# mengcaopku/DCNet

Measured on AMD Instinct MI355X. Metric: clips/sec (T=8, 416x416, bs8) fwd+bwd, higher is better.
Workload: dtype f32; 1 GPU; T=8 416x416 bs8/GPU L=20 fp32, 64 img/GPU/step as pairs, fwd+5 losses+bwd+RMSprop; arith=f16x2-split MFMA, fp32 accumulate, parallelism=dp1, ranks_seen=1, reducer=none, step=hipGraph replay (fwd+losses+bwd+RMSprop), sampler=mt

## Files before the change

### dcnet_amd/csrc/optim.hip

```cpp
#include "common.h"

namespace {

constexpr int RMS_CHUNK = 32;
template <int K> struct Chunk { float* t[K][RMS_CHUNK]; long long n[RMS_CHUNK]; };

template <int W, bool READ, class F>
__device__ __forceinline__ void walk(float* const (&w)[W], const float* __restrict__ g, const long long n, F f) {
  uintptr_t bits = READ ? (uintptr_t)g : 0;
#pragma unroll
  for (int k = 0; k < W; ++k) bits |= (uintptr_t)w[k];
  const long long n4 = (bits & 15) == 0 ? n / 4 : 0;
  const long long stride = (long long)gridDim.x * 256;
  for (long long i = (long long)blockIdx.x * 256 + threadIdx.x; i < n4; i += stride) {
    f32x4 x[W];
#pragma unroll
    for (int k = 0; k < W; ++k) x[k] = reinterpret_cast<const f32x4*>(w[k])[i];
    const f32x4 gg = READ ? reinterpret_cast<const f32x4*>(g)[i] : f32x4{};
#pragma unroll
    for (int e = 0; e < 4; ++e) {
      float a[W];
#pragma unroll
      for (int k = 0; k < W; ++k) a[k] = x[k][e];
      f(a, gg[e]);
#pragma unroll
      for (int k = 0; k < W; ++k) x[k][e] = a[k];
    }
#pragma unroll
    for (int k = 0; k < W; ++k) reinterpret_cast<f32x4*>(w[k])[i] = x[k];
  }
  for (long long i = n4 * 4 + (long long)blockIdx.x * 256 + threadIdx.x; i < n; i += stride) {
    float a[W];
#pragma unroll
    for (int k = 0; k < W; ++k) a[k] = w[k][i];
    f(a, READ ? g[i] : 0.f);
#pragma unroll
    for (int k = 0; k < W; ++k) w[k][i] = a[k];
  }
}

__device__ __forceinline__ void rms_update(float& p, const float g0, float& v, float lr, float alpha, float eps, float wd) {
#pragma clang fp contract(off)
  const float g = wd != 0.f ? g0 + wd * p : g0;
  v = v * alpha + (1.f - alpha) * g * g;
  p = p - lr * (g / (sqrtf(v) + eps));
}

constexpr int CTL_NORM = 0, CTL_COEF = 1, CTL_APPLY = 2, CTL_SKIPS = 3;
__device__ __forceinline__ float clip_mul(const float g0, const float coef) {
#pragma clang fp contract(off)
  return g0 * coef;
}

template <bool CLIP, int NS, int K, class F>
__device__ __forceinline__ void update_walk(const Chunk<K>& c, const float* __restrict__ ctl, F f) {
  static_assert(K >= 2 + NS, "parameter, gradient and NS state tables");
  float coef = 1.f;
  if (CLIP) {
    if (reinterpret_cast<const int*>(ctl)[CTL_APPLY] == 0) return;
    coef = ctl[CTL_COEF];
  }
  const int t = blockIdx.y;
  float* w[1 + NS];
  w[0] = c.t[0][t];
#pragma unroll
  for (int k = 0; k < NS; ++k) w[1 + k] = c.t[2 + k][t];
  walk<1 + NS, true>(w, c.t[1][t], c.n[t], [=](float (&a)[1 + NS], const float g0) { f(a, CLIP ? clip_mul(g0, coef) : g0); });
}

template <bool CLIP>
__device__ __forceinline__ void rmsprop_body(const Chunk<3>& c, float lr, const float* __restrict__ lr_dev, float alpha, float eps, float wd,
                                             const float* __restrict__ ctl) {
  if (lr_dev) lr = lr_dev[0];
  update_walk<CLIP, 1>(c, ctl, [=](float (&a)[2], const float g) { rms_update(a[0], g, a[1], lr, alpha, eps, wd); });
}

__global__ __launch_bounds__(256) void rmsprop_kernel(const Chunk<3> c, float lr, const float* __restrict__ lr_dev, float alpha, float eps, float wd) {
  rmsprop_body<false>(c, lr, lr_dev, alpha, eps, wd, nullptr);
}
__global__ __launch_bounds__(256) void rmsprop_clip_kernel(const Chunk<3> c, float lr, const float* __restrict__ lr_dev, float alpha, float eps, float wd,
                                                           const float* __restrict__ ctl) {
  rmsprop_body<true>(c, lr, lr_dev, alpha, eps, wd, ctl);
}

constexpr int STEP_CHUNK = 128;
struct StepChunk { int* step[STEP_CHUNK]; float* scal[STEP_CHUNK]; };

__device__ __forceinline__ void adam_prepare_body(const StepChunk& c, float lr, const float* __restrict__ lr_dev, double beta1, double beta2) {
  if (threadIdx.x != 0) return;
  if (lr_dev) lr = lr_dev[0];
  const int t = c.step[blockIdx.x][0] + 1;
  c.step[blockIdx.x][0] = t;
  const double bc1 = 1.0 - pow(beta1, (double)t), bc2 = 1.0 - pow(beta2, (double)t);
  c.scal[blockIdx.x][0] = (float)((double)lr / bc1);
  c.scal[blockIdx.x][1] = (float)(1.0 / sqrt(bc2));
}

__global__ __launch_bounds__(64) void adam_prepare_kernel(const StepChunk c, float lr, const float* __restrict__ lr_dev, double beta1, double beta2) {
  adam_prepare_body(c, lr, lr_dev, beta1, beta2);
}
__global__ __launch_bounds__(64) void adam_prepare_clip_kernel(const StepChunk c, float lr, const float* __restrict__ lr_dev, double beta1, double beta2,
                                                               const int* __restrict__ ctl) {
  if (ctl[CTL_APPLY] == 0) return;
  adam_prepare_body(c, lr, lr_dev, beta1, beta2);
}

__global__ __launch_bounds__(64) void adamw_prepare_kernel(const StepChunk c, float lr, const float* __restrict__ lr_dev, double beta1, double beta2,
                                                           double wd, const int* __restrict__ ctl) {
  if (ctl && ctl[CTL_APPLY] == 0) return;
  adam_prepare_body(c, lr, lr_dev, beta1, beta2);
  if (threadIdx.x != 0) return;
  if (lr_dev) lr = lr_dev[0];
  c.scal[blockIdx.x][2] = (float)(1.0 - (double)lr * wd);
}

__device__ __forceinline__ void adam_update(float& p, const float g0, float& m, float& v, float step_size, float inv_bc2_sqrt, float w1,
                                            float beta2, float w2, float eps, float wd) {
#pragma clang fp contract(off)
  const float g = wd != 0.f ? g0 + wd * p : g0;
  const float d = g - m;
  m = w1 < 0.5f ? m + w1 * d : g - d * (1.f - w1);
  v = v * beta2 + w2 * g * g;
  const float denom = sqrtf(v) * inv_bc2_sqrt + eps;
  p = p - step_size * (m / denom);
}

__device__ __forceinline__ void adamw_update(float& p, const float g, float& m, float& v, float step_size, float inv_bc2_sqrt, float decay,
                                             float w1, float beta2, float w2, float eps) {
#pragma clang fp contract(off)
  const float q = p * decay;
  const float d = g - m;
  m = w1 < 0.5f ? m + w1 * d : g - d * (1.f - w1);
  v = v * beta2 + w2 * g * g;
  const float denom = sqrtf(v) * inv_bc2_sqrt + eps;
  p = q - step_size * (m / denom);
}

template <bool CLIP, bool DECOUPLED = false>
__device__ __forceinline__ void adam_body(const Chunk<5>& c, float w1, float beta2, float w2, float eps, float wd, const float* __restrict__ ctl) {
  const float* __restrict__ s = c.t[4][blockIdx.y];
  const float step_size = s[0], inv_bc2_sqrt = s[1], decay = DECOUPLED ? s[2] : 1.f;
  update_walk<CLIP, 2>(c, ctl, [=](float (&a)[3], const float g) {
    if (DECOUPLED) adamw_update(a[0], g, a[1], a[2], step_size, inv_bc2_sqrt, decay, w1, beta2, w2, eps);
    else adam_update(a[0], g, a[1], a[2], step_size, inv_bc2_sqrt, w1, beta2, w2, eps, wd);
  });
}

__global__ __launch_bounds__(256) void adamw_kernel(const Chunk<5> c, float w1, float beta2, float w2, float eps) {
  adam_body<false, true>(c, w1, beta2, w2, eps, 0.f, nullptr);
}
__global__ __launch_bounds__(256) void adamw_clip_kernel(const Chunk<5> c, float w1, float beta2, float w2, float eps, const float* __restrict__ ctl) {
  adam_body<true, true>(c, w1, beta2, w2, eps, 0.f, ctl);
}

__global__ __launch_bounds__(256) void adam_kernel(const Chunk<5> c, float w1, float beta2, float w2, float eps, float wd) {
  adam_body<false>(c, w1, beta2, w2, eps, wd, nullptr);
}
__global__ __launch_bounds__(256) void adam_clip_kernel(const Chunk<5> c, float w1, float beta2, float w2, float eps, float wd,
                                                        const float* __restrict__ ctl) {
  adam_body<true>(c, w1, beta2, w2, eps, wd, ctl);
}

__device__ __forceinline__ void sgd_update(float& p, const float g0, float& buf, float lr, float mu, float wd) {
#pragma clang fp contract(off)
  const float g = wd != 0.f ? g0 + wd * p : g0;
  buf = buf * mu + g;
  p = p - lr * buf;
}

template <bool CLIP>
__device__ __forceinline__ void sgd_body(const Chunk<3>& c, float lr, const float* __restrict__ lr_dev, float mu, float wd, const float* __restrict__ ctl) {
  if (lr_dev) lr = lr_dev[0];
  update_walk<CLIP, 1>(c, ctl, [=](float (&a)[2], const float g) { sgd_update(a[0], g, a[1], lr, mu, wd); });
}

__global__ __launch_bounds__(256) void sgd_kernel(const Chunk<3> c, float lr, const float* __restrict__ lr_dev, float mu, float wd) {
  sgd_body<false>(c, lr, lr_dev, mu, wd, nullptr);
}
__global__ __launch_bounds__(256) void sgd_clip_kernel(const Chunk<3> c, float lr, const float* __restrict__ lr_dev, float mu, float wd,
                                                       const float* __restrict__ ctl) {
  sgd_body<true>(c, lr, lr_dev, mu, wd, ctl);
}

__global__ __launch_bounds__(64) void ema_prepare_kernel(int* __restrict__ step, float* __restrict__ w, double decay, double tau,
                                                         const int* __restrict__ ctl) {
  if (threadIdx.x != 0 || blockIdx.x != 0) return;
  if (ctl && ctl[CTL_APPLY] == 0) return;
  const int t = step[0] + 1;
  step[0] = t;
  const double d = tau > 0.0 ? decay * (1.0 - exp(-(double)t / tau)) : decay;
  w[0] = (float)(1.0 - d);
}

template <bool WB, class F>
__device__ __forceinline__ void walk2(const Chunk<2>& c, F f) {
  const int t = blockIdx.y;
  float* __restrict__ a = c.t[0][t]; float* __restrict__ b = c.t[1][t];
  const long long n = c.n[t];
  const long long n4 = ((((uintptr_t)a | (uintptr_t)b) & 15) == 0) ? n / 4 : 0;
  const long long stride = (long long)gridDim.x * 256;
  f32x4* __restrict__ a4 = reinterpret_cast<f32x4*>(a); f32x4* __restrict__ b4 = reinterpret_cast<f32x4*>(b);
  const auto f4 = [&](f32x4& x, f32x4& y) {
#pragma unroll
    for (int e = 0; e < 4; ++e) {
      float xe = x[e], ye = y[e];
      f(xe, ye);
      x[e] = xe; y[e] = ye;
    }
  };
  long long i = (long long)blockIdx.x * 256 + threadIdx.x;
  for (; i + stride < n4; i += 2 * stride) {
    f32x4 x0 = a4[i], x1 = a4[i + stride], y0 = b4[i], y1 = b4[i + stride];
    f4(x0, y0); f4(x1, y1);
    a4[i] = x0; a4[i + stride] = x1;
    if (WB) { b4[i] = y0; b4[i + stride] = y1; }
  }
  for (; i < n4; i += stride) {
    f32x4 x0 = a4[i], y0 = b4[i];
    f4(x0, y0);
    a4[i] = x0;
    if (WB) b4[i] = y0;
  }
  for (i = n4 * 4 + (long long)blockIdx.x * 256 + threadIdx.x; i < n; i += stride) {
    float x = a[i], y = b[i];
    f(x, y);
    a[i] = x;
    if (WB) b[i] = y;
  }
}

__device__ __forceinline__ float ema_lerp(const float s, const float x, const float w) {
#pragma clang fp contract(off)
  const float d = x - s;
  const float r = w < 0.5f ? s + w * d : x - d * (1.f - w);
  return d == 0.f ? s : r;
}

__global__ __launch_bounds__(256) void ema_update_kernel(const Chunk<2> c, const float* __restrict__ wp, const int* __restrict__ ctl) {
  if (ctl && ctl[CTL_APPLY] == 0) return;
  const float w = wp[0];
  walk2<false>(c, [=](float& s, float& x) { s = ema_lerp(s, x, w); });
}

__global__ __launch_bounds__(256) void tensor_swap_kernel(const Chunk<2> c) {
  walk2<true>(c, [](float& a, float& b) { const float a0 = a; a = b; b = a0; });
}


template <int WAVES>
__device__ __forceinline__ double block_sum_f64(double v, double* red) {
#pragma unroll
  for (int o = 32; o > 0; o >>= 1) v += __shfl_xor(v, o);
  if ((threadIdx.x & 63) == 0) red[threadIdx.x >> 6] = v;
  __syncthreads();
  double s = red[0];
#pragma unroll
  for (int w = 1; w < WAVES; ++w) s += red[w];
  return s;
}

__device__ __forceinline__ f32x4 load4(const float* __restrict__ g, long long i, bool vec) {
  if (vec) return reinterpret_cast<const f32x4*>(g)[i];
  f32x4 r;
  r[0] = g[4 * i]; r[1] = g[4 * i + 1]; r[2] = g[4 * i + 2]; r[3] = g[4 * i + 3];
  return r;
}
__device__ __forceinline__ double add_squares(double acc, const f32x4 gg) {
#pragma unroll
  for (int e = 0; e < 4; ++e) { const double x = (double)gg[e]; acc += x * x; }
  return acc;
}

__global__ __launch_bounds__(256) void grad_sumsq_kernel(const Chunk<1> c, double* __restrict__ partials) {
  __shared__ double red[4];
  const int t = blockIdx.y;
  const float* __restrict__ g = c.t[0][t];
  const long long n = c.n[t], n4 = n / 4;
  const bool vec = (((uintptr_t)g) & 15) == 0;
  const long long stride = (long long)gridDim.x * 256;
  double acc = 0.0;
  long long i = (long long)blockIdx.x * 256 + threadIdx.x;
  for (; i + 3 * stride < n4; i += 4 * stride) {
    const f32x4 a = load4(g, i, vec), b = load4(g, i + stride, vec), d = load4(g, i + 2 * stride, vec), e = load4(g, i + 3 * stride, vec);
    acc = add_squares(add_squares(add_squares(add_squares(acc, a), b), d), e);
  }
  for (; i < n4; i += stride) acc = add_squares(acc, load4(g, i, vec));
  for (i = n4 * 4 + (long long)blockIdx.x * 256 + threadIdx.x; i < n; i += stride) {
    const double x = (double)g[i]; acc += x * x;
  }
  const double s = block_sum_f64<4>(acc, red);
  if (threadIdx.x == 0) partials[(long long)t * gridDim.x + blockIdx.x] = s;
}

__device__ __forceinline__ float clip_coef(const float norm, const float max_norm) {
#pragma clang fp contract(off)
  const float coef = max_norm / (norm + 1e-6f);
  return coef > 1.f ? 1.f : coef;
}

__global__ __launch_bounds__(1024) void grad_clip_coef_kernel(const double* __restrict__ partials, long long slots, float max_norm, int skip_nonfinite,
                                                              float* __restrict__ ctl) {
  __shared__ double red[16];
  double a0 = 0.0, a1 = 0.0, a2 = 0.0, a3 = 0.0;
  long long i = threadIdx.x;
  for (; i + 3 * 1024 < slots; i += 4 * 1024) {
    const double p0 = partials[i], p1 = partials[i + 1024], p2 = partials[i + 2 * 1024], p3 = partials[i + 3 * 1024];
    a0 += p0; a1 += p1; a2 += p2; a3 += p3;
  }
  if (i < slots) a0 += partials[i];
  if (i + 1024 < slots) a1 += partials[i + 1024];
  if (i + 2 * 1024 < slots) a2 += partials[i + 2 * 1024];
  const double s = block_sum_f64<16>((a0 + a1) + (a2 + a3), red);
  if (threadIdx.x != 0) return;
  const float norm = (float)sqrt(s);
  const int apply = (skip_nonfinite && !__builtin_isfinite(s)) ? 0 : 1;
  ctl[CTL_NORM] = norm;
  ctl[CTL_COEF] = clip_coef(norm, max_norm);
  int* w = reinterpret_cast<int*>(ctl);
  w[CTL_APPLY] = apply;
  if (!apply) w[CTL_SKIPS] = w[CTL_SKIPS] + 1;
}

__global__ __launch_bounds__(256) void grad_scale_kernel(const Chunk<1> c, const float* __restrict__ ctl) {
  const float coef = ctl[CTL_COEF];
  float* const w[1] = {c.t[0][blockIdx.y]};
  walk<1, false>(w, nullptr, c.n[blockIdx.y], [=](float (&a)[1], float) { a[0] = clip_mul(a[0], coef); });
}

inline unsigned blocks_for(long long biggest) {
  const long long bx = (biggest / 4 + 255) / 256;
  return (unsigned)(bx < 1 ? 1 : (bx > 128 ? 128 : bx));
}
inline long long longest(const int64_t* numel, int m) {
  long long biggest = 0;
  for (int i = 0; i < m; ++i)
    if (numel[i] > biggest) biggest = numel[i];
  return biggest;
}

template <class F>
inline int for_chunks(int count, int cap, F f) {
  for (int base = 0; base < count; base += cap) {
    const int e = f(base, count - base < cap ? count - base : cap);
    if (e != DCN_OK) return e;
  }
  return DCN_OK;
}

inline long long sumsq_slots(const int64_t* numel, int count) {
  long long total = 0;
  for_chunks(count, RMS_CHUNK, [&](int base, int m) {
    total += (long long)blocks_for(longest(numel + base, m)) * m;
    return DCN_OK;
  });
  return total;
}

template <int K> using Tables = const float* const* const (&)[K];

template <int K>
int check_tensors(const char* who, Tables<K> tab, const int64_t* numel, int count, bool empties = false) {
  for (int k = 0; k < count; ++k) {
    bool there = true;
    for (int j = 0; j < K; ++j) there = there && tab[j][k];
    DCN_CHECK_ARG(numel[k] >= 0 && (there || (empties && numel[k] == 0)), "%s: null tensor %d", who, k);
  }
  return DCN_OK;
}

template <int K, class L>
int launch_chunks(const char* who, Tables<K> tab, const int64_t* numel, int count, bool empties, L launch) {
  return for_chunks(count, RMS_CHUNK, [&](int base, int m) -> int {
    Chunk<K> c{};
    for (int i = 0; i < m; ++i) {
      for (int j = 0; j < K; ++j) c.t[j][i] = const_cast<float*>(tab[j][base + i]);
      c.n[i] = numel[base + i];
    }
    const long long biggest = longest(numel + base, m);
    if (empties && biggest == 0) return DCN_OK;
    launch(c, dim3(blocks_for(biggest), m));
    DCN_CHECK_LAUNCH(who);
    return DCN_OK;
  });
}

#define OPTIM_LAUNCH(kernel, ...) hipLaunchKernelGGL(kernel, grid, dim3(256), 0, (hipStream_t)stream, __VA_ARGS__)

}

extern "C" int64_t dcn_grad_sumsq_slots(const int64_t* numel, int count) {
  if (!numel || count <= 0) { dcn_set_error("grad_sumsq_slots: bad argument"); return -1; }
  for (int i = 0; i < count; ++i)
    if (numel[i] < 0) { dcn_set_error("grad_sumsq_slots: negative element count of tensor %d", i); return -1; }
  return sumsq_slots(numel, count);
}

extern "C" int dcn_grad_sumsq(const float* const* grads, const int64_t* numel, int count, double* partials, int64_t slots, void* stream) {
  DCN_CHECK_ARG(grads && numel && partials && count > 0, "grad_sumsq: bad argument");
  if (const int e = check_tensors<1>("grad_sumsq", {grads}, numel, count)) return e;
  DCN_CHECK_ARG(slots == sumsq_slots(numel, count), "grad_sumsq: the partials buffer has %lld slots, these tensors need %lld (dcn_grad_sumsq_slots)",
                (long long)slots, sumsq_slots(numel, count));
  long long at = 0;
  return launch_chunks<1>("grad_sumsq", {grads}, numel, count, false, [&](const Chunk<1>& c, dim3 grid) {
    OPTIM_LAUNCH(grad_sumsq_kernel, c, partials + at);
    at += (long long)grid.x * grid.y;
  });
}

extern "C" int dcn_grad_clip_coef(const double* partials, int64_t slots, float max_norm, int skip_nonfinite, void* ctrl, void* stream) {
  DCN_CHECK_ARG(partials && ctrl && slots > 0, "grad_clip_coef: bad argument");
  DCN_CHECK_ARG(max_norm > 0.f, "grad_clip_coef: max_norm %g is not a positive number", (double)max_norm);
  hipLaunchKernelGGL(grad_clip_coef_kernel, dim3(1), dim3(1024), 0, (hipStream_t)stream, partials, (long long)slots, max_norm, skip_nonfinite,
                     (float*)ctrl);
  DCN_CHECK_LAUNCH("grad_clip_coef");
  return DCN_OK;
}

extern "C" int dcn_grad_scale(float* const* grads, const int64_t* numel, int count, const void* ctrl, void* stream) {
  DCN_CHECK_ARG(grads && numel && ctrl && count > 0, "grad_scale: bad argument");
  if (const int e = check_tensors<1>("grad_scale", {grads}, numel, count)) return e;
  return launch_chunks<1>("grad_scale", {grads}, numel, count, false,
                          [&](const Chunk<1>& c, dim3 grid) { OPTIM_LAUNCH(grad_scale_kernel, c, (const float*)ctrl); });
}

static int rmsprop_step(const char* who, float* const* params, const float* const* grads, float* const* square_avgs, const int64_t* numel,
                        int count, float lr, const float* lr_dev, float alpha, float eps, float weight_decay, const float* ctl, void* stream) {
  DCN_CHECK_ARG(params && grads && square_avgs && numel && count > 0, "%s: bad argument", who);
  if (const int e = check_tensors<3>(who, {params, grads, square_avgs}, numel, count)) return e;
  return launch_chunks<3>(who, {params, grads, square_avgs}, numel, count, false, [&](const Chunk<3>& c, dim3 grid) {
    if (ctl) OPTIM_LAUNCH(rmsprop_clip_kernel, c, lr, lr_dev, alpha, eps, weight_decay, ctl);
    else OPTIM_LAUNCH(rmsprop_kernel, c, lr, lr_dev, alpha, eps, weight_decay);
  });
}

extern "C" int dcn_rmsprop_step(float* const* params, const float* const* grads, float* const* square_avgs, const int64_t* numel,
                                int count, float lr, const float* lr_dev, float alpha, float eps, float weight_decay, void* stream) {
  return rmsprop_step("rmsprop_step", params, grads, square_avgs, numel, count, lr, lr_dev, alpha, eps, weight_decay, nullptr, stream);
}

extern "C" int dcn_rmsprop_step_clipped(float* const* params, const float* const* grads, float* const* square_avgs, const int64_t* numel,
                                        int count, float lr, const float* lr_dev, float alpha, float eps, float weight_decay, const void* ctrl,
                                        void* stream) {
  DCN_CHECK_ARG(ctrl, "rmsprop_step_clipped: no control block");
  return rmsprop_step("rmsprop_step_clipped", params, grads, square_avgs, numel, count, lr, lr_dev, alpha, eps, weight_decay, (const float*)ctrl, stream);
}

static int adam_prepare(const char* who, bool decoupled, int* const* steps, float* const* scal, int count, float lr, const float* lr_dev, double beta1,
                        double beta2, double weight_decay, const int* ctl, void* stream) {
  DCN_CHECK_ARG(steps && scal && count > 0, "%s: bad argument", who);
  DCN_CHECK_ARG(beta1 >= 0.0 && beta1 < 1.0 && beta2 >= 0.0 && beta2 < 1.0, "%s: betas (%g, %g) outside [0, 1)", who, beta1, beta2);
  DCN_CHECK_ARG(!decoupled || weight_decay >= 0.0, "%s: negative weight_decay", who);
  for (int k = 0; k < count; ++k)
    DCN_CHECK_ARG(steps[k] && scal[k], "%s: null tensor %d", who, k);
  return for_chunks(count, STEP_CHUNK, [&](int base, int m) -> int {
    StepChunk c{};
    for (int i = 0; i < m; ++i) { c.step[i] = steps[base + i]; c.scal[i] = scal[base + i]; }
    const dim3 grid(m), block(64);
    if (decoupled) hipLaunchKernelGGL(adamw_prepare_kernel, grid, block, 0, (hipStream_t)stream, c, lr, lr_dev, beta1, beta2, weight_decay, ctl);
    else if (ctl) hipLaunchKernelGGL(adam_prepare_clip_kernel, grid, block, 0, (hipStream_t)stream, c, lr, lr_dev, beta1, beta2, ctl);
    else hipLaunchKernelGGL(adam_prepare_kernel, grid, block, 0, (hipStream_t)stream, c, lr, lr_dev, beta1, beta2);
    DCN_CHECK_LAUNCH(who);
    return DCN_OK;
  });
}

extern "C" int dcn_adam_prepare(int* const* steps, float* const* scal, int count, float lr, const float* lr_dev, double beta1, double beta2,
                                void* stream) {
  return adam_prepare("adam_prepare", false, steps, scal, count, lr, lr_dev, beta1, beta2, 0.0, nullptr, stream);
}

extern "C" int dcn_adam_prepare_clipped(int* const* steps, float* const* scal, int count, float lr, const float* lr_dev, double beta1, double beta2,
                                        const void* ctrl, void* stream) {
  DCN_CHECK_ARG(ctrl, "adam_prepare_clipped: no control block");
  return adam_prepare("adam_prepare_clipped", false, steps, scal, count, lr, lr_dev, beta1, beta2, 0.0, (const int*)ctrl, stream);
}

extern "C" int dcn_adamw_prepare(int* const* steps, float* const* scal, int count, float lr, const float* lr_dev, double beta1, double beta2,
                                 double weight_decay, void* stream) {
  return adam_prepare("adamw_prepare", true, steps, scal, count, lr, lr_dev, beta1, beta2, weight_decay, nullptr, stream);
}

extern "C" int dcn_adamw_prepare_clipped(int* const* steps, float* const* scal, int count, float lr, const float* lr_dev, double beta1, double beta2,
                                         double weight_decay, const void* ctrl, void* stream) {
  DCN_CHECK_ARG(ctrl, "adamw_prepare_clipped: no control block");
  return adam_prepare("adamw_prepare_clipped", true, steps, scal, count, lr, lr_dev, beta1, beta2, weight_decay, (const int*)ctrl, stream);
}

static int adam_step(const char* who, bool decoupled, float* const* params, const float* const* grads, float* const* exp_avgs,
                     float* const* exp_avg_sqs, const float* const* scal, const int64_t* numel, int count, double beta1, double beta2, float eps,
                     float weight_decay, const float* ctl, void* stream) {
  DCN_CHECK_ARG(params && grads && exp_avgs && exp_avg_sqs && scal && numel && count > 0, "%s: bad argument", who);
  DCN_CHECK_ARG(beta1 >= 0.0 && beta1 < 1.0 && beta2 >= 0.0 && beta2 < 1.0, "%s: betas (%g, %g) outside [0, 1)", who, beta1, beta2);
  if (decoupled) DCN_CHECK_ARG(eps >= 0.f, "%s: negative eps", who);
  else DCN_CHECK_ARG(eps >= 0.f && weight_decay >= 0.f, "%s: negative eps or weight_decay", who);
  if (const int e = check_tensors<5>(who, {params, grads, exp_avgs, exp_avg_sqs, scal}, numel, count)) return e;
  const float w1 = (float)(1.0 - beta1), b2 = (float)beta2, w2 = (float)(1.0 - beta2);
  return launch_chunks<5>(who, {params, grads, exp_avgs, exp_avg_sqs, scal}, numel, count, false, [&](const Chunk<5>& c, dim3 grid) {
    if (decoupled && ctl) OPTIM_LAUNCH(adamw_clip_kernel, c, w1, b2, w2, eps, ctl);
    else if (decoupled) OPTIM_LAUNCH(adamw_kernel, c, w1, b2, w2, eps);
    else if (ctl) OPTIM_LAUNCH(adam_clip_kernel, c, w1, b2, w2, eps, weight_decay, ctl);
    else OPTIM_LAUNCH(adam_kernel, c, w1, b2, w2, eps, weight_decay);
  });
}

extern "C" int dcn_adam_step(float* const* params, const float* const* grads, float* const* exp_avgs, float* const* exp_avg_sqs,
                             const float* const* scal, const int64_t* numel, int count, double beta1, double beta2, float eps,
                             float weight_decay, void* stream) {
  return adam_step("adam_step", false, params, grads, exp_avgs, exp_avg_sqs, scal, numel, count, beta1, beta2, eps, weight_decay, nullptr, stream);
}

extern "C" int dcn_adam_step_clipped(float* const* params, const float* const* grads, float* const* exp_avgs, float* const* exp_avg_sqs,
                                     const float* const* scal, const int64_t* numel, int count, double beta1, double beta2, float eps,
                                     float weight_decay, const void* ctrl, void* stream) {
  DCN_CHECK_ARG(ctrl, "adam_step_clipped: no control block");
  return adam_step("adam_step_clipped", false, params, grads, exp_avgs, exp_avg_sqs, scal, numel, count, beta1, beta2, eps, weight_decay,
                   (const float*)ctrl, stream);
}

extern "C" int dcn_adamw_step(float* const* params, const float* const* grads, float* const* exp_avgs, float* const* exp_avg_sqs,
                              const float* const* scal, const int64_t* numel, int count, double beta1, double beta2, float eps, void* stream) {
  return adam_step("adamw_step", true, params, grads, exp_avgs, exp_avg_sqs, scal, numel, count, beta1, beta2, eps, 0.f, nullptr, stream);
}

extern "C" int dcn_adamw_step_clipped(float* const* params, const float* const* grads, float* const* exp_avgs, float* const* exp_avg_sqs,
                                      const float* const* scal, const int64_t* numel, int count, double beta1, double beta2, float eps,
                                      const void* ctrl, void* stream) {
  DCN_CHECK_ARG(ctrl, "adamw_step_clipped: no control block");
  return adam_step("adamw_step_clipped", true, params, grads, exp_avgs, exp_avg_sqs, scal, numel, count, beta1, beta2, eps, 0.f, (const float*)ctrl,
                   stream);
}

static int sgd_step(const char* who, float* const* params, const float* const* grads, float* const* momentum_bufs, const int64_t* numel, int count,
                    float lr, const float* lr_dev, float momentum, float weight_decay, const float* ctl, void* stream) {
  DCN_CHECK_ARG(params && grads && momentum_bufs && numel && count > 0, "%s: bad argument", who);
  DCN_CHECK_ARG(momentum >= 0.f && weight_decay >= 0.f, "%s: negative momentum or weight_decay", who);
  if (const int e = check_tensors<3>(who, {params, grads, momentum_bufs}, numel, count)) return e;
  return launch_chunks<3>(who, {params, grads, momentum_bufs}, numel, count, false, [&](const Chunk<3>& c, dim3 grid) {
    if (ctl) OPTIM_LAUNCH(sgd_clip_kernel, c, lr, lr_dev, momentum, weight_decay, ctl);
    else OPTIM_LAUNCH(sgd_kernel, c, lr, lr_dev, momentum, weight_decay);
  });
}

extern "C" int dcn_sgd_step(float* const* params, const float* const* grads, float* const* momentum_bufs, const int64_t* numel, int count,
                            float lr, const float* lr_dev, float momentum, float weight_decay, void* stream) {
  return sgd_step("sgd_step", params, grads, momentum_bufs, numel, count, lr, lr_dev, momentum, weight_decay, nullptr, stream);
}

extern "C" int dcn_sgd_step_clipped(float* const* params, const float* const* grads, float* const* momentum_bufs, const int64_t* numel, int count,
                                    float lr, const float* lr_dev, float momentum, float weight_decay, const void* ctrl, void* stream) {
  DCN_CHECK_ARG(ctrl, "sgd_step_clipped: no control block");
  return sgd_step("sgd_step_clipped", params, grads, momentum_bufs, numel, count, lr, lr_dev, momentum, weight_decay, (const float*)ctrl, stream);
}

extern "C" int dcn_ema_prepare(int* step, float* w, double decay, double tau, const void* ctrl, void* stream) {
  DCN_CHECK_ARG(step && w, "ema_prepare: bad argument");
  DCN_CHECK_ARG(decay >= 0.0 && decay < 1.0, "ema_prepare: decay %g outside [0, 1)", decay);
  DCN_CHECK_ARG(tau >= 0.0, "ema_prepare: tau %g is negative", tau);
  hipLaunchKernelGGL(ema_prepare_kernel, dim3(1), dim3(64), 0, (hipStream_t)stream, step, w, decay, tau, (const int*)ctrl);
  DCN_CHECK_LAUNCH("ema_prepare");
  return DCN_OK;
}

extern "C" int dcn_ema_update(float* const* shadow, const float* const* src, const int64_t* numel, int count, const float* w, const void* ctrl,
                              void* stream) {
  DCN_CHECK_ARG(count >= 0 && w && (count == 0 || (shadow && src && numel)), "ema_update: bad argument");
  if (const int e = check_tensors<2>("ema_update", {shadow, src}, numel, count, true)) return e;
  return launch_chunks<2>("ema_update", {shadow, src}, numel, count, true,
                          [&](const Chunk<2>& c, dim3 grid) { OPTIM_LAUNCH(ema_update_kernel, c, w, (const int*)ctrl); });
}

extern "C" int dcn_tensor_swap(float* const* a, float* const* b, const int64_t* numel, int count, void* stream) {
  DCN_CHECK_ARG(count >= 0 && (count == 0 || (a && b && numel)), "tensor_swap: bad argument");
  if (const int e = check_tensors<2>("tensor_swap", {a, b}, numel, count, true)) return e;
  return launch_chunks<2>("tensor_swap", {a, b}, numel, count, true, [&](const Chunk<2>& c, dim3 grid) { OPTIM_LAUNCH(tensor_swap_kernel, c); });
}
```

### dcnet_amd/csrc/wprep.hip

```cpp
#include "common.h"

namespace {

struct FilterJob {
  const float* src;
  float* ohwi;
  float* ohwi_split;
  float* t;
  float* t_split;
  unsigned* amax;
  void* ohwi_b16;
  void* t_b16;
  int co, ci, T;
  int blk0;
  int ablk0;
  int pad_;
};

__device__ __forceinline__ int find_job(const FilterJob* jobs, int njobs, int b, bool amax) {
  int lo = 0, hi = njobs - 1;
  while (lo < hi) {
    const int mid = (lo + hi + 1) >> 1;
    if ((amax ? jobs[mid].ablk0 : jobs[mid].blk0) <= b) lo = mid; else hi = mid - 1;
  }
  return lo;
}

constexpr int AMAX_CHUNK = 4096;

__global__ __launch_bounds__(256) void filters_amax_kernel(const FilterJob* __restrict__ jobs, int njobs) {
  __shared__ float red[4];
  const int j = find_job(jobs, njobs, blockIdx.x, true);
  const FilterJob job = jobs[j];
  const long long numel = (long long)job.co * job.ci * job.T;
  const long long base = (long long)(blockIdx.x - job.ablk0) * AMAX_CHUNK;
  float vmax = 0.f;
#pragma unroll
  for (int k = 0; k < AMAX_CHUNK / 1024; ++k) {
    const long long i = base + k * 1024 + threadIdx.x * 4;
    if (i + 3 < numel) {
      const f32x4 v = *reinterpret_cast<const f32x4*>(job.src + i);
      vmax = fmaxf(fmaxf(vmax, fmaxf(fabsf(v[0]), fabsf(v[1]))), fmaxf(fabsf(v[2]), fabsf(v[3])));
    } else {
      for (long long q = i; q < numel; ++q) vmax = fmaxf(vmax, fabsf(job.src[q]));
    }
  }
  vmax = wave_max(vmax);
  if ((threadIdx.x & 63) == 0) red[threadIdx.x >> 6] = vmax;
  __syncthreads();
  if (threadIdx.x == 0) amax_update(job.amax, fmaxf(fmaxf(red[0], red[1]), fmaxf(red[2], red[3])), blockIdx.x);
}

__device__ __forceinline__ float scale_of(unsigned bits) {
  const int be = (int)((bits >> 23) & 0xFF);
  int e = (be == 0 || be == 255) ? 0 : 14 - (be - 126);
  e = e > 100 ? 100 : (e < -100 ? -100 : e);
  return __uint_as_float((unsigned)(e + 127) << 23);
}

typedef _Float16 f16x8_t __attribute__((ext_vector_type(8)));
__device__ __forceinline__ void split_store8(float* dst, const float* v, float s) {
  f16x8_t h, l;
#pragma unroll
  for (int k = 0; k < 8; ++k) { const float t = v[k] * s; h[k] = (_Float16)t; l[k] = (_Float16)(t - (float)h[k]); }
  *reinterpret_cast<f16x8_t*>(dst) = h;
  *reinterpret_cast<f16x8_t*>(dst + 4) = l;
}

__global__ __launch_bounds__(256) void filters_xform_kernel(const FilterJob* __restrict__ jobs, int njobs) {
  __shared__ float tile[32][33];
  const int j = find_job(jobs, njobs, blockIdx.x, false);
  const FilterJob job = jobs[j];
  const int tci = job.ci / 32, tco = job.co / 32;
  int b = blockIdx.x - job.blk0;
  const int ci0 = (b % tci) * 32; b /= tci;
  const int co0 = (b % tco) * 32; b /= tco;
  const int tap = b;
  const float s = scale_of(amax_read(job.amax));
  const long long numel = (long long)job.co * job.ci * job.T;
  const int r = threadIdx.x >> 3, c4 = (threadIdx.x & 7) * 4;
  {
    const float* sp = job.src + ((long long)(co0 + r) * job.ci + ci0 + c4) * job.T + tap;
#pragma unroll
    for (int e = 0; e < 4; ++e) tile[r][c4 + e] = sp[(long long)e * job.T];
  }
  __syncthreads();
  if (job.ohwi) {
    const f32x4 v = {tile[r][c4], tile[r][c4 + 1], tile[r][c4 + 2], tile[r][c4 + 3]};
    *reinterpret_cast<f32x4*>(job.ohwi + ((long long)(co0 + r) * job.T + tap) * job.ci + ci0 + c4) = v;
  }
  if (job.t) {
    const f32x4 v = {tile[c4][r], tile[c4 + 1][r], tile[c4 + 2][r], tile[c4 + 3][r]};
    *reinterpret_cast<f32x4*>(job.t + ((long long)(ci0 + r) * job.T + tap) * job.co + co0 + c4) = v;
  }
  if (threadIdx.x < 128) {
    const int rr = threadIdx.x >> 2, g = (threadIdx.x & 3) * 8;
    float v[8];
    typedef __bf16 bf16x8_t __attribute__((ext_vector_type(8)));
    if (job.ohwi_b16) {
      bf16x8_t b;
#pragma unroll
      for (int e = 0; e < 8; ++e) b[e] = (__bf16)tile[rr][g + e];
      *reinterpret_cast<bf16x8_t*>(reinterpret_cast<__bf16*>(job.ohwi_b16) + ((long long)(co0 + rr) * job.T + tap) * job.ci + ci0 + g) = b;
    }
    if (job.t_b16) {
      bf16x8_t b;
#pragma unroll
      for (int e = 0; e < 8; ++e) b[e] = (__bf16)tile[g + e][rr];
      *reinterpret_cast<bf16x8_t*>(reinterpret_cast<__bf16*>(job.t_b16) + ((long long)(ci0 + rr) * job.T + tap) * job.co + co0 + g) = b;
    }
    if (job.ohwi_split) {
#pragma unroll
      for (int e = 0; e < 8; ++e) v[e] = tile[rr][g + e];
      split_store8(job.ohwi_split + ((long long)(co0 + rr) * job.T + tap) * job.ci + ci0 + g, v, s);
    }
    if (job.t_split) {
#pragma unroll
      for (int e = 0; e < 8; ++e) v[e] = tile[g + e][rr];
      split_store8(job.t_split + ((long long)(ci0 + rr) * job.T + tap) * job.co + co0 + g, v, s);
    }
  }
  if (blockIdx.x == job.blk0 && threadIdx.x == 0) {
    if (job.ohwi_split) job.ohwi_split[numel] = s;
    if (job.t_split) job.t_split[numel] = s;
  }
}

}

extern "C" int dcn_filter_job_bytes(void) { return (int)sizeof(FilterJob); }

extern "C" int dcn_prepare_filters(const void* jobs, int njobs, int total_blocks, int total_amax_blocks,
                                   uint32_t* amax_all, int64_t amax_words, void* stream_) {
  hipStream_t stream = (hipStream_t)stream_;
  DCN_CHECK_ARG(jobs && njobs > 0 && total_blocks > 0 && total_amax_blocks > 0 && amax_all && amax_words > 0, "prepare_filters: bad argument");
  if (hipMemsetAsync(amax_all, 0, (size_t)amax_words * 4, stream) != hipSuccess) { dcn_set_error("prepare_filters: memset failed"); return DCN_ERR_LAUNCH; }
  hipLaunchKernelGGL(filters_amax_kernel, dim3(total_amax_blocks), dim3(256), 0, stream, (const FilterJob*)jobs, njobs);
  DCN_CHECK_LAUNCH("filters_amax");
  hipLaunchKernelGGL(filters_xform_kernel, dim3(total_blocks), dim3(256), 0, stream, (const FilterJob*)jobs, njobs);
  DCN_CHECK_LAUNCH("filters_xform");
  return DCN_OK;
}
```

### dcnet_amd/darknet.py

```python
from __future__ import annotations

import os
from typing import Dict, List, Optional, Sequence

import numpy as np
import torch
import torch.nn as nn

from . import convblock, ops


def parse_model_config(path: str) -> List[dict]:
    blocks: List[dict] = []
    with open(path, "r") as fh:
        for raw in fh:
            line = raw.strip()
            if not line or line.startswith("#"):
                continue
            if line.startswith("["):
                blocks.append({"type": line[1:-1].rstrip()})
                if blocks[-1]["type"] in ("convolutional", "yoloconvolutional"):
                    blocks[-1]["batch_normalize"] = 0
            else:
                key, value = line.split("=", 1)
                blocks[-1][key.strip()] = value.strip()
    return blocks


_ANCHORS = "10,13,  16,30,  33,23,  30,61,  62,45,  59,119,  116,90,  156,198,  373,326"


def yolov3_blocks(width: int = 416, height: int = 416) -> List[dict]:
    blocks: List[dict] = [dict(type="net", batch="1", subdivisions="1", width=str(width), height=str(height),
                               channels="3", momentum="0.9", decay="0.0005")]

    def conv(filters, size, stride=1, bn=1, act="leaky", kind="convolutional"):
        b = {"type": kind, "batch_normalize": bn} if bn else {"type": kind, "batch_normalize": 0}
        if bn:
            b["batch_normalize"] = "1"
        b.update(filters=str(filters), size=str(size), stride=str(stride), pad="1", activation=act)
        blocks.append(b)

    def shortcut():
        blocks.append({"type": "shortcut", "from": "-3", "activation": "linear"})

    conv(32, 3)
    for filters, reps in ((64, 1), (128, 2), (256, 8), (512, 8), (1024, 4)):
        conv(filters, 3, 2)
        for _ in range(reps):
            conv(filters // 2, 1); conv(filters, 3); shortcut()
    for mask, (filters, lateral) in zip(("6,7,8", "3,4,5", "0,1,2"), ((512, None), (256, 61), (128, 36))):
        if lateral is not None:
            blocks.append({"type": "route", "layers": "-4"})
            conv(filters, 1)
            blocks.append({"type": "upsample", "stride": "2"})
            blocks.append({"type": "route", "layers": f"-1, {lateral}"})
        for _ in range(2):
            conv(filters, 1); conv(filters * 2, 3)
        conv(filters, 1, kind="yoloconvolutional")
        conv(filters * 2, 3)
        conv(255, 1, bn=0, act="linear")
        blocks.append({"type": "yolo", "mask": mask, "anchors": _ANCHORS, "classes": "80", "num": "9",
                       "jitter": ".3", "ignore_thresh": ".7", "truth_thresh": "1", "random": "1"})
    return blocks


def write_cfg(path: str, blocks: Optional[Sequence[dict]] = None) -> None:
    blocks = yolov3_blocks() if blocks is None else blocks
    with open(path, "w") as fh:
        for b in blocks:
            fh.write(f"[{b['type']}]\n")
            for k, v in b.items():
                if k != "type" and not (k == "batch_normalize" and str(v) == "0"):
                    fh.write(f"{k}={v}\n")
            fh.write("\n")


class EmptyLayer(nn.Module):
    """Placeholder for route / shortcut slots (model/darknet.py:239-243)."""


class MyUpsample2(nn.Module):
    def forward(self, x):
        return x[:, :, :, None, :, None].expand(-1, -1, -1, 2, -1, 2).reshape(x.size(0), x.size(1), x.size(2) * 2, x.size(3) * 2)


class YOLOLayer(nn.Module):
    def __init__(self, anchors, num_classes, img_dim):
        super().__init__()
        self.anchors, self.num_classes, self.image_dim = anchors, num_classes, img_dim


def create_modules(module_defs: List[dict]):
    hyper = module_defs.pop(0)
    filters_out = [int(hyper["channels"])]
    module_list = nn.ModuleList()
    for i, d in enumerate(module_defs):
        seq = nn.Sequential()
        t = d["type"]
        if t in ("convolutional", "yoloconvolutional"):
            bn = int(d["batch_normalize"]); filters = int(d["filters"]); k = int(d["size"])
            pad = (k - 1) // 2 if int(d["pad"]) else 0
            seq.add_module(f"conv_{i}", nn.Conv2d(filters_out[-1], filters, k, int(d["stride"]), pad, bias=not bn))
            if bn:
                seq.add_module(f"batch_norm_{i}", nn.BatchNorm2d(filters))
            if d["activation"] == "leaky":
                seq.add_module(f"leaky_{i}", nn.LeakyReLU(0.1))
        elif t == "upsample":
            assert int(d["stride"]) == 2
            seq.add_module(f"upsample_{i}", MyUpsample2())
            filters = filters_out[-1]
        elif t == "route":
            layers = [int(x) for x in d["layers"].split(",")]
            filters = sum(filters_out[1:][l] if l >= 0 else filters_out[l] for l in layers)
            seq.add_module(f"route_{i}", EmptyLayer())
        elif t == "shortcut":
            filters = filters_out[int(d["from"])]
            seq.add_module(f"shortcut_{i}", EmptyLayer())
        elif t == "yolo":
            idx = [int(x) for x in d["mask"].split(",")]
            a = [int(x) for x in d["anchors"].split(",")]
            a = [(a[j], a[j + 1]) for j in range(0, len(a), 2)]
            seq.add_module(f"yolo_{i}", YOLOLayer([a[j] for j in idx], int(d["classes"]), 256))
            filters = filters_out[-1]
        else:
            raise ValueError(f"unsupported cfg block type {t!r}")
        module_list.append(seq)
        filters_out.append(filters)
    return hyper, module_list



class _ConvOp:
    __slots__ = ("slot", "src", "dst", "res", "cin", "cout", "k", "stride", "bn", "leaky", "need_dx")


class _UpCatOp:
    __slots__ = ("dst", "up_src", "lat_src", "c_up", "c_lat")


class _AliasOp:
    __slots__ = ("dst", "src")


def build_plan(module_defs: List[dict], in_channels: int = 3):
    n = len(module_defs)
    ch: List[int] = []
    prev = in_channels
    for i, d in enumerate(module_defs):
        t = d["type"]
        if t in ("convolutional", "yoloconvolutional"):
            prev = int(d["filters"])
        elif t == "route":
            ls = [int(x) for x in d["layers"].split(",")]
            prev = sum(ch[l if l >= 0 else i + l] for l in ls)
        elif t == "shortcut":
            prev = ch[i + int(d["from"])]
        ch.append(prev)
    taps = [i - 1 for i, d in enumerate(module_defs) if d["type"] == "yoloconvolutional"]
    live = [False] * n
    stack = list(taps)
    while stack:
        i = stack.pop()
        if i < 0 or live[i]:
            continue
        live[i] = True
        d = module_defs[i]; t = d["type"]
        if t in ("convolutional", "yoloconvolutional", "upsample"):
            stack.append(i - 1)
        elif t == "shortcut":
            stack += [i - 1, i + int(d["from"])]
        elif t == "route":
            stack += [l if l >= 0 else i + l for l in (int(x) for x in d["layers"].split(","))]
    consumers: Dict[int, List[int]] = {i: [] for i in range(-1, n)}
    for i, d in enumerate(module_defs):
        if not live[i]:
            continue
        t = d["type"]
        if t in ("convolutional", "yoloconvolutional", "upsample"):
            consumers[i - 1].append(i)
        elif t == "shortcut":
            consumers[i - 1].append(i); consumers[i + int(d["from"])].append(i)
        elif t == "route":
            for l in (int(x) for x in d["layers"].split(",")):
                consumers[l if l >= 0 else i + l].append(i)
    plan = []
    fused_shortcuts = set(); fused_upsamples = set()
    for i, d in enumerate(module_defs):
        if not live[i]:
            continue
        t = d["type"]
        if t in ("convolutional", "yoloconvolutional"):
            op = _ConvOp()
            op.slot = i; op.src = i - 1; op.dst = i; op.res = None
            op.cin = in_channels if i == 0 else ch[i - 1]; op.cout = int(d["filters"])
            op.k = int(d["size"]); op.stride = int(d["stride"])
            op.bn = bool(int(d["batch_normalize"])); op.leaky = d["activation"] == "leaky"
            op.need_dx = i > 0
            nxt = module_defs[i + 1] if i + 1 < n else None
            if (nxt is not None and nxt["type"] == "shortcut" and live[i + 1] and consumers[i] == [i + 1]
                    and i not in taps):
                op.dst = i + 1; op.res = i + 1 + int(nxt["from"])
                fused_shortcuts.add(i + 1)
            plan.append(op)
        elif t == "shortcut":
            if i not in fused_shortcuts:
                raise NotImplementedError("unfused shortcut (pattern not present in YOLOv3)")
        elif t == "upsample":
            nxt = module_defs[i + 1]
            ok = nxt["type"] == "route" and consumers[i] == [i + 1]
            ls = [int(x) for x in nxt["layers"].split(",")] if ok else []
            if not (ok and len(ls) == 2 and ls[0] == -1):
                raise NotImplementedError("upsample not followed by route(-1, k)")
            fused_upsamples.add(i + 1)
            op = _UpCatOp()
            op.dst = i + 1; op.up_src = i - 1; op.lat_src = ls[1] if ls[1] >= 0 else i + 1 + ls[1]
            op.c_up = ch[i - 1]; op.c_lat = ch[op.lat_src]
            plan.append(op)
        elif t == "route":
            if i in fused_upsamples:
                continue
            ls = [int(x) for x in d["layers"].split(",")]
            if len(ls) != 1:
                raise NotImplementedError("route concat without upsample")
            op = _AliasOp(); op.dst = i; op.src = ls[0] if ls[0] >= 0 else i + ls[0]
            plan.append(op)
    return plan, taps, ch



def _inputs(op):
    return (op.src, op.res) if isinstance(op, _ConvOp) else (op.up_src, op.lat_src) if isinstance(op, _UpCatOp) else (op.src,)


def _cpad(c: int) -> int:
    return 4 if c <= 4 else ops.pad32(c)


def _b16_diag_layer(diag, op, p, x, res, w, bank, act, out, amx):
    fold = (p["gamma"], p["beta"], p["rm"], p["rv"], 1e-5)
    if not diag.get("layers", lambda s_: True)(op.slot):
        ops.set_precision(diag.get("arith", "fp32"))
        try:
            ss = ops.bn_fold(*fold) if op.bn else (None, p["b"])
            o, _ = ops.conv2d_fwd(ops.to_f32(x), w, op.k, op.stride, ss[0], ss[1], act, 0.1,
                                  residual=None if res is None else ops.to_f32(diag.get("_r32", {}).get(op.res, res)))
        finally:
            ops.set_precision("bf16s")
        if res is not None and diag.get("res32"):
            diag.setdefault("_r32", {})[op.dst] = o
        out[op.dst] = o; amx[op.dst] = None
        return x, res, True
    x = ops.to_b16(x)
    if res is not None and diag.get("res32"):
        o32, _ = convblock.conv_forward(x, op.k, op.stride, op.cout, bank=bank, fold=fold, act=act, slope=0.1, out_f32=True)
        r32 = diag.setdefault("_r32", {})
        o32 = o32 + (r32[op.res] if op.res in r32 else ops.to_f32(res))
        r32[op.dst] = o32
        out[op.dst] = ops.to_b16(o32); amx[op.dst] = None
        return x, res, True
    return x, (None if res is None else ops.to_b16(res)), False


def _run_forward(plan, taps, x_nhwc, P, training: bool, save: Optional[dict], banks=None, taps_b16: bool = False):
    out: Dict[int, torch.Tensor] = {-1: x_nhwc}
    am = ops.use_amax()
    s16 = ops.storage_b16()
    amx: Dict[int, Optional[torch.Tensor]] = {-1: None}
    readers: Dict[int, list] = {}
    f8_left: Dict[int, int] = {}
    for op in plan:
        for s_ in _inputs(op):
            if s_ is not None:
                readers.setdefault(s_, []).append(op)

    def sole_pre_reader(op, x):
        rd = readers.get(op.dst, [])
        if not (am and ops.PRE_ACT and training and save is not None and len(rd) == 1 and op.dst not in taps and op.res is None):
            return False
        nx = rd[0]
        ho, wo = ops.conv_out_hw(x.shape[1], x.shape[2], op.k, op.stride)
        return (isinstance(nx, _ConvOp) and nx.bn and nx.src == op.dst and nx.res != op.dst
                and ops.pre_supported(x.shape[0], ho, wo, nx.cin, nx.cout, nx.k, nx.stride))

    early = [i for i, op in enumerate(plan) if isinstance(op, _ConvOp) and op.k == 3 and op.cin == 32 and op.cout == 64]
    early_at = early[-1] if early else -1
    early_event = None
    for i_op, op in enumerate(plan):
        if i_op == early_at + 1 and early_at >= 0:
            early_event = torch.cuda.Event(); early_event.record()
        if isinstance(op, _ConvOp):
            p = P[op.slot]
            x = out[op.src]; ax = amx.get(op.src)
            bank = banks.get(op.slot, p["w"]) if banks is not None else None
            if bank is not None and getattr(banks, "pending", None) is not None:
                torch.cuda.current_stream().wait_stream(banks.pending)
                banks.pending = None
            if bank is not None:
                w, aw, wsp, w16 = bank["ohwi"], (bank["amax"] if am else None), bank["split"], bank["b16"]
            else:
                w = ops.weight_to_ohwi(p["w"]); wsp = w16 = None
                aw = ops.absmax(p["w"]) if (am and op.cin > 4) else None
            ao = ops.amax_slot(x.device) if am else None
            res = out[op.res] if op.res is not None else None
            act = ops.ACT_LEAKY if op.leaky else ops.ACT_NONE
            if s16 and ops.B16_DIAG is not None and not training and op.cin > 4:
                x, res, done = _b16_diag_layer(ops.B16_DIAG, op, p, x, res, w, bank, act, out, amx)
                if done:
                    continue
            last8 = (s16 and x.dtype == torch.bfloat16 and ops.f8_takes(op.cin, op.cout, op.k)
                     and convblock.last_q8_reader(f8_left, op.src, sum(1 for r_ in readers.get(op.src, []) if isinstance(r_, _ConvOp)
                                                                      and ops.f8_takes(r_.cin, r_.cout, r_.k))))

            def conv(**kw):
                return convblock.conv_forward(x, op.k, op.stride, op.cout, w=w, bank=bank, amax_x=ax, amax_w=aw, w_split=wsp, w_b16=w16,
                                              drop_q8=last8, **kw)

            if op.bn and training:
                ay = ops.amax_slot(x.device) if (not isinstance(x, ops.PreAct) and sole_pre_reader(op, x)) else None
                y, stats = conv(want_stats=True, amax_out=ay)
                q_ = ops.storage_f8() and any(isinstance(r_, _ConvOp) and r_.src == op.dst and ops.f8_takes(r_.cin, r_.cout, r_.k)
                                              for r_ in readers.get(op.dst, []))
                mi, o, ao = convblock.train_bn_forward(y, stats, p["gamma"], p["beta"], 1e-5, p["momentum"], p["rm"], p["rv"], act, 0.1,
                                                       residual=res, amax_out=ao, amax_y=ay, out_b16=s16, quant=q_)
                if save is not None:
                    save[op.slot] = convblock.SavedLayer(x, y, w, bank, ax, aw, mi=mi)
            else:
                fold, shift = ((p["gamma"], p["beta"], p["rm"], p["rv"], 1e-5), None) if op.bn else (None, p["b"])
                if save is None:
                    o, _ = conv(fold=fold, shift=shift, act=act, slope=0.1, residual=res, amax_out=ao)
                else:
                    a, ss = conv(fold=fold, shift=shift, act=act, slope=0.1, amax_out=ao if res is None else None)
                    o = a if res is None else ops.scale_act(a, None, None, ops.ACT_NONE, 0.0, residual=res, amax_out=ao)
                    save[op.slot] = convblock.SavedLayer(x, a, w, bank, ax, aw, scale=None if ss is None else ss[0])
            if s16:
                o = ops.to_b16(o)
            out[op.dst] = o; amx[op.dst] = ao
        elif isinstance(op, _UpCatOp):
            up, lat = out[op.up_src], out[op.lat_src]
            if up.dtype != lat.dtype:
                up = ops.to_b16(up) if lat.dtype == torch.bfloat16 else ops.to_f32(up)
            n, h, w_, _ = lat.shape
            buf = torch.empty((n, h, w_, op.c_up + op.c_lat), dtype=lat.dtype, device=lat.device)
            ops.upsample2_into(up, buf[..., :op.c_up])
            ops.copy_slice(lat, buf[..., op.c_up:])
            out[op.dst] = buf
            amx[op.dst] = ops.absmax(lat, ops.absmax(up)) if am else None
        else:
            out[op.dst] = out[op.src]; amx[op.dst] = amx.get(op.src)
    return [ops.to_f32(out[t]) if (s16 and not taps_b16) else out[t] for t in taps], [amx.get(t) for t in taps], early_event


def _run_backward(plan, taps, grads_taps, P, save, training: bool, sink=None, bucket_bytes: int = 0):
    pending: list = []
    pending_bytes = 0
    g: Dict[int, Optional[torch.Tensor]] = {}
    s16 = ops.storage_b16()

    def add(slot, t):
        cur = g.get(slot)
        if cur is None:
            if not t.is_contiguous():
                buf = torch.empty(t.shape, dtype=t.dtype, device=t.device)
                ops.copy_slice(t, buf)
                t = buf
            g[slot] = t
        else:
            ops.copy_slice(t, cur, accumulate=True)

    for t, gt in zip(taps, grads_taps):
        if gt is not None:
            g0 = gt.clone(memory_format=torch.contiguous_format)
            add(t, ops.to_b16(g0) if s16 else g0)
    pg: Dict[int, dict] = {}
    producer = {op.dst: op for op in plan if isinstance(op, _ConvOp)}
    first_use: Dict[int, int] = {}
    for i, op in enumerate(plan):
        for s_ in _inputs(op):
            if s_ is not None:
                first_use.setdefault(s_, i)
    index_of = {id(op): i for i, op in enumerate(plan)}
    tapped: Dict[int, torch.Tensor] = {}
    held = None

    def release():
        nonlocal held, pending_bytes
        ops.release_held_wgrads()
        if held is not None:
            d_, slot_, hw_ = held
            held = None
            d_["w"] = hw_.issue()
            if sink is not None:
                pending.append((slot_, "w", d_["w"])); pending_bytes += d_["w"].numel() * 4

    def finished(slot, d):
        nonlocal pending, pending_bytes
        pg[slot] = d
        if sink is not None:
            for k_, t_ in d.items():
                if t_ is not None:
                    pending.append((slot, k_, t_)); pending_bytes += t_.numel() * 4
            if pending_bytes >= bucket_bytes:
                sink(pending); pending = []; pending_bytes = 0

    for op in reversed(plan):
        dout = g.pop(op.dst, None)
        if dout is None:
            continue
        if isinstance(op, _AliasOp):
            add(op.src, dout)
        elif isinstance(op, _UpCatOp):
            n, h2, w2, _ = dout.shape
            cur = g.get(op.up_src)
            if cur is None:
                cur = torch.empty((n, h2 // 2, w2 // 2, op.c_up), dtype=dout.dtype, device=dout.device)
                ops.upsample2_bwd(dout[..., :op.c_up], cur, False)
                g[op.up_src] = cur
            else:
                ops.upsample2_bwd(dout[..., :op.c_up], cur, True)
            add(op.lat_src, dout[..., op.c_up:])
        else:
            p = P[op.slot]
            rec = save.pop(op.slot)
            x, y = rec.x, rec.y
            act = ops.ACT_LEAKY if op.leaky else ops.ACT_NONE
            stem_fused = (op.bn and training and not op.need_dx and ops.STEM_FUSED_BWD and torch.is_tensor(x) and x.shape[3] == 4 and op.cout == 32
                          and op.k == 3 and op.stride == 1 and op.res is None and torch.is_tensor(y) and y.is_contiguous() and x.shape[2] >= 32)
            if s16 and torch.is_tensor(x) and x.dtype == torch.float32 and dout.dtype == torch.bfloat16 and not stem_fused:
                dout = ops.to_f32(dout)
            shape = tuple(p["w"].shape)
            d = {}
            ady = ops.amax_slot(dout.device) if ops.use_amax() else None
            if stem_fused:
                dw, d["gamma"], d["beta"] = ops.stem_bwd_weight_bn(x, y, dout, rec.mi[0], rec.mi[1], p["gamma"], p["beta"], act, 0.1,
                                                                   part=tapped.pop(op.slot, None))
                d["w"] = ops.weight_grad_to_oihw(dw, shape)
                finished(op.slot, d)
                continue
            if op.bn and training:
                dy, d["gamma"], d["beta"] = ops.bn_act_bwd(y, dout, rec.mi[0], rec.mi[1], p["gamma"], p["beta"], act, 0.1, amax_out=ady,
                                                           part=tapped.pop(op.slot, None),
                                                           quant=bool(op.need_dx) and ops.f8_takes(op.cout, op.cin, op.k))
            else:
                if rec.scale is not None:
                    dy, dgamma, d["beta"] = convblock.frozen_bn_backward(y, dout, rec.scale, p["gamma"], p["beta"], act, 0.1,
                                                                         want_sums=p["affine_grad"])
                    d["gamma"] = dgamma
                else:
                    dy = ops.act_bwd(y, dout, 0.1) if op.leaky else dout
                    if p["b"] is not None:
                        d["b"] = dy.reshape(-1, op.cout).sum(0)
                ady = None
            if op.res is not None:
                add(op.res, dout)
            release()

            def dgrad():
                if not op.need_dx:
                    return
                cur = g.get(op.src)
                b16 = s16 and dy.dtype == torch.bfloat16
                prev = producer.get(op.src)
                tap = None
                if prev is not None and prev.bn and first_use.get(op.src) == index_of[id(op)]:
                    tap = convblock.bn_tap_for(b16, training, x.shape[3], op.k, op.stride, save.get(prev.slot), P[prev.slot]["gamma"],
                                               P[prev.slot]["beta"], ops.ACT_LEAKY if prev.leaky else ops.ACT_NONE, 0.1)
                fb = rec.bank
                dx, part = convblock.conv_dgrad(dy, x.shape, op.k, op.stride, w=rec.w, bank=fb, out=cur, accumulate=cur is not None, tap=tap,
                                                amax_dy=ady, amax_w=rec.aw, wt_ready=fb and (fb["t"], fb["tsplit"]), wt_b16=fb and fb["tb16"])
                if part is not None:
                    tapped[prev.slot] = part
                if cur is None:
                    g[op.src] = dx

            _, dw = convblock.schedule_wgrad(x, dy, op.k, op.stride, shape, dgrad, amax_x=rec.ax, amax_dy=ady, may_hold=True)
            if isinstance(dw, ops.HeldWgrad):
                held = (d, op.slot, dw)
            else:
                d["w"] = dw
            finished(op.slot, d)
    release()
    if sink is not None and pending:
        sink(pending)
    if pg:
        ops.join_side(next(iter(P.values()))["w"].device)
    return pg


class _DarknetFn(torch.autograd.Function):

    @staticmethod
    def forward(ctx, net: "Darknet", training: bool, image: torch.Tensor, *flat):
        plan, taps = net._plan, net._taps
        P = net._param_table(flat, ctx.needs_input_grad[3:])
        x = ops.nchw_to_nhwc(image.contiguous(), 4)
        need_grad = any(ctx.needs_input_grad[3:]) and bool(net.__dict__.get("_grad_on", True))
        ctx.no_backward_reason = None if need_grad else "nothing was saved: the forward ran with gradients off (or no parameter requires one)"
        if ops.storage_f8() and not training and need_grad:
            need_grad = False
            ctx.no_backward_reason = ("fp8 storage has no backward with BatchNorm on its running statistics (eval mode, freeze_batchnorm): "
                                      "fp32 and bf16 storage (\"bf16s\") have it")
        save = {} if need_grad else None
        outs, tap_amax, net._early_event = _run_forward(plan, taps, x, P, training, save, net._filter_banks(P),
                                                        taps_b16=bool(net.__dict__.get("_taps_b16")))
        net._tap_amax = tap_amax
        if save is not None:
            for rec in save.values():
                rec.unlink_outputs(outs)
            ctx.save_for_backward(*outs)
        ctx.net, ctx.training, ctx.save, ctx.nflat = net, training, save, len(flat)
        ctx.P = P
        return tuple(outs)

    @staticmethod
    def backward(ctx, *grads):
        net = ctx.net
        if ctx.save is None:
            why = getattr(ctx, "no_backward_reason", None) or ("this node's saved tensors were consumed by an earlier backward "
                                                               "(one backward per forward; retain_graph is not supported)")
            raise (NotImplementedError if "fp8 storage" in why else RuntimeError)("dcnet_amd.Darknet: " + why)
        outs = ctx.saved_tensors
        save = ctx.save
        ctx.save = None
        for rec in save.values():
            rec.link_outputs(outs)
        red = net.__dict__.get("_grad_reducer")
        sink = None
        if red is not None:
            pmap = net._slot_params()
            sink = lambda items: red.push([(pmap[(slot, key)], t) for slot, key, t in items if (slot, key) in pmap])
        pg = _run_backward(net._plan, net._taps, grads, ctx.P, save, ctx.training, sink, red.bucket_bytes if red is not None else 0)
        if red is not None:
            red.join_backward()
        flat_grads: List[Optional[torch.Tensor]] = []
        for op in net._conv_ops:
            d = pg.get(op.slot, {})
            flat_grads.append(d.get("w"))
            if op.bn:
                flat_grads += [d.get("gamma"), d.get("beta")]
            else:
                flat_grads.append(d.get("b"))
        return (None, None, None) + tuple(flat_grads)


class Darknet(nn.Module):

    def __init__(self, config_path: str = "./model/yolov3.cfg", img_size: int = 416, obj_out: bool = False):
        super().__init__()
        if obj_out:
            raise NotImplementedError("obj_out=True (YOLO detection output) is outside the DCNet hot path")
        self.config_path = config_path
        self.obj_out = obj_out
        if config_path and os.path.exists(config_path):
            self.module_defs = parse_model_config(config_path)
        else:
            self.module_defs = yolov3_blocks()
        self.hyperparams, self.module_list = create_modules(self.module_defs)
        self.img_size = img_size
        self.seen = 0
        self.header_info = np.array([0, 0, 0, self.seen, 0], dtype=np.int32)
        self._plan, self._taps, self._ch = build_plan(self.module_defs, int(self.hyperparams["channels"]))
        self._conv_ops = [op for op in self._plan if isinstance(op, _ConvOp)]

    def _flat_params(self) -> List[torch.Tensor]:
        flat = []
        for op in self._conv_ops:
            seq = self.module_list[op.slot]
            conv = seq[0]
            flat.append(conv.weight)
            if op.bn:
                flat += [seq[1].weight, seq[1].bias]
            else:
                flat.append(conv.bias)
        return flat

    def _param_table(self, flat, needs=None):
        P = {}
        it = iter(flat)
        nd = iter(needs if needs is not None else [True] * len(flat))
        for op in self._conv_ops:
            seq = self.module_list[op.slot]
            d = dict(w=next(it).detach(), b=None, gamma=None, beta=None, rm=None, rv=None, momentum=0.1, affine_grad=True)
            next(nd)
            if op.bn:
                bn = seq[1]
                d["gamma"], d["beta"] = next(it).detach(), next(it).detach()
                d["affine_grad"] = bool(next(nd)) | bool(next(nd))
                d["rm"], d["rv"], d["momentum"] = bn.running_mean, bn.running_var, bn.momentum
            else:
                d["b"] = next(it).detach()
                next(nd)
            P[op.slot] = d
        return P

    def _slot_params(self):
        out = {}
        for op in self._conv_ops:
            seq = self.module_list[op.slot]
            out[(op.slot, "w")] = seq[0].weight
            if op.bn:
                out[(op.slot, "gamma")] = seq[1].weight; out[(op.slot, "beta")] = seq[1].bias
            elif seq[0].bias is not None:
                out[(op.slot, "b")] = seq[0].bias
        return out

    def _filter_banks(self, P):
        if not ops.FILTER_BANKS:
            return None
        fb = convblock.cached_filter_banks(self.__dict__, "_fbanks", {slot: d["w"] for slot, d in P.items()})
        main = torch.cuda.current_stream()
        prep = self.__dict__.get("_prep_stream")
        if prep is None or prep.device != main.device:
            prep = torch.cuda.Stream(device=main.device)
            self.__dict__["_prep_stream"] = prep
        prep.wait_stream(main)
        with torch.cuda.stream(prep):
            fb.refresh()
        fb.pending = prep
        return fb

    def forward_nhwc(self, x: torch.Tensor, taps_b16: bool = False) -> List[torch.Tensor]:
        self.__dict__["_taps_b16"] = bool(taps_b16) and ops.storage_b16()
        self.__dict__["_grad_on"] = torch.is_grad_enabled()
        if not x.is_cuda:
            raise RuntimeError("dcnet_amd.Darknet runs on an MI355X only: move the model and inputs to cuda "
                               "(there is no CPU path; the CPU restatement lives in oracle/ for tests)")
        training = self.training and not self.__dict__.get("_bn_frozen", False)
        if training:
            torch._foreach_add_([self.module_list[op.slot][1].num_batches_tracked for op in self._conv_ops if op.bn], 1)
        return list(_DarknetFn.apply(self, training, x, *self._flat_params()))

    def freeze_batchnorm(self, frozen: bool = True) -> None:
        self.__dict__["_bn_frozen"] = bool(frozen)
        self.train(self.training)

    def train(self, mode: bool = True):
        super().train(mode)
        if self.__dict__.get("_bn_frozen", False):
            for m in self.modules():
                if isinstance(m, nn.modules.batchnorm._BatchNorm):
                    m.training = False
        return self

    def forward(self, x, targets=None):
        if targets is not None:
            raise NotImplementedError("YOLO detection training (targets=...) is outside the DCNet hot path")
        return [t.permute(0, 3, 1, 2) for t in self.forward_nhwc(x)]

    def load_weights(self, weights_path: str) -> None:
        with open(weights_path, "rb") as fp:
            header = np.fromfile(fp, dtype=np.int32, count=5)
            weights = np.fromfile(fp, dtype=np.float32)
        self.header_info = header
        self.seen = int(header[3])
        ptr = 0

        def take(t: torch.Tensor):
            nonlocal ptr
            n = t.numel()
            if ptr + n > weights.size:
                raise ValueError(f"{weights_path}: truncated weights file")
            t.data.copy_(torch.from_numpy(weights[ptr:ptr + n]).view_as(t))
            ptr += n

        for d, seq in zip(self.module_defs, self.module_list):
            if d["type"] in ("convolutional", "yoloconvolutional"):
                conv = seq[0]
                if int(d["batch_normalize"]):
                    bn = seq[1]
                    take(bn.bias); take(bn.weight); take(bn.running_mean); take(bn.running_var)
                else:
                    take(conv.bias)
                take(conv.weight)

    def save_weights(self, path: str, cutoff: int = -1, reference_layout: bool = False) -> None:
        hdr = np.array(self.header_info, dtype=np.int32).copy()
        hdr[3] = self.seen
        defs = self.module_defs if cutoff == -1 else self.module_defs[:cutoff]
        if reference_layout and cutoff == -1:
            defs = self.module_defs[:-1]
        kinds = ("convolutional",) if reference_layout else ("convolutional", "yoloconvolutional")
        with open(path, "wb") as fp:
            hdr.tofile(fp)
            for d, seq in zip(defs, self.module_list):
                if d["type"] in kinds:
                    conv = seq[0]
                    if int(d["batch_normalize"]):
                        bn = seq[1]
                        for t in (bn.bias, bn.weight, bn.running_mean, bn.running_var):
                            t.detach().cpu().numpy().astype(np.float32).tofile(fp)
                    else:
                        conv.bias.detach().cpu().numpy().astype(np.float32).tofile(fp)
                    conv.weight.detach().cpu().numpy().astype(np.float32).tofile(fp)
```

### dcnet_amd/functions.py

```python
from __future__ import annotations

from typing import Optional

import torch

from . import convblock, ops


class ConvBNAct(torch.autograd.Function):

    @staticmethod
    def forward(ctx, x, weight, gamma, beta, bn, ksize: int, training: bool, slope: float, amax_x=None, bank=None, out_b16: bool = False,
                grad_on: bool = True):
        cout = weight.shape[0]
        am = ops.use_amax()
        if bank is not None and x.shape[3] != weight.shape[1]:
            bank = None
        ctx.wparam = convblock.direct_wgrad_param(weight, training)
        ctx.b16 = ops.storage_b16() and bank is not None
        ctx.x_f32 = x.dtype == torch.float32
        w = wsp = aw = ax = ao = None
        if ctx.b16:
            x = ops.to_b16(x.contiguous())
        else:
            if bank is not None:
                w, wsp = bank["ohwi"], bank["split"]
                aw = bank["amax"] if am else None
            else:
                w = ops.weight_to_ohwi(weight, ci_pad=x.shape[3])
                aw = ops.absmax(weight.detach()) if am else None
            ax = (amax_x if amax_x is not None else ops.absmax(x)) if am else None
            ao = ops.amax_slot(x.device) if am else None
        if training:
            y, stats = convblock.conv_forward(x, ksize, 1, cout, w=w, bank=bank, want_stats=True, amax_x=ax, amax_w=aw, w_split=wsp)
            aux, out, _ = convblock.train_bn_forward(y, stats, gamma.detach(), beta.detach(), bn.eps, bn.momentum, bn.running_mean,
                                                     bn.running_var, ops.ACT_LEAKY, slope, bn=bn, amax_out=ao, out_f32=not out_b16)
        else:
            out, aux = convblock.conv_forward(x, ksize, 1, cout, w=w, bank=bank, fold=(gamma.detach(), beta.detach(), bn.running_mean,
                                                                                       bn.running_var, bn.eps),
                                              act=ops.ACT_LEAKY, slope=slope, out_f32=not out_b16, amax_x=ax, amax_w=aw, amax_out=ao, w_split=wsp)
            y = out
            if ctx.b16 and ops.storage_f8():
                y = None
            elif ctx.b16 and grad_on and any(ctx.needs_input_grad[:4]):
                y = ops.to_b16(out)
        if y is not None:
            ctx.save_for_backward(x, y, aux, w, gamma, beta)
        ctx.bank = bank
        ctx.meta = (ksize, training, slope, tuple(weight.shape))
        ctx.amax = (ax, aw)
        if ao is not None:
            ctx.mark_non_differentiable(ao)
        return out, ao

    @staticmethod
    def backward(ctx, dout, _ga=None):
        ksize, training, slope, wshape = ctx.meta
        if ctx.b16 and not training and not ctx.saved_tensors:
            raise NotImplementedError("ConvBNAct, fp8 storage: no backward with BatchNorm on its running statistics (eval mode, "
                                      "freeze_batchnorm); fp32 and bf16 storage (\"bf16s\") have it")
        x, y, aux, w, gamma, beta = ctx.saved_tensors
        gamma, beta = gamma.detach(), beta.detach()
        ax, aw = ctx.amax
        bank = ctx.bank
        dout = dout.contiguous()
        ady = None
        if training:
            ady = ops.amax_slot(dout.device) if ops.use_amax() else None
            dy, dgamma, dbeta = ops.bn_act_bwd(y, dout, aux[0], aux[1], gamma, beta, ops.ACT_LEAKY, slope, amax_out=ady,
                                               quant=ctx.needs_input_grad[0] and ops.f8_takes(y.shape[3], x.shape[3], ksize))
        else:
            dy, dgamma, dbeta = convblock.frozen_bn_backward(y, dout, aux[0], gamma, beta, ops.ACT_LEAKY, slope,
                                                             want_sums=ctx.needs_input_grad[2] or ctx.needs_input_grad[3])

        def dgrad():
            if not ctx.needs_input_grad[0]:
                return None
            return convblock.conv_dgrad(dy, x.shape, ksize, 1, w=w, bank=bank, out_f32=ctx.x_f32, amax_dy=ady, amax_w=aw,
                                        wt_ready=bank and (bank["t"], bank["tsplit"]))[0]

        dx, dwt = convblock.schedule_wgrad(x, dy, ksize, 1, wshape, dgrad, amax_x=ax, amax_dy=ady, direct_into=ctx.wparam)
        if ctx.wparam is None:
            ops.join_side(x.device)
        return dx, dwt, dgamma, dbeta, None, None, None, None, None, None, None, None


class ConvBias(torch.autograd.Function):

    @staticmethod
    def forward(ctx, x, weight, bias, amax_x=None):
        cout = weight.shape[0]
        cop = ops.pad32(cout)
        ctx.wparam = convblock.direct_wgrad_param(weight)
        w = ops.weight_to_ohwi(weight, ci_pad=x.shape[3], co_pad=cop)
        b = torch.zeros(cop, dtype=torch.float32, device=x.device)
        b[:cout] = bias.detach()
        ctx.wshape = tuple(weight.shape)
        ctx.b16 = ops.storage_b16() and weight.shape[2] == 1 and x.shape[3] % 32 == 0
        ctx.x_f32 = x.dtype == torch.float32
        ctx.amax, bank = (None, None), None
        if ctx.b16:
            x = ops.to_b16(x.contiguous())
            w = w.reshape(cop, -1).to(torch.bfloat16)
            bank = {"b16": w.reshape(-1)}
        y, _ = convblock.conv_forward(x, weight.shape[2], 1, cop, w=w, bank=bank, shift=b, out_f32=True)
        ctx.save_for_backward(x, w)
        if not ctx.b16:
            ctx.amax = (amax_x, ops.absmax(weight.detach()) if ops.use_amax() else None)
        return y

    @staticmethod
    def backward(ctx, dy):
        x, w = ctx.saved_tensors
        co, ci, k, _ = ctx.wshape
        ax, aw = ctx.amax
        dy = dy.contiguous()
        rowsum = lambda: ops.colsum_rows(dy.view(-1, dy.shape[-1]))[:co]
        if ctx.b16:
            db = rowsum()
            dy, ady = ops.to_b16(dy), None
        else:
            db = None
            ady = ops.absmax(dy) if ops.use_amax() else None

        def dgrad():
            nonlocal db
            if db is None:
                db = rowsum()
            if not ctx.needs_input_grad[0]:
                return None
            bank = {"tb16": w.t().contiguous().reshape(-1)} if ctx.b16 else None
            return convblock.conv_dgrad(dy, x.shape, k, 1, w=w, bank=bank, out_f32=ctx.x_f32, amax_dy=ady, amax_w=aw)[0]

        dx, dwt = convblock.schedule_wgrad(x, dy, k, 1, ctx.wshape, dgrad, amax_x=ax, amax_dy=ady, after=False, direct_into=ctx.wparam)
        if ctx.wparam is None:
            ops.join_side(x.device)
        return dx, dwt, db, None


class L2Norm(torch.autograd.Function):

    @staticmethod
    def forward(ctx, x):
        out, norm, _, _ = ops.l2norm_score_fwd(x)
        ctx.save_for_backward(out, norm)
        return out

    @staticmethod
    def backward(ctx, dout):
        out, norm = ctx.saved_tensors
        dx, _ = ops.l2norm_score_bwd(out, norm, dout.contiguous(), None, None, 0)
        return dx


class NormScore(torch.autograd.Function):

    @staticmethod
    def forward(ctx, x, q, want_neg: bool):
        n, h, w, e = x.shape
        q = q.contiguous()
        corr, norm, score, flip = ops.l2norm_score_fwd(x, q, h * w, want_flip=want_neg)
        ctx.save_for_backward(corr, norm, q)
        if not want_neg:
            return corr, score.view(n, h, w), None
        return corr, score.view(n, h, w), flip.view(n, h, w)

    @staticmethod
    def backward(ctx, dcorr, dscore, dneg):
        corr, norm, q = ctx.saved_tensors
        q = q.detach()
        n, h, w, _ = corr.shape
        dout = dcorr.contiguous() if dcorr is not None else None
        ds = dscore.contiguous().view(-1) if dscore is not None else None
        dn = dneg.contiguous().view(-1) if dneg is not None else None
        use_q = q if (ds is not None or dn is not None) else None
        dx, dq = ops.l2norm_score_bwd(corr, norm, dout, use_q, ds, h * w, dscore_flip=dn)
        return dx, dq, None


class RowDot(torch.autograd.Function):

    @staticmethod
    def forward(ctx, x, q, flip: bool):
        n, h, w, e = x.shape
        x = x.contiguous(); q = q.contiguous()
        ctx.save_for_backward(x, q)
        ctx.flip = flip
        return ops.rowdot_fwd(x, q, h * w, flip).view(n, h, w)

    @staticmethod
    def backward(ctx, ds):
        x, q = ctx.saved_tensors
        n, h, w, e = x.shape
        dx, dq = ops.rowdot_bwd(x, q.detach(), ds.contiguous().view(-1), h * w, ctx.flip, ctx.needs_input_grad[0], ctx.needs_input_grad[1])
        return dx, dq, None


class NormAccumulate(torch.autograd.Function):

    @staticmethod
    def forward(ctx, x, acc: Optional[torch.Tensor], scale: float):
        out, _, _, _ = ops.l2norm_score_fwd(x, out=acc, out_scale=scale, accumulate=acc is not None)
        ctx.mark_dirty(*([acc] if acc is not None else []))
        return out

    @staticmethod
    def backward(ctx, g):
        raise NotImplementedError("the n_frame (inference) model has no backward; train with pair semantics")


class PhraseAttn(torch.autograd.Function):

    @staticmethod
    def forward(ctx, context, embedded, ids, w0, b0, w1, b1, normalize: bool):
        context = context.contiguous(); embedded = embedded.contiguous(); ids = ids.contiguous()
        d = context.shape[2]
        wa = w0.detach().reshape(-1).contiguous(); wb = None if w1 is None else w1.detach().reshape(-1).contiguous()
        attn, out, vnorm = ops.phrase_attn_fwd(context, embedded, ids, wa, b0.detach(), wb, None if b1 is None else b1.detach(), normalize)
        ctx.save_for_backward(context, embedded, wa, wb if wb is not None else wa.new_empty(0), attn, out,
                              vnorm if vnorm is not None else wa.new_empty(0))
        ctx.meta = (normalize, w1 is not None, tuple(w0.shape), d)
        ctx.mark_non_differentiable(attn)
        return out[0], (out[1] if w1 is not None else None), attn

    @staticmethod
    def backward(ctx, g0, g1, _gattn):
        context, embedded, wa, wb, attn, out, vnorm = ctx.saved_tensors
        normalize, two, wshape, d = ctx.meta
        dout = torch.zeros_like(out) if (g0 is None or (two and g1 is None)) else torch.empty_like(out)
        if g0 is not None:
            ops.copy_slice(g0.contiguous(), dout[0])
        if two and g1 is not None:
            ops.copy_slice(g1.contiguous(), dout[1])
        dctx, demb, dwb = ops.phrase_attn_bwd(context, embedded, wa, wb if two else None, attn, out, vnorm if normalize else None, dout, normalize)
        h = 2 if two else 1
        dw0 = dwb[:d].view(wshape); db0 = dwb[h * d:h * d + 1]
        dw1 = dwb[d:2 * d].view(wshape) if two else None
        db1 = dwb[2 * d + 1:2 * d + 2] if two else None
        return dctx, demb, None, dw0, db0, dw1, db1, None


class HeadTail(torch.autograd.Function):

    @staticmethod
    def forward(ctx, l0, l1, l2, s0, s1, s2, q_loc, coord, w_le, b_le, g_le, be_le, w_lt, b_lt, g_lt, be_lt, bn_le, bn_lt, training: bool):
        logits = [l0.contiguous(), l1.contiguous(), l2.contiguous()]
        B = logits[0].shape[0]
        sims = [s.contiguous().view(B, -1) for s in (s0, s1, s2)]
        P = coord.shape[0]
        cnt = B * P
        det = lambda t: t.detach().contiguous()
        w_le, b_le, g_le, be_le, w_lt, b_lt, g_lt, be_lt = map(det, (w_le, b_le, g_le, be_le, w_lt, b_lt, g_lt, be_lt))
        q_loc = q_loc.contiguous()
        e8, xh, stat, mom = ops.locemb_fwd(coord, w_le, b_le, g_le, be_le, bn_le, training, cnt)
        only, obj_map, objn, X = ops.head_obj(logits, sims, e8)
        wp = ops.pad_rows(w_lt, X.shape[1])
        M = ops.gemm_nt(X, wp).view(B, 8, -1)
        Mp, bp, saved = ops.locbn_fwd(M, mom, b_lt, g_lt, be_lt, bn_lt, training, cnt)
        loc_map = ops.locmod_fwd(e8, Mp, bp, q_loc)
        outbox, loc, mm = ops.head_final_fwd(logits, sims, loc_map)
        if training:
            ops.bump_batches(bn_le); ops.bump_batches(bn_lt)
        ctx.save_for_backward(*logits, *sims, *loc, *only, q_loc, coord, w_le, g_le, be_le, b_lt, g_lt, e8, xh, stat, mom, obj_map, objn, X,
                              wp, M, Mp, bp, saved, mm, bn_lt.running_mean)
        ctx.training = training
        ctx.wshape = tuple(w_lt.shape)
        return (*outbox, *loc, *only)

    @staticmethod
    def backward(ctx, do0, do1, do2, dl0, dl1, dl2, dn0, dn1, dn2):
        sv = ctx.saved_tensors
        logits, sims, loc, only = list(sv[0:3]), list(sv[3:6]), list(sv[6:9]), list(sv[9:12])
        (q_loc, coord, w_le, g_le, be_le, b_lt, g_lt, e8, xh, stat, mom, obj_map, objn, X, wp, M, Mp, bp, saved, mm, rmean_lt) = sv[12:]
        B, P = obj_map.shape
        cnt = B * P
        training = ctx.training
        cg = lambda t: None if t is None else t.contiguous()
        d_out = [cg(do0), cg(do1), cg(do2)]; d_loc = [cg(dl0), cg(dl1), cg(dl2)]; d_only = [cg(dn0), cg(dn1), cg(dn2)]
        dloc_map = ops.head_dloc(logits, sims, loc, d_out, d_loc, mm)
        dE_part, dsum = ops.locmod_bwd(e8, Mp, bp, q_loc, dloc_map)
        dE_a = ops.colsum(dE_part.view(B, P * 8)).view(P, 8)
        dMp = dsum[:, :8]
        dbp = ops.colsum(dsum[:, 8])
        dq_loc = dsum[:, 9]
        dM, gout, dmom = ops.locbn_bwd(M, mom, b_lt, g_lt, rmean_lt, saved, dMp, dbp, training, cnt)
        dM2 = dM.view(B * 8, -1)
        dX = ops.gemm_nn(dM2, wp)
        dwp = ops.gemm_tn(dM2, X)
        dw_lt = ops.pad_rows(dwp, P)
        dobj, dE_b = ops.head_fold(dX, e8, obj_map)
        dlogits, dsim = ops.head_dlogits(logits, sims, loc, only, d_out, d_only, obj_map, objn, dobj)
        g88 = ops.locemb_bwd(coord, w_le, g_le, be_le, xh, stat, dE_a, dE_b, dmom, training)
        shp = [t.shape for t in logits]
        dsim = [d.view(s_[0], s_[1], s_[2]) for d, s_ in zip(dsim, shp)]
        return (*dlogits, *dsim, dq_loc, None, g88[:64].view(8, 8), g88[64:72], g88[72:80], g88[80:88],
                dw_lt.view(ctx.wshape), gout[2], gout[0], gout[1], None, None, None)


class InterframeSample(torch.autograd.Function):

    @staticmethod
    def forward(ctx, fv, raw_neg, top_k: int):
        n, h, w, e = fv.shape
        f = fv.contiguous().view(n, h * w, e)
        index, neg_idx, frame, corr, negf = ops.k9_fwd(f, raw_neg, top_k)
        ctx.save_for_backward(index, neg_idx)
        ctx.shape = (n, h, w, e)
        ctx.mark_non_differentiable(index, neg_idx)
        return frame, corr, negf, index, neg_idx

    @staticmethod
    def backward(ctx, d_frame, d_corr, d_neg, _a, _b):
        index, neg_idx = ctx.saved_tensors
        n, h, w, e = ctx.shape
        z = lambda g, like: torch.zeros(like, dtype=torch.float32, device=index.device) if g is None else g.contiguous()
        b, k, m = neg_idx.shape
        dfv = ops.k9_bwd(index, neg_idx, z(d_frame, (b, k, e)), z(d_corr, (b, k, e)), z(d_neg, (b, k, m, e)), h * w)
        return dfv.view(n, h, w, e), None, None


class CrossModalSample(torch.autograd.Function):

    @staticmethod
    def forward(ctx, fv, context, conv_w, conv_b, neg, csr_off, csr_src):
        n, h, w, e = fv.shape
        v = fv.contiguous().view(n, h * w, e)
        context = context.contiguous()
        vit, cn = ops.colnorm_fwd(v)
        lag, ln = ops.lagnorm_fwd(context)
        cols, _ = ops.crossmap(lag, vit, conv_w.detach().contiguous(), conv_b.detach().contiguous())
        lag_pos, neg_cross = ops.k14_gather(lag, vit, cols, neg)
        ctx.save_for_backward(vit, cn, lag, ln, cols, csr_off, csr_src)
        ctx.shape = (n, h, w, e)
        ctx.mark_non_differentiable(cols)
        return vit, lag_pos, neg_cross, cols

    @staticmethod
    def backward(ctx, d_vit, d_lag_pos, d_neg, _c):
        vit, cn, lag, ln, cols, csr_off, csr_src = ctx.saved_tensors
        n, h, w, e = ctx.shape
        hw = h * w
        dq = torch.zeros_like(vit) if d_vit is None else d_vit.contiguous()
        extra = ops.k14_negscatter(d_neg.contiguous(), csr_off, csr_src, hw) if d_neg is not None else None
        dv = ops.colnorm_bwd(vit, cn, dq, extra, n - 1)
        dctx = None
        if d_lag_pos is not None and ctx.needs_input_grad[1]:
            dctx = ops.k14_dlag(lag, ln, cols, d_lag_pos.contiguous())
        return dv.view(n, h, w, e), dctx, None, None, None, None, None


class Contrastive(torch.autograd.Function):

    @staticmethod
    def forward(ctx, q, pos, neg, temperature: float):
        q, pos, neg = q.contiguous(), pos.contiguous(), neg.contiguous()
        ctx.save_for_backward(q, pos, neg)
        ctx.t = temperature
        return ops.contrastive_fwd(q, pos, neg, temperature)

    @staticmethod
    def backward(ctx, g):
        q, pos, neg = ctx.saved_tensors
        dq, dpos, dneg = ops.contrastive_bwd(q, pos, neg, ctx.t, g.contiguous().view(1))
        return dq, dpos, dneg, None


class DenseLosses(torch.autograd.Function):

    @staticmethod
    def forward(ctx, ob0, ob1, ob2, s0, s1, s2, n0, n1, n2, l0, l1, l2, ti, tf, size: int):
        c = lambda t: t.contiguous()
        outbox = [c(ob0), c(ob1), c(ob2)]; sim = [c(s0), c(s1), c(s2)]; neg = [c(n0), c(n1), c(n2)]; loc = [c(l0), c(l1), c(l2)]
        out, lse = ops.dense_loss_fwd(outbox, sim, neg, loc, ti, tf, size)
        ctx.save_for_backward(*outbox, *sim, *neg, *loc, ti, tf, lse)
        ctx.size = size
        return out[0], out[1], out[2]

    @staticmethod
    def backward(ctx, gy, gr, gl):
        sv = ctx.saved_tensors
        outbox, sim, neg, loc = list(sv[0:3]), list(sv[3:6]), list(sv[6:9]), list(sv[9:12])
        ti, tf, lse = sv[12:]
# ... 268 lines not shown
```

### dcnet_amd/lib.py

```python
from __future__ import annotations

import ctypes
import os
from ctypes import c_char_p, c_double, c_float, c_int, c_int64, c_void_p

_HERE = os.path.dirname(os.path.abspath(__file__))
LIB_PATH = os.path.join(_HERE, "libdcnet_hip.so")

P, I, L, F, D = c_void_p, c_int, c_int64, c_float, c_double

SIGNATURES = {
    "dcn_last_error": (c_char_p, []),
    "dcn_version": (I, []),
    "dcn_nchw_to_nhwc": (I, [P, P, I, I, I, I, I, P]),
    "dcn_nhwc_to_nchw": (I, [P, P, I, I, I, I, I, P]),
    "dcn_oihw_to_ohwi": (I, [P, P, I, I, I, I, I, P]),
    "dcn_ohwi_to_oihw": (I, [P, P, I, I, I, I, I, P]),
    "dcn_conv2d_fwd": (I, [P, P, P, I, I, I, I, I, I, I, P, P, I, F, P, I, I, P, I, P, P, P, P, P, I, P]),
    "dcn_absmax": (I, [P, L, I, I, P, P]),
    "dcn_f8_scale": (I, [P, L, I, I, P, P, P]),
    "dcn_conv2d_stats_rows": (I, [I, I, I, I, I, I]),
    "dcn_conv1_tile": (I, [L, I, I, I, I, I]),
    "dcn_l2norm_score_fwd_form": (I, [I]),
    "dcn_bn_apply_form": (I, [I, I]),
    "dcn_igemm_split_build": (I, [I, I]),
    "dcn_gemm3_variant": (I, []),
    "dcn_conv2d_bwd_data": (I, [P, I, P, P, P, I, I, I, I, I, I, I, I, P, P, P, I, P, P]),
    "dcn_conv2d_bwd_data_tap": (I, [P, I, P, P, P, I, I, I, I, I, I, I, I, P, P, P, I, P, P, P, P, P, P, I, F, P, I, P, P]),
    "dcn_conv2d_bwd_data_tap_rows": (I, [I, I, I, I, I, I, I]),
    "dcn_conv2d_pre_supported": (I, [I, I, I, I, I, I, I]),
    "dcn_conv2d_fwd_pre": (I, [P, P, P, I, I, I, I, I, I, I, P, P, I, F, I, P, P, P, P]),
    "dcn_conv2d_bwd_weight_pre_supported": (I, [I, I, I, I, I, I, I]),
    "dcn_conv2d_bwd_weight_pre": (I, [P, I, P, I, P, P, P, I, I, I, I, I, I, I, P, P, I, F, P, P, P]),
    "dcn_bn_act_amax_bound": (I, [P, P, P, I, F, P, P]),
    "dcn_gemm3_supported": (I, [I, I, I, I]),
    "dcn_gemm3_presplit": (I, [P, I, L, P, I, L, I, I, I, P, P]),
    "dcn_gemm3": (I, [P, I, L, I, P, I, L, I, P, I, L, P, L, I, I, I, I, I, P, P, P]),
    "dcn_filter_job_bytes": (I, []),
    "dcn_prepare_filters": (I, [P, I, I, I, P, L, P]),
    "dcn_conv2d_geom_size": (L, [I, I, I, I, I]),
    "dcn_conv2d_geom": (I, [P, I, I, I, I, I, P]),
    "dcn_conv2d_bwd_weight": (I, [P, I, P, I, P, P, P, P, I, I, I, I, I, I, I, P, P, P]),
    "dcn_conv2d_bwd_weight_ws": (L, [I, I, I, I, I, I, I]),
    "dcn_stem_bwd_weight_bn": (I, [P, P, P, I, P, P, P, P, I, F, P, L, I, I, I, I, P, P, P]),
    "dcn_stem_bwd_weight_bn_ws": (L, [I, I, I]),
    "dcn_stem_bwd_weight_bn_b16": (I, [P, P, P, I, P, P, P, P, I, F, P, L, I, I, I, I, P, P, P]),
    "dcn_bn_ws": (L, [I]),
    "dcn_bn_finalize": (I, [P, I, I, L, P, P, F, F, P, P, P, P, P, P, P, P]),
    "dcn_bn_fold": (I, [P, P, P, P, F, I, P, P, P]),
    "dcn_channel_stats": (I, [P, L, I, I, P, P]),
    "dcn_channel_stats_rows": (I, [L]),
    "dcn_scale_act": (I, [P, P, P, I, F, P, P, L, I, I, P, P]),
    "dcn_bn_act_bwd_reduce": (I, [P, P, I, P, P, P, P, I, F, L, I, P, P]),
    "dcn_bn_bwd_sums": (I, [P, I, I, P, P, P]),
    "dcn_bn_act_bwd_apply": (I, [P, P, I, P, P, P, P, I, F, P, L, L, I, P, P, P]),
    "dcn_act_bwd": (I, [P, P, I, F, L, I, P, P]),
    "dcn_frozen_bn_act_bwd": (I, [P, P, I, P, P, P, I, F, L, I, I, P, P, P, P]),
    "dcn_coattn_e_size": (L, [I, I]),
    "dcn_coattn_saved_size": (L, [I, I, I]),
    "dcn_coattn_fwd_ws": (L, [I, I, I]),
    "dcn_coattn_fwd": (I, [P, P, I, L, P, P, I, L, P, P, P, P, I, I, I, F, P]),
    "dcn_coattn_bwd_ws": (L, [I, I, I]),
    "dcn_coattn_bwd": (I, [P, P, I, L, P, P, I, L, P, P, I, L, P, P, P, P, P, I, L, I, P, I, I, I, F, P]),
    "dcn_l2norm_score_fwd": (I, [P, I, P, I, P, P, P, P, L, I, I, F, I, P]),
    "dcn_l2norm_score_bwd": (I, [P, I, P, P, I, P, P, P, P, I, P, L, I, I, P]),
    "dcn_rowdot_fwd": (I, [P, I, P, I, P, L, I, I, P]),
    "dcn_rowdot_bwd": (I, [P, I, P, I, P, P, I, P, L, I, I, P]),
    "dcn_phrase_attn_fwd": (I, [P, P, P, P, P, P, P, P, P, P, I, I, I, I, I, P]),
    "dcn_phrase_attn_bwd_ws": (L, [I, I, I]),
    "dcn_phrase_attn_bwd": (I, [P, P, P, P, P, P, P, P, P, P, P, P, I, I, I, I, I, P]),
    "dcn_colsum": (I, [P, I, I, I, P, P]),
    "dcn_locemb_fwd": (I, [P, P, P, P, P, P, P, F, F, I, L, I, P, P, P, P, P]),
    "dcn_locemb_bwd": (I, [P, P, P, P, P, P, P, P, P, I, I, P, P]),
    "dcn_head_obj": (I, [P, P, P, P, P, P, P, P, P, I, P]),
    "dcn_pad_rows": (I, [P, I, P, I, I, I, I, P]),
    "dcn_locbn_fwd": (I, [P, P, P, P, P, P, P, F, F, I, I, L, I, P, P, P, P]),
    "dcn_locbn_bwd": (I, [P, P, P, P, P, P, P, L, P, I, I, L, I, P, P, P, P]),
    "dcn_head_final_fwd": (I, [P, P, P, P, P, P, P, P, I, P]),
    "dcn_head_dloc": (I, [P, P, P, P, P, P, P, P, P, I, P]),
    "dcn_head_fold": (I, [P, P, P, I, I, I, P, P, P]),
    "dcn_head_dlogits": (I, [P, P, P, P, P, P, P, P, P, P, P, P, P, I, P]),
    "dcn_k9_fwd": (I, [P, P, P, I, I, I, I, I, P, P, P, P, P, P]),
    "dcn_k9_bwd": (I, [P, P, P, P, P, I, I, I, I, I, P, P]),
    "dcn_colnorm_fwd": (I, [P, I, I, I, P, P, P]),
    "dcn_colnorm_bwd": (I, [P, P, P, P, I, I, I, I, P, P]),
    "dcn_lagnorm_fwd": (I, [P, I, I, I, P, P, P]),
    "dcn_crossmap": (I, [P, P, P, P, I, I, I, I, P, P, P]),
    "dcn_k14_gather": (I, [P, P, P, P, I, I, I, I, I, P, P, P]),
    "dcn_k14_negscatter": (I, [P, P, P, I, I, P, P]),
    "dcn_k14_dlag": (I, [P, P, P, P, I, I, I, I, P, P]),
    "dcn_build_target": (I, [P, P, I, I, P, P, P]),
    "dcn_target_dense": (I, [P, P, I, I, P, P, P]),
    "dcn_dense_loss_fwd": (I, [P, P, P, P, P, P, I, I, P, P, P, P]),
    "dcn_dense_loss_bwd": (I, [P, P, P, P, P, P, P, P, I, I, P, P, P, P, P]),
    "dcn_contrastive_fwd": (I, [P, P, P, L, I, I, F, P, P, P]),
    "dcn_contrastive_bwd": (I, [P, P, P, L, I, I, F, P, P, P, P, P]),
    "dcn_decode_boxes": (I, [P, P, I, I, P, P, P]),
    "dcn_box_iou": (I, [P, P, I, P, P]),
    "dcn_gemm_nt_batched": (I, [P, I, L, P, I, L, P, I, L, I, I, I, I, P]),
    "dcn_mt_sample_crossmodal_csr": (I, [P, I, I, I, P, P]),
    "dcn_upsample2_nhwc": (I, [P, I, P, I, I, I, I, I, P]),
    "dcn_upsample2_nhwc_bwd": (I, [P, I, P, I, I, I, I, I, I, P]),
    "dcn_copy_slice": (I, [P, I, P, I, L, I, I, P]),
    "dcn_locmod_fwd": (I, [P, P, P, P, P, I, I, I, P]),
    "dcn_locmod_bwd_ws": (L, [I, I]),
    "dcn_locmod_bwd": (I, [P, P, P, P, P, P, P, P, I, I, I, P]),
    "dcn_gemm_nt": (I, [P, I, P, I, P, I, I, I, I, P, I, P, I, I, P]),
    "dcn_gemm_nn": (I, [P, I, P, I, P, I, I, I, I, I, I, P]),
    "dcn_gemm_tn": (I, [P, I, P, I, P, I, I, I, I, I, P]),
    "dcn_lstm_cell_fwd": (I, [P, P, P, P, I, P, P, P, P, I, I, I, P]),
    "dcn_lstm_cell_bwd": (I, [P, I, P, P, P, P, P, I, P, I, P, P, I, I, P]),
    "dcn_bilstm_sync_bytes": (L, []),
    "dcn_bilstm_fwd": (I, [P, P, P, P, P, P, P, P, P, P, P, I, I, I, P]),
    "dcn_bilstm_bwd": (I, [P, P, P, P, P, P, P, P, I, I, I, P]),
    "dcn_rmsprop_step": (I, [P, P, P, P, I, F, P, F, F, F, P]),
    "dcn_adam_prepare": (I, [P, P, I, F, P, D, D, P]),
    "dcn_adam_step": (I, [P, P, P, P, P, P, I, D, D, F, F, P]),
    "dcn_sgd_step": (I, [P, P, P, P, I, F, P, F, F, P]),
    "dcn_grad_sumsq_slots": (L, [P, I]),
    "dcn_grad_sumsq": (I, [P, P, I, P, L, P]),
    "dcn_grad_clip_coef": (I, [P, L, F, I, P, P]),
    "dcn_grad_scale": (I, [P, P, I, P, P]),
    "dcn_rmsprop_step_clipped": (I, [P, P, P, P, I, F, P, F, F, F, P, P]),
    "dcn_adam_prepare_clipped": (I, [P, P, I, F, P, D, D, P, P]),
    "dcn_adam_step_clipped": (I, [P, P, P, P, P, P, I, D, D, F, F, P, P]),
    "dcn_sgd_step_clipped": (I, [P, P, P, P, I, F, P, F, F, P, P]),
    "dcn_adamw_prepare": (I, [P, P, I, F, P, D, D, D, P]),
    "dcn_adamw_step": (I, [P, P, P, P, P, P, I, D, D, F, P]),
    "dcn_adamw_prepare_clipped": (I, [P, P, I, F, P, D, D, D, P, P]),
    "dcn_adamw_step_clipped": (I, [P, P, P, P, P, P, I, D, D, F, P, P]),
    "dcn_ema_prepare": (I, [P, P, D, D, P, P]),
    "dcn_ema_update": (I, [P, P, P, I, P, P, P]),
    "dcn_tensor_swap": (I, [P, P, P, I, P]),
    "dcn_fusion_prefill": (I, [P, P, P, I, P, I, I, I, P]),
    "dcn_fusion_bwd_ws": (L, [I, I]),
    "dcn_fusion_bwd": (I, [P, P, P, P, P, P, P, I, I, I, I, I, P]),
    "dcn_row_lengths": (I, [P, I, I, P, P]),
    "dcn_embedding_fwd": (I, [P, P, P, I, I, I, P]),
    "dcn_embedding_bwd": (I, [P, P, P, I, I, I, P]),
    "dcn_set_tuning": (I, [c_char_p, I]),
    "dcn_tuning_info": (I, [I, P, P, P, P, P]),
    "dcn_stream_create": (P, [I]),
    "dcn_stream_destroy": (I, [P]),
    "dcn_stream_priority_range": (I, [P, P]),
    "dcn_prof_enable": (I, [I]),
    "dcn_prof_collect": (I, [P, P, P, P]),
    "dcn_prof_records": (I, [P, P, P, P, I]),
    "dcn_mt_sample_interframe": (I, [P, P, I, I, I, I, P]),
    "dcn_mt_sample_crossmodal": (I, [P, I, I, I, P]),
    "dcn_quant_job_bytes": (I, []),
    "dcn_quant_rows_e4m3_batched": (I, [P, I, I, L, P]),
    "dcn_mt_sample_step": (I, [P, I, I, I, I, I, P, P, P, P, P]),
    "dcn_device_sample_ws": (L, [I]),
    "dcn_device_sample": (I, [P, I, I, I, I, I, P, P, P, P, P, P]),
    "dcn_conv2d_stats_rows_b16": (I, [I, I, I, I, I, I]),
    "dcn_conv2d_fwd_b16": (I, [P, P, P, I, I, I, I, I, I, I, I, P, P, I, F, P, I, I, P, I, P]),
    "dcn_conv2d_bwd_data_b16": (I, [P, I, P, P, I, I, I, I, I, I, I, I, I, P, P, P, P, P, I, F, P, I, P, P]),
    "dcn_conv2d_bwd_weight_ws_b16": (L, [I, I, I, I, I, I, I]),
    "dcn_conv2d_bwd_weight_b16": (I, [P, I, P, I, P, P, P, P, I, I, I, I, I, I, I, P]),
    "dcn_scale_act_b16": (I, [P, I, P, P, I, F, P, I, P, I, L, I, I, P]),
    "dcn_bn_act_bwd_reduce_rows_b16": (I, [L]),
    "dcn_bn_act_bwd_reduce_b16": (I, [P, I, P, I, I, P, P, P, P, I, F, L, I, P, P]),
    "dcn_bn_act_bwd_apply_b16": (I, [P, I, P, I, I, P, P, P, P, I, F, P, L, L, I, P, P]),
    "dcn_frozen_bn_act_bwd_b16": (I, [P, P, I, I, P, P, P, I, F, L, I, I, P, P, P]),
    "dcn_cast_rows": (I, [P, I, I, P, I, I, L, I, I, P]),
    "dcn_upsample2_nhwc_b16": (I, [P, I, P, I, I, I, I, I, P]),
    "dcn_upsample2_nhwc_bwd_b16": (I, [P, I, P, I, I, I, I, I, I, P]),
    "dcn_quant_rows_e4m3": (I, [P, I, L, I, P, I, P, P]),
    "dcn_quant_fusable": (I, [I]),
    "dcn_scale_act_b16_q": (I, [P, P, P, I, F, P, I, P, L, I, P, P, P]),
    "dcn_bn_act_bwd_apply_b16_q": (I, [P, P, I, P, P, P, P, I, F, P, L, L, I, P, P, P, P]),
    "dcn_conv2d_stats_rows_f8": (I, [I, I, I, I, I, I]),
    "dcn_conv2d_fwd_f8": (I, [P, P, P, P, P, I, I, I, I, I, I, I, I, P, P, I, F, P, I, I, P, I, P]),
    "dcn_conv2d_bwd_data_f8": (I, [P, P, P, P, P, I, I, I, I, I, I, I, I, I, P, P, P, P, P, I, F, P, I, P, P]),
    "dcn_post_topk": (I, [P, P, P, P, P, I, I, I, I, P, P, P, P, P, P, P, P, P]),
    "dcn_post_fusion": (I, [P, P, P, P, I, I, I, I, P, P, P]),
    "dcn_clip_prep_ws": (L, [I, I]),
    "dcn_clip_prep": (I, [P, L, P, P, I, I, P, P, P, P]),
    "dcn_bank_write": (I, [P, I, P, P, L, I, P]),
    "dcn_coattn_bank_fwd": (I, [P, P, P, P, L, P, P, I, L, P, P, P, P, I, I, I, F, P]),
    "dcn_post_fusion_bank": (I, [P, P, I, I, I, I, P, P, P]),
    "dcn_bank_write_b16": (I, [P, I, P, P, P, L, I, P]),
    "dcn_bank_concat_b16": (I, [P, L, P, I, L, P, I, I, I, P]),
    "dcn_coattn_bank_form": (I, [I, I]),
}
_VALUE_FUNCS = {"dcn_version", "dcn_conv2d_stats_rows", "dcn_conv2d_bwd_data_tap_rows", "dcn_conv2d_pre_supported",
                "dcn_conv2d_bwd_weight_pre_supported", "dcn_gemm3_supported", "dcn_channel_stats_rows", "dcn_filter_job_bytes", "dcn_prof_records",
                "dcn_conv2d_stats_rows_b16", "dcn_bn_act_bwd_reduce_rows_b16", "dcn_conv2d_stats_rows_f8", "dcn_quant_fusable", "dcn_quant_job_bytes",
                "dcn_conv1_tile", "dcn_l2norm_score_fwd_form", "dcn_bn_apply_form", "dcn_igemm_split_build", "dcn_gemm3_variant",
                "dcn_coattn_bank_form"}
ABI_VERSION = 317


class DcnError(RuntimeError):
    pass


class _Lib:
    def __init__(self, path: str):
        if not os.path.exists(path):
            raise DcnError(
                f"{path} not found: build it with `python -m dcnet_amd.build` "
                "(hipcc --offload-arch=gfx950).  There is no CPU or eager fallback.")
        self._dll = ctypes.CDLL(path)
        for name, (res, args) in SIGNATURES.items():
            try:
                fn = getattr(self._dll, name)
            except AttributeError as e:
                raise DcnError(f"{path} does not export {name}; rebuild the library") from e
            fn.restype = res
            fn.argtypes = args
            if res is I and name not in _VALUE_FUNCS:
                setattr(self, name[4:], self._checked(name, fn))
            else:
                setattr(self, name[4:], fn)
        for kv in [t for t in os.environ.get("DCN_TUNE", "").split(",") if t]:
            k_, v_ = kv.split("=")
            if self._dll.dcn_set_tuning(k_.encode(), int(v_)) != 0:
                raise DcnError(f"DCN_TUNE: {self._dll.dcn_last_error().decode()}")
        if self._dll.dcn_version() != ABI_VERSION:
            raise DcnError(f"{path} has ABI version {self._dll.dcn_version()}, this binding was written for {ABI_VERSION}: "
                           "rebuild the library (python -m dcnet_amd.build --force)")

    def _checked(self, name, fn):
        def call(*a):
            rc = fn(*a)
            if rc != 0:
                raise DcnError(f"{name} failed ({rc}): {self._dll.dcn_last_error().decode()}")
        call.__name__ = name
        return call


def tuning(L: "_Lib" = None) -> dict:
    dll = (L or lib())._dll
    out = {}
    name, desc, val, dflt, abl = c_char_p(), c_char_p(), c_int(), c_int(), c_int()
    while dll.dcn_tuning_info(len(out), ctypes.byref(name), ctypes.byref(val), ctypes.byref(dflt), ctypes.byref(desc), ctypes.byref(abl)) == 0:
        out[name.value.decode()] = {"value": val.value, "default": dflt.value, "desc": desc.value.decode(), "ablation": abl.value}
    return out


def ablation_build() -> bool:
    return tuning()["abl"]["ablation"] == 2


_lib = None


def lib() -> _Lib:
    global _lib
    if _lib is None:
        _lib = _Lib(LIB_PATH)
    return _lib
```

### dcnet_amd/ops.py

```python
from __future__ import annotations

from typing import Optional, Tuple

import ctypes
import os

import torch

from .lib import DcnError, ablation_build, lib

ACT_NONE, ACT_LEAKY = 0, 1

PRECISIONS = {"fp32_mfma": 0, "fp32_bf16x3": 1, "bf16": 2, "fp8": 3, "fp32": 4, "bf16s": 2, "fp8s": 2}
_precision = "fp32"


def set_precision(mode: str) -> None:
    global _precision
    if mode not in PRECISIONS:
        raise ValueError(f"precision {mode!r}: expected one of {sorted(PRECISIONS)}")
    lib().set_tuning(b"precision", PRECISIONS[mode])
    _precision = mode


# ... 177 lines not shown
SLAB_COUNTERS = 4096


def slab_counters(device, slot: int = 0) -> torch.Tensor:
    key = (torch.device(device).index, slot, torch.cuda.current_stream().cuda_stream)
    buf = _slab_counters.get(key)
    if buf is None:
        buf = torch.zeros(SLAB_COUNTERS, dtype=torch.int32, device=device)
        _slab_counters[key] = buf
    return buf


def pad32(c: int) -> int:
    return (c + 31) // 32 * 32


def nchw_to_nhwc(x: torch.Tensor, c_pad: Optional[int] = None) -> torch.Tensor:
    _chk(x, "nchw_to_nhwc")
    n, c, h, w = x.shape
    c_pad = c if c_pad is None else c_pad
    out = torch.empty((n, h, w, c_pad), dtype=torch.float32, device=x.device)
    lib().nchw_to_nhwc(x.data_ptr(), out.data_ptr(), n, c, h, w, c_pad, _s())
    return out


def nhwc_to_nchw(x: torch.Tensor, c: Optional[int] = None) -> torch.Tensor:
    _chk(x, "nhwc_to_nchw")
    n, h, w, ld = x.shape
    c = ld if c is None else c
    out = torch.empty((n, c, h, w), dtype=torch.float32, device=x.device)
    lib().nhwc_to_nchw(x.data_ptr(), out.data_ptr(), n, c, h, w, ld, _s())
    return out


def weight_to_ohwi(w: torch.Tensor, ci_pad: Optional[int] = None, co_pad: Optional[int] = None) -> torch.Tensor:
    w = w.detach()
    _chk(w, "weight_to_ohwi")
    co, ci, kh, kw = w.shape
    if ci <= 4:
        tmp = torch.empty((co, kh, kw, 4), dtype=torch.float32, device=w.device)
        lib().oihw_to_ohwi(w.data_ptr(), tmp.data_ptr(), co, ci, kh, kw, 4, _s())
        out = torch.zeros((co, 64), dtype=torch.float32, device=w.device)
        out[:, :kh * kw * 4] = tmp.view(co, -1)
        return out
    ci_pad = pad32(ci) if ci_pad is None else ci_pad
    co_pad = co if co_pad is None else co_pad
    if kh == 1 and kw == 1 and ci_pad == ci and co_pad == co:
        return w.view(co, 1, 1, ci)
    alloc = torch.zeros if co_pad != co else torch.empty
    out = alloc((co_pad, kh, kw, ci_pad), dtype=torch.float32, device=w.device)
    lib().oihw_to_ohwi(w.data_ptr(), out.data_ptr(), co, ci, kh, kw, ci_pad, _s())
    return out


def weight_grad_to_oihw(dw: torch.Tensor, shape: Tuple[int, int, int, int]) -> torch.Tensor:
    co, ci, kh, kw = shape
    if ci <= 4:
        tmp = dw[:, :kh * kw * 4].contiguous().view(co, kh, kw, 4)
        out = torch.empty(shape, dtype=torch.float32, device=dw.device)
        lib().ohwi_to_oihw(tmp.data_ptr(), out.data_ptr(), co, ci, kh, kw, 4, _s())
        return out
    _chk(dw, "weight_grad_to_oihw")
    ci_pad = dw.shape[3]
    if kh == 1 and kw == 1 and ci_pad == ci and dw.shape[0] == co:
        return dw.view(co, ci, 1, 1)
    out = torch.empty(shape, dtype=torch.float32, device=dw.device)
    lib().ohwi_to_oihw(dw.data_ptr(), out.data_ptr(), co, ci, kh, kw, ci_pad, _s())
    return out


def conv_out_hw(h: int, w: int, k: int, stride: int) -> Tuple[int, int]:
    pad = (k - 1) // 2
    return (h + 2 * pad - k) // stride + 1, (w + 2 * pad - k) // stride + 1


class PreAct:
    __slots__ = ("y", "scale", "shift", "act", "slope")

    def __init__(self, y, scale, shift, act, slope):
        self.y, self.scale, self.shift, self.act, self.slope = y, scale, shift, act, slope

    shape = property(lambda self: self.y.shape)
    device = property(lambda self: self.y.device)

    def materialise(self, amax_out=None):
        return scale_act(self.y, self.scale, self.shift, self.act, self.slope, amax_out=amax_out)


PRE_ACT = True


def pre_supported(n, h, wd, cin, cout, ksize, stride) -> bool:
    return bool(PRE_ACT and _precision == "fp32" and lib().conv2d_pre_supported(n, h, wd, cin, cout, ksize, stride)
                and lib().conv2d_bwd_weight_pre_supported(n, h, wd, cin, cout, ksize, stride))


def bn_act_amax_bound(amax_y, scale, shift, slope):
    out = amax_slot(amax_y.device)
    lib().bn_act_amax_bound(amax_y.data_ptr(), scale.data_ptr(), shift.data_ptr(), scale.numel(), float(slope), out.data_ptr(), _s())
    return out


def conv2d_fwd(x, w_ohwi, ksize, stride, scale=None, shift=None, act=ACT_NONE, slope=0.0,
               residual=None, out=None, want_stats=False, accumulate=False, amax_x=None, amax_w=None, amax_out=None,
               w_split_ready=None, w_b16=None):
    pre = isinstance(x, PreAct)
    if pre and not (scale is None and shift is None and residual is None and act == ACT_NONE and not accumulate and amax_out is None
                    and amax_x is not None and amax_w is not None):
        raise DcnError("conv2d_fwd: a PreAct input takes no epilogue and needs both abs-max words")
    _chk(x.y if pre else x, "conv2d_fwd x")
    n, h, wd, cin = x.shape
    cout = w_ohwi.shape[0]
    ho, wo = conv_out_hw(h, wd, ksize, stride)
    if out is None:
        out = torch.empty((n, ho, wo, cout), dtype=torch.float32, device=x.device)
    ldy = out.stride(2)
    stats = None
    if want_stats:
        rows = lib().conv2d_stats_rows(n, h, wd, cout, ksize, stride)
        stats = torch.empty((rows, 2, cout), dtype=torch.float32, device=x.device)
    if pre:
        lib().conv2d_fwd_pre(x.y.data_ptr(), w_ohwi.data_ptr(), out.data_ptr(), n, h, wd, cin, cout, ksize, stride,
                             x.scale.data_ptr(), x.shift.data_ptr(), x.act, float(x.slope), ldy, _p(stats),
                             amax_x.data_ptr(), amax_w.data_ptr(), _s())
        return out, stats
    wsplit = None
    if cin != 4:
        amax_x = _amax_or_pass(x, amax_x); amax_w = _amax_or_pass(w_ohwi, amax_w)
        if w_split_ready is not None and amax_w is not None and _precision == "fp32":
            wsplit = w_split_ready
        elif amax_w is not None and _precision == "fp32":
            wsplit = scratch(w_ohwi.numel() + 16, x.device, slot=5)
    else:
        wsplit = scratch(27 * 32 + 16, x.device, slot=5)
    ready = int(wsplit is not None and wsplit is w_split_ready)
    if w_b16 is not None and cin != 4 and _precision == "bf16":
        wsplit, ready = w_b16, 2
    lib().conv2d_fwd(x.data_ptr(), w_ohwi.data_ptr(), out.data_ptr(), n, h, wd, cin, cout, ksize, stride,
                     _p(scale), _p(shift), act, float(slope), _p(residual),
                     0 if residual is None else residual.stride(2), ldy, _p(stats), int(accumulate), 0,
                     _p(amax_x), _p(amax_w), _p(amax_out), _p(wsplit), ready, _s())
    return out, stats


def conv2d_bwd_data(dy, w_ohwi, in_hw, ksize, stride, out=None, accumulate=False, amax_dy=None, amax_w=None, wt_ready=None,
                    wt_b16=None, tap=None):
    n, ho, wo, cout = dy.shape
    cin = w_ohwi.shape[3]
    h, wd = in_hw
    if out is None:
        out = torch.empty((n, h, wd, cin), dtype=torch.float32, device=dy.device)
    amax_dy = _amax_or_pass(dy, amax_dy); amax_w = _amax_or_pass(w_ohwi, amax_w)
    if wt_ready is not None:
        wt, wts = wt_ready
        if _precision != "fp32":
            wts = None
    else:
        wt, wts = scratch(w_ohwi.numel() + 16, dy.device, slot=1), None
    ready = int(wt_ready is not None)
    if wt_ready is not None and wt_b16 is not None and _precision == "bf16":
        wts, ready = wt_b16, 2
    if tap is not None:
        cap = lib().conv2d_bwd_data_tap_rows(n, h, wd, cin, cout, ksize, stride)
        part = torch.empty((max(cap, 1), 2, cin), dtype=torch.float32, device=dy.device)
        rows = ctypes.c_int(0)
        lib().conv2d_bwd_data_tap(dy.data_ptr(), dy.stride(2), w_ohwi.data_ptr(), wt.data_ptr(), out.data_ptr(),
                                  n, h, wd, cin, cout, ksize, stride, int(accumulate), 0, _p(amax_dy), _p(amax_w),
                                  ready, _p(wts), tap["y"].data_ptr() if cap else 0, tap["mean"].data_ptr(), tap["invstd"].data_ptr(),
                                  _p(tap.get("gamma")), _p(tap.get("beta")), int(tap["act"]), float(tap["slope"]),
                                  part.data_ptr() if cap else 0, cap, ctypes.addressof(rows), _s())
        return out, (part[:rows.value] if rows.value > 0 else None)
    lib().conv2d_bwd_data(dy.data_ptr(), dy.stride(2), w_ohwi.data_ptr(), wt.data_ptr(), out.data_ptr(),
                          n, h, wd, cin, cout, ksize, stride, int(accumulate), 0, _p(amax_dy), _p(amax_w),
                          ready, _p(wts), _s())
    return out


def _fwd_out_stats(name, x, cout, ksize, stride, out, out_f32, stats_rows):
    n, h, wd, _ = x.shape
    dtype = torch.float32 if out_f32 else torch.bfloat16
    if out is None:
        out = torch.empty((n, *conv_out_hw(h, wd, ksize, stride), cout), dtype=dtype, device=x.device)
    if out.dtype != dtype or out.stride(3) != 1:
        raise ValueError(f"{name}: out dtype / layout")
    stats = None
    if stats_rows is not None:
        stats = torch.empty((stats_rows(n, h, wd, cout, ksize, stride), 2, cout), dtype=torch.float32, device=x.device)
    return out, stats


def _bwd_data_tapped(fn, operands, out, out_f32, n, h, wd, cin, cout, ksize, stride, accumulate, tap, stats_rows):
    part = None
    rows = ctypes.c_int(0)
    cap = 0
    if tap is not None and stride == 1 and _b16(tap["y"]) and tap["y"].is_contiguous():
        cap = stats_rows(n, h, wd, cin, ksize, 1)
        part = torch.empty((max(cap, 1), 2, cin), dtype=torch.float32, device=out.device)
    fn(*operands, out.data_ptr(), int(out_f32), n, h, wd, cin, cout, ksize, stride, int(accumulate),
       tap["y"].data_ptr() if cap else 0, tap["mean"].data_ptr() if cap else 0, tap["invstd"].data_ptr() if cap else 0,
       _p(tap.get("gamma")) if cap else 0, _p(tap.get("beta")) if cap else 0, int(tap["act"]) if cap else 0, float(tap["slope"]) if cap else 0.0,
       part.data_ptr() if cap else 0, cap, ctypes.addressof(rows), _s())
    if tap is not None:
        return out, (part[:rows.value] if rows.value > 0 else None)
    return out


def conv2d_fwd_b16(x, w16, cout, ksize, stride, scale=None, shift=None, act=ACT_NONE, slope=0.0, residual=None, out=None,
                   want_stats=False, accumulate=False, out_f32=False):
    _chk16(x, "conv2d_fwd_b16 x")
    n, h, wd, cin = x.shape
    if not (w16.is_cuda and w16.dtype == torch.bfloat16 and w16.is_contiguous() and w16.numel() == cout * ksize * ksize * cin):
        raise ValueError("conv2d_fwd_b16: w16 must be the contiguous bf16 bank [Cout][k*k*Cin]")
    out, stats = _fwd_out_stats("conv2d_fwd_b16", x, cout, ksize, stride, out, out_f32, lib().conv2d_stats_rows_b16 if want_stats else None)
    if residual is not None:
        _rows16(residual, "conv2d_fwd_b16 residual")
        if not _b16(residual):
            raise ValueError("conv2d_fwd_b16: residual must be bf16")
    lib().conv2d_fwd_b16(x.data_ptr(), w16.data_ptr(), out.data_ptr(), int(out_f32), n, h, wd, cin, cout, ksize, stride, _p(scale), _p(shift),
                         act, float(slope), _p(residual), 0 if residual is None else residual.stride(2), out.stride(2), _p(stats),
                         int(accumulate), _s())
    return out, stats


def conv2d_bwd_data_b16(dy, wt16, in_hw, cin, ksize, stride, out=None, accumulate=False, tap=None, out_f32=False):
    n, ho, wo, cout = dy.shape
    h, wd = in_hw
    _rows16(dy, "conv2d_bwd_data_b16 dy")
    if not _b16(dy) or not (wt16.dtype == torch.bfloat16 and wt16.is_contiguous() and wt16.numel() == cin * ksize * ksize * cout):
        raise ValueError("conv2d_bwd_data_b16: dy must be bf16, wt16 the contiguous bf16 bank [Cin][k*k*Cout]")
    if out is None:
        out = torch.empty((n, h, wd, cin), dtype=torch.float32 if out_f32 else torch.bfloat16, device=dy.device)
    if out.dtype != (torch.float32 if out_f32 else torch.bfloat16) or not out.is_contiguous():
        raise ValueError("conv2d_bwd_data_b16: out dtype / layout")
    return _bwd_data_tapped(lib().conv2d_bwd_data_b16, (dy.data_ptr(), dy.stride(2), wt16.data_ptr()), out, out_f32, n, h, wd, cin, cout, ksize, stride,
                            accumulate, tap, lib().conv2d_stats_rows_b16)


def quant_rows_e4m3(x: torch.Tensor):
    _rows16(x, "quant_rows_e4m3 x")
    if not _b16(x):
        raise ValueError("quant_rows_e4m3: x must be bf16")
    c = x.shape[-1]
    rows = x.numel() // c
    q = torch.empty(x.shape, dtype=torch.uint8, device=x.device)
    sc = torch.empty(rows, dtype=torch.uint8, device=x.device)
    lib().quant_rows_e4m3(x.data_ptr(), x.stride(-2) if x.dim() > 1 else c, rows, c, q.data_ptr(), c, sc.data_ptr(), _s())
    return q, sc


def bank_q8(bank, key: str, b16: torch.Tensor, rows: int):
    q = bank.get(key) if isinstance(bank, dict) else None
    return q if q is not None else quant_rows_e4m3(b16.view(rows, -1))


def conv2d_fwd_f8(x8, xs, w8, ws, cout, ksize, stride, scale=None, shift=None, act=ACT_NONE, slope=0.0, residual=None, want_stats=False,
                  out_f32=False):
    n, h, wd, cin = x8.shape
    if not (x8.dtype == torch.uint8 and x8.is_contiguous() and w8.dtype == torch.uint8 and w8.is_contiguous() and w8.numel() == cout * ksize * ksize * cin
            and xs.dtype == torch.uint8 and xs.numel() == n * h * wd and ws.dtype == torch.uint8 and ws.numel() == cout):
        raise ValueError("conv2d_fwd_f8: x8 / w8 must be contiguous uint8 e4m3 tensors with one e8m0 byte per pixel / per filter")
    out, stats = _fwd_out_stats("conv2d_fwd_f8", x8, cout, ksize, stride, None, out_f32, lib().conv2d_stats_rows_f8 if want_stats else None)
    if residual is not None and not (_b16(residual) and residual.is_contiguous()):
        raise ValueError("conv2d_fwd_f8: residual must be a contiguous bf16 tensor")
    lib().conv2d_fwd_f8(x8.data_ptr(), xs.data_ptr(), w8.data_ptr(), ws.data_ptr(), out.data_ptr(), int(out_f32), n, h, wd, cin, cout, ksize, stride,
                        _p(scale), _p(shift), act, float(slope), _p(residual), 0, cout, _p(stats), 0, _s())
    return out, stats


def conv2d_bwd_data_f8(dy8, dys, wt8, wts, in_hw, cin, ksize, stride, out=None, accumulate=False, tap=None, out_f32=False):
    n, ho, wo, cout = dy8.shape
    h, wd = in_hw
    if not (dy8.dtype == torch.uint8 and dy8.is_contiguous() and wt8.dtype == torch.uint8 and wt8.is_contiguous()
            and wt8.numel() == cin * ksize * ksize * cout and dys.numel() == n * ho * wo and wts.numel() == cin):
        raise ValueError("conv2d_bwd_data_f8: dy8 / wt8 must be contiguous uint8 e4m3 tensors with one e8m0 byte per pixel / per bank row")
    if out is None:
        out = torch.empty((n, h, wd, cin), dtype=torch.float32 if out_f32 else torch.bfloat16, device=dy8.device)
    if out.dtype != (torch.float32 if out_f32 else torch.bfloat16) or not out.is_contiguous():
        raise ValueError("conv2d_bwd_data_f8: out dtype / layout")
    return _bwd_data_tapped(lib().conv2d_bwd_data_f8, (dy8.data_ptr(), dys.data_ptr(), wt8.data_ptr(), wts.data_ptr()), out, out_f32, n, h, wd, cin, cout,
                            ksize, stride, accumulate, tap, lib().conv2d_stats_rows_f8)


def conv2d_bwd_weight_b16(x, dy, ksize, stride, slot: int = 0):
    n, h, wd, cin = x.shape
    cout = dy.shape[3]
    _rows16(x, "conv2d_bwd_weight_b16 x"); _rows16(dy, "conv2d_bwd_weight_b16 dy")
    if not (_b16(x) and _b16(dy)):
        raise ValueError("conv2d_bwd_weight_b16: bf16 tensors only")
    dw = torch.empty((cout, ksize, ksize, cin), dtype=torch.float32, device=x.device)
    if STEP_ABL and _step_abl(1):
        return dw
    nws = lib().conv2d_bwd_weight_ws_b16(n, h, wd, cin, cout, ksize, stride)
    ws = scratch(nws, x.device, slot=slot) if nws > 0 else None
    cnt = slab_counters(x.device, slot) if nws > 0 else None
    geom = conv_geom(x.device, n, h, wd, ksize, stride)
    lib().conv2d_bwd_weight_b16(x.data_ptr(), x.stride(2), dy.data_ptr(), dy.stride(2), dw.data_ptr(), _p(ws), _p(cnt), geom.data_ptr(),
                                n, h, wd, cin, cout, ksize, stride, _s())
    return dw


FILTER_BANKS = True


class FilterBanks:

    def __init__(self, weights, device):
        import struct
        self.device = torch.device(device)
        self.items = {}
        pairs = weights.items() if isinstance(weights, dict) else enumerate(weights)
        ok = [(i, w) for i, w in pairs if w is not None and w.dim() == 4 and w.shape[0] % 32 == 0 and w.shape[1] % 32 == 0
              and w.is_cuda and w.dtype == torch.float32 and w.is_contiguous()]
        self.amax = torch.zeros(max(1, len(ok)) * AMAX_WORDS, dtype=torch.int32, device=self.device)
        rec = lib().filter_job_bytes()
        assert rec == 8 * 8 + 6 * 4, rec
        blob = bytearray()
        blk = ablk = 0
        self._ptrs = []
        for j, (i, w) in enumerate(ok):
            co, ci, kh, kw = w.shape
            T = kh * kw
            numel = w.numel()
            ohwi = torch.empty((co, kh, kw, ci), dtype=torch.float32, device=self.device) if T > 1 else None
            split = torch.empty(numel + 16, dtype=torch.float32, device=self.device)
            t = torch.empty(numel + 16, dtype=torch.float32, device=self.device)
            tsplit = torch.empty(numel + 16, dtype=torch.float32, device=self.device)
            am = self.amax[j * AMAX_WORDS:(j + 1) * AMAX_WORDS]
            b16 = torch.empty(numel, dtype=torch.bfloat16, device=self.device)
            tb16 = torch.empty(numel, dtype=torch.bfloat16, device=self.device)
            self.items[i] = dict(ohwi=ohwi, split=split, t=t, tsplit=tsplit, amax=am, b16=b16, tb16=tb16, shape=(co, ci, kh, kw))
            blob += struct.pack("<8Q6i", w.data_ptr(), 0 if ohwi is None else ohwi.data_ptr(), split.data_ptr(), t.data_ptr(),
                                tsplit.data_ptr(), am.data_ptr(), b16.data_ptr(), tb16.data_ptr(), co, ci, T, blk, ablk, 0)
            self._ptrs.append((i, w.data_ptr()))
            blk += T * (co // 32) * (ci // 32); ablk += (numel + 4095) // 4096
        self.njobs, self.blocks, self.ablocks = len(ok), blk, ablk
        self._q8_jobs = None; self._q8_key = None
        self.jobs = torch.frombuffer(blob, dtype=torch.uint8).clone().to(self.device) if ok else None

    def valid_for(self, weights) -> bool:
        return all(weights.get(i) is not None and weights[i].data_ptr() == ptr for i, ptr in self._ptrs) if isinstance(weights, dict) \
            else all(weights[i] is not None and weights[i].data_ptr() == ptr for i, ptr in self._ptrs)

    def refresh(self):
        if self.njobs:
            lib().prepare_filters(self.jobs.data_ptr(), self.njobs, self.blocks, self.ablocks, self.amax.data_ptr(),
                                  self.amax.numel(), _s())
            if storage_f8():
                self._refresh_q8()

    def _refresh_q8(self):
        import struct
        if self._q8_jobs is None or self._q8_key != F8_MIN_K:
            rec = lib().quant_job_bytes()
            assert rec == 3 * 8 + 4 * 4, rec
            blob = bytearray(); blk = 0; elems = 0; n = 0
            for it in self.items.values():
                co, ci, kh, kw = it["shape"]
                it.pop("q8", None); it.pop("tq8", None)
                for key, src, rows, ok in (("q8", it["b16"], co, f8_takes(ci, co, kh)), ("tq8", it["tb16"], ci, f8_takes(co, ci, kh))):
                    if not ok:
                        continue
                    c = src.numel() // rows
                    q = torch.empty((rows, c), dtype=torch.uint8, device=self.device)
                    sc = torch.empty(rows, dtype=torch.uint8, device=self.device)
                    it[key] = (q, sc)
                    blob += struct.pack("<3Q4i", src.data_ptr(), q.data_ptr(), sc.data_ptr(), rows, c, blk, 0)
                    blk += (rows + 3) // 4; elems += rows * c; n += 1
            self._q8_jobs = (torch.frombuffer(blob, dtype=torch.uint8).clone().to(self.device), n, blk, elems) if n else (None, 0, 0, 0)
            self._q8_key = F8_MIN_K
        jobs, n, blk, elems = self._q8_jobs
        if n:
            lib().quant_rows_e4m3_batched(jobs.data_ptr(), n, blk, elems, _s())

    def get(self, i, w):
        it = self.items.get(i)
        if it is None:
            return None
        if it["ohwi"] is None:
            co, ci, kh, kw = it["shape"]
            it = dict(it); it["ohwi"] = w.detach().view(co, 1, 1, ci)
        return it


_geom = {}


def conv_geom(device, n: int, h: int, wd: int, ksize: int, stride: int) -> torch.Tensor:
    key = (torch.device(device).index, n, h, wd, ksize, stride)
    t = _geom.get(key)
    if t is None:
        t = torch.empty(lib().conv2d_geom_size(n, h, wd, ksize, stride), dtype=torch.int32, device=device)
        lib().conv2d_geom(t.data_ptr(), n, h, wd, ksize, stride, _s())
        torch.cuda.current_stream().synchronize()
        _geom[key] = t
    return t


STEP_ABL = 0


def _step_abl(bit: int) -> bool:
    if not ablation_build():
        raise RuntimeError(f"ops.STEP_ABL = {STEP_ABL} makes results wrong by construction and is honoured only by an ablation build "
                           "of the library: DCN_EXTRA_FLAGS=-DDCN_ABL=1 python -m dcnet_amd.build")
    return bool(STEP_ABL & bit)


def conv2d_bwd_weight(x, dy, ksize, stride, cout=None, slot: int = 0, amax_x=None, amax_dy=None):
    if _b16(dy) and not isinstance(x, PreAct):
        return conv2d_bwd_weight_b16(x, dy, ksize, stride, slot=slot)
    n, h, wd, cin = x.shape
    cout = dy.shape[3] if cout is None else cout
    dw = torch.empty((cout, 64) if cin == 4 else (cout, ksize, ksize, cin), dtype=torch.float32, device=x.device)
    if STEP_ABL and _step_abl(1):
        return dw
    nws = lib().conv2d_bwd_weight_ws(n, h, wd, cin, cout, ksize, stride)
    ws = scratch(nws, x.device, slot=slot) if nws > 0 else None
    cnt = slab_counters(x.device, slot) if nws > 0 else None
    if isinstance(x, PreAct):
        if amax_x is None:
            raise DcnError("conv2d_bwd_weight: a PreAct input needs the abs-max word of the activation")
        amax_dy = _amax_or_pass(dy, amax_dy)
        lib().conv2d_bwd_weight_pre(x.y.data_ptr(), x.y.stride(2), dy.data_ptr(), dy.stride(2), dw.data_ptr(), _p(ws), _p(cnt),
                                    n, h, wd, cin, cout, ksize, stride, x.scale.data_ptr(), x.shift.data_ptr(), x.act, float(x.slope),
                                    amax_x.data_ptr(), amax_dy.data_ptr(), _s())
        return dw
    geom = conv_geom(x.device, n, h, wd, ksize, stride)
    if (cin >= 64 and cout >= 64 and (cin >= 128 or cout >= 128)) or (cin == 32 and cout == 64 and ksize == 3):
        amax_x = _amax_or_pass(x, amax_x); amax_dy = _amax_or_pass(dy, amax_dy)
    lib().conv2d_bwd_weight(x.data_ptr(), x.stride(2), dy.data_ptr(), dy.stride(2), dw.data_ptr(), _p(ws), _p(cnt), geom.data_ptr(),
                            n, h, wd, cin, cout, ksize, stride, _p(amax_x), _p(amax_dy), _s())
    return dw


_side = {}


def side_stream(device) -> "torch.cuda.Stream":
    key = (torch.device(device).index, torch.cuda.current_stream(device).cuda_stream, SIDE_PRIORITY)
    if key not in _side:
        if SIDE_PRIORITY:
            with torch.cuda.device(device):
                handle = lib().stream_create(SIDE_PRIORITY)
            if not handle:
                raise DcnError("dcn_stream_create failed")
            _side[key] = torch.cuda.ExternalStream(handle, device=device)
        else:
            _side[key] = torch.cuda.Stream(device=device)
    return _side[key]


SIDE_PRIORITY = 0
WGRAD_SIDE = True
WGRAD_AFTER_DGRAD = True


WGRAD_HELD = True


class HeldWgrad:

    def __init__(self, x, dy, ksize, stride, wshape, amax_x=None, amax_dy=None):
        self.args = (x, dy, ksize, stride, wshape, amax_x, amax_dy)
        self.main = torch.cuda.current_stream()
        self.side = side_stream(x.device)
        self.event = torch.cuda.Event()
        self.event.record(self.main)

    def issue(self):
        x, dy, ksize, stride, wshape, amax_x, amax_dy = self.args
        self.args = None
        self.side.wait_event(self.event)
        return _wgrad_side_launch(self.main, self.side, x, dy, ksize, stride, wshape, amax_x, amax_dy)


def _wgrad_oihw(x, dy, ksize, stride, wshape, slot, amax_x, amax_dy):
    dw = conv2d_bwd_weight(x, dy, ksize, stride, slot=slot, amax_x=amax_x, amax_dy=amax_dy)
    if wshape[0] != dw.shape[0]:
        dw = dw[:wshape[0]].contiguous()
    return weight_grad_to_oihw(dw, wshape)


def _wgrad_side_launch(main, side, x, dy, ksize, stride, wshape, amax_x, amax_dy):
    with torch.cuda.stream(side):
        out = _wgrad_oihw(x, dy, ksize, stride, wshape, 3, amax_x, amax_dy)
    for t in ((x.y, x.scale, x.shift) if isinstance(x, PreAct) else (x,)) + (dy,):
        t.record_stream(side)
    out.record_stream(main)
    return out


def wgrad_on_side(x, dy, ksize, stride, wshape, amax_x=None, amax_dy=None):
    if not WGRAD_SIDE:
        return _wgrad_oihw(x, dy, ksize, stride, wshape, 0, amax_x, amax_dy)
    main = torch.cuda.current_stream()
    side = side_stream(x.device)
    side.wait_stream(main)
    return _wgrad_side_launch(main, side, x, dy, ksize, stride, wshape, amax_x, amax_dy)


WGRAD_DIRECT = False
HEAD_WGRAD_DIRECT = True
_held_direct: list = []


def hold_wgrad_into(param, x, dy, ksize, stride, wshape, amax_x=None, amax_dy=None) -> None:
    _held_direct.append((HeldWgrad(x, dy, ksize, stride, wshape, amax_x=amax_x, amax_dy=amax_dy), param))


def reset_held_wgrads() -> None:
    _held_direct.clear()


def release_held_wgrads() -> None:
    while _held_direct:
        hw, param = _held_direct.pop(0)
        out = hw.issue()
        with torch.cuda.stream(hw.side):
            if param.grad is None:
                param.grad = out.view_as(param)
            else:
                param.grad.add_(out.view_as(param))


def finish_wgrads(device) -> None:
    release_held_wgrads()
    cur = torch.cuda.current_stream(device)
    idx = torch.device(device).index
    for key, st in _side.items():
        if key[0] == idx and st is not cur:
            cur.wait_stream(st)


def join_side(device) -> None:
    if WGRAD_SIDE:
        torch.cuda.current_stream().wait_stream(side_stream(device))


def bn_finalize(stats, count, gamma, beta, eps, momentum, running_mean, running_var):
    rows, _, c = stats.shape
    dev = stats.device
    res = torch.empty((4, c), dtype=torch.float32, device=dev)
    ws = scratch(lib().bn_ws(c), dev, slot=2)
    lib().bn_finalize(stats.data_ptr(), rows, c, int(count), _p(gamma), _p(beta), float(eps), float(momentum),
                      _p(running_mean), _p(running_var), res[0].data_ptr(), res[1].data_ptr(),
                      res[2].data_ptr(), res[3].data_ptr(), ws.data_ptr(), _s())
    return res


def bn_fold(gamma, beta, running_mean, running_var, eps=1e-5):
    c = gamma.numel()
    res = torch.empty((2, c), dtype=torch.float32, device=gamma.device)
    lib().bn_fold(gamma.data_ptr(), beta.data_ptr(), running_mean.data_ptr(), running_var.data_ptr(), float(eps), c,
                  res[0].data_ptr(), res[1].data_ptr(), _s())
    return res


def channel_stats(x2d):
    rows, c = x2d.shape
    r = lib().channel_stats_rows(rows)
    stats = torch.empty((r, 2, c), dtype=torch.float32, device=x2d.device)
    lib().channel_stats(x2d.data_ptr(), rows, c, c, stats.data_ptr(), _s())
    return stats


def quant_of(x: torch.Tensor):
    q = getattr(x, "_dcn_q8", None)
    return q if q is not None else quant_rows_e4m3(x)


def scale_act(y, scale, shift, act, slope, residual=None, out=None, amax_out=None, out_b16=False, out_f32=False, quant=False):
    c = y.shape[-1]
    rows = y.numel() // c
    if quant and _b16(y) and out is None and not out_f32 and y.is_contiguous() and lib().quant_fusable(c) and (residual is None or _b16(residual)):
        out = torch.empty(y.shape, dtype=torch.bfloat16, device=y.device)
        q8 = torch.empty(y.shape, dtype=torch.uint8, device=y.device)
        qs = torch.empty(rows, dtype=torch.uint8, device=y.device)
        if residual is not None:
            _rows16(residual, "scale_act residual")
        lib().scale_act_b16_q(y.data_ptr(), _p(scale), _p(shift), act, float(slope), _p(residual), 0 if residual is None else residual.stride(-2),
                              out.data_ptr(), rows, c, q8.data_ptr(), qs.data_ptr(), _s())
        out._dcn_q8 = (q8, qs)
        return out
    if _b16(y) or out_b16 or _b16(out):
        if out is None:
            out = torch.empty(y.shape, dtype=torch.float32 if out_f32 else torch.bfloat16, device=y.device)
        if not y.is_contiguous() or (residual is not None and not _b16(residual)):
            raise ValueError("scale_act (bf16 storage): contiguous y, bf16 residual")
        _rows16(out, "scale_act out")
        if residual is not None:
            _rows16(residual, "scale_act residual")
        lib().scale_act_b16(y.data_ptr(), int(not _b16(y)), _p(scale), _p(shift), act, float(slope), _p(residual),
                            0 if residual is None else residual.stride(-2), out.data_ptr(), int(not _b16(out)), rows, c, out.stride(-2), _s())
        return out
    if out is None:
        out = torch.empty_like(y)
    _chk(y, "scale_act y"); _rows(out, "scale_act out")
    lib().scale_act(y.data_ptr(), _p(scale), _p(shift), act, float(slope), _p(residual), out.data_ptr(), rows, c,
                    out.stride(-2), _p(amax_out), _s())
    return out


def _bn_bwd_partials(y, dout, mean, invstd, gamma, beta, act, slope, part):
    c = y.shape[-1]
    rows = y.numel() // c
    if part is not None:
        return part, part.shape[0]
    if _b16(dout) or _b16(y):
        r = lib().bn_act_bwd_reduce_rows_b16(rows)
        part = scratch(r * 2 * c, y.device, slot=0)
        lib().bn_act_bwd_reduce_b16(y.data_ptr(), int(not _b16(y)), dout.data_ptr(), int(not _b16(dout)), dout.stride(-2), mean.data_ptr(), invstd.data_ptr(),
                                    _p(gamma), _p(beta), act, float(slope), rows, c, part.data_ptr(), _s())
        return part, r
    r = lib().channel_stats_rows(rows)
    part = scratch(r * 2 * c, y.device, slot=0)
    lib().bn_act_bwd_reduce(y.data_ptr(), dout.data_ptr(), dout.stride(-2), mean.data_ptr(), invstd.data_ptr(), _p(gamma), _p(beta),
                            act, float(slope), rows, c, part.data_ptr(), _s())
    return part, r


def bn_act_bwd(y, dout, mean, invstd, gamma, beta, act, slope, amax_out=None, part=None, quant=False):
    c = y.shape[-1]
    rows = y.numel() // c
    dev = y.device
    lddo = dout.stride(-2)
    part, r = _bn_bwd_partials(y, dout, mean, invstd, gamma, beta, act, slope, part)
    sums = torch.empty((2, c), dtype=torch.float32, device=dev)
    ws = scratch(lib().bn_ws(c), dev, slot=2)
    lib().bn_bwd_sums(part.data_ptr(), r, c, sums.data_ptr(), ws.data_ptr(), _s())
    if _b16(dout) or _b16(y):
        dy = torch.empty(y.shape, dtype=torch.bfloat16, device=dev)
        if quant and _b16(y) and _b16(dout) and lib().quant_fusable(c):
            q8 = torch.empty(y.shape, dtype=torch.uint8, device=dev)
            qs = torch.empty(rows, dtype=torch.uint8, device=dev)
            lib().bn_act_bwd_apply_b16_q(y.data_ptr(), dout.data_ptr(), lddo, mean.data_ptr(), invstd.data_ptr(), _p(gamma), _p(beta), act, float(slope),
                                         sums.data_ptr(), rows, rows, c, dy.data_ptr(), q8.data_ptr(), qs.data_ptr(), _s())
            dy._dcn_q8 = (q8, qs)
            return dy, sums[1], sums[0]
        lib().bn_act_bwd_apply_b16(y.data_ptr(), int(not _b16(y)), dout.data_ptr(), int(not _b16(dout)), lddo, mean.data_ptr(), invstd.data_ptr(), _p(gamma),
                                   _p(beta), act, float(slope), sums.data_ptr(), rows, rows, c, dy.data_ptr(), _s())
        return dy, sums[1], sums[0]
    dy = torch.empty_like(y)
    lib().bn_act_bwd_apply(y.data_ptr(), dout.data_ptr(), lddo, mean.data_ptr(), invstd.data_ptr(), _p(gamma), _p(beta),
                           act, float(slope), sums.data_ptr(), rows, rows, c, dy.data_ptr(), _p(amax_out), _s())
    return dy, sums[1], sums[0]


def stem_bwd_weight_bn(x, y, dout, mean, invstd, gamma, beta, act, slope, part=None):
    n, h, wd, c = y.shape
    rows = n * h * wd
    dev = y.device
    lddo = dout.stride(-2)
    part, r = _bn_bwd_partials(y, dout, mean, invstd, gamma, beta, act, slope, part)
    sums = torch.empty((2, c), dtype=torch.float32, device=dev)
    ws = scratch(lib().bn_ws(c), dev, slot=2)
    lib().bn_bwd_sums(part.data_ptr(), r, c, sums.data_ptr(), ws.data_ptr(), _s())
    dw = torch.empty((c, 64), dtype=torch.float32, device=dev)
    slabs = scratch(lib().stem_bwd_weight_bn_ws(n, h, wd), dev, slot=0)
    fn = lib().stem_bwd_weight_bn_b16 if _b16(dout) else lib().stem_bwd_weight_bn
    fn(x.data_ptr(), y.data_ptr(), dout.data_ptr(), lddo, mean.data_ptr(), invstd.data_ptr(), _p(gamma), _p(beta),
       act, float(slope), sums.data_ptr(), rows, n, h, wd, c, dw.data_ptr(), slabs.data_ptr(), _s())
    return dw, sums[1], sums[0]


_nbt = None


def bump_batches(bn) -> None:
    if _nbt is not None:
        _nbt.append(bn.num_batches_tracked)
    else:
        bn.num_batches_tracked += 1


def batches_begin() -> None:
    global _nbt
    _nbt = []


def batches_end() -> None:
    global _nbt
    pend, _nbt = _nbt, None
    if pend:
# ... 819 lines not shown
```

### include/dcnet_hip.h

```cpp
#ifndef DCNET_HIP_H
#define DCNET_HIP_H

#include <stdint.h>

#ifdef __cplusplus
extern "C" {
#endif

#define DCN_OK 0
#define DCN_ERR_ARG (-1)
#define DCN_ERR_LAUNCH (-2)

#define DCN_AMAX_WORDS 64
#define DCN_SLAB_COUNTERS 4096

#define DCN_ACT_NONE 0
#define DCN_ACT_LEAKY 1

#define DCN_ABI_VERSION 317

const char* dcn_last_error(void);
int dcn_version(void);

int dcn_nchw_to_nhwc(const float* src, float* dst, int n, int c, int h, int w, int c_pad, void* stream);
int dcn_nhwc_to_nchw(const float* src, float* dst, int n, int c, int h, int w, int ld, void* stream);
int dcn_oihw_to_ohwi(const float* src, float* dst, int co, int ci, int kh, int kw, int ci_pad, void* stream);
int dcn_ohwi_to_oihw(const float* src, float* dst, int co, int ci, int kh, int kw, int ci_pad, void* stream);

int dcn_conv2d_fwd(const float* x, const float* w, float* y,
                   int n, int h, int wd, int cin, int cout, int ksize, int stride,
                   const float* scale, const float* shift, int act, float slope,
                   const float* residual, int ldr, int ldy,
                   float* stats, int accumulate, const float* f8_scales,
                   const uint32_t* amax_x, const uint32_t* amax_w, uint32_t* amax_y, float* w_split, int w_split_ready,
                   void* stream);
int dcn_absmax(const float* x, int64_t rows, int c, int ld, uint32_t* amax, void* stream);
int dcn_conv2d_stats_rows(int n, int h, int wd, int cout, int ksize, int stride);
int dcn_conv1_tile(int64_t rows, int cout, int ntaps, int cin, int stats, int storage);
int dcn_l2norm_score_fwd_form(int c);
int dcn_bn_apply_form(int c, int params_aligned);
int dcn_igemm_split_build(int kind, int ksteps);
int dcn_gemm3_variant(void);
int dcn_f8_scale(const float* x, int64_t rows, int c, int ld, float* scale, void* ws, void* stream);

int dcn_conv2d_bwd_data(const float* dy, int lddy, const float* w, float* wt, float* dx,
                        int n, int h, int wd, int cin, int cout, int ksize, int stride,
                        int accumulate, const float* f8_scales, const uint32_t* amax_dy, const uint32_t* amax_w,
                        int wt_ready, const float* wt_split, void* stream);
int dcn_conv2d_bwd_data_tap(const float* dy, int lddy, const float* w, float* wt, float* dx,
                            int n, int h, int wd, int cin, int cout, int ksize, int stride,
                            int accumulate, const float* f8_scales, const uint32_t* amax_dy, const uint32_t* amax_w,
                            int wt_ready, const float* wt_split,
                            const float* tap_y, const float* tap_mean, const float* tap_invstd, const float* tap_gamma,
                            const float* tap_beta, int tap_act, float tap_slope, float* tap_stats, int tap_stats_rows,
                            int* tap_rows, void* stream);
int dcn_conv2d_bwd_data_tap_rows(int n, int h, int wd, int cin, int cout, int ksize, int stride);
int dcn_conv2d_pre_supported(int n, int h, int wd, int cin, int cout, int ksize, int stride);
int dcn_conv2d_fwd_pre(const float* x, const float* w, float* y, int n, int h, int wd, int cin, int cout, int ksize, int stride,
                       const float* pre_scale, const float* pre_shift, int pre_act, float pre_slope,
                       int ldy, float* stats, const uint32_t* amax_x, const uint32_t* amax_w, void* stream);
int dcn_conv2d_bwd_weight_pre_supported(int n, int h, int wd, int cin, int cout, int ksize, int stride);
int dcn_conv2d_bwd_weight_pre(const float* x, int ldx, const float* dy, int lddy, float* dw, float* ws, uint32_t* counters,
                              int n, int h, int wd, int cin, int cout, int ksize, int stride,
                              const float* pre_scale, const float* pre_shift, int pre_act, float pre_slope,
                              const uint32_t* amax_x, const uint32_t* amax_dy, void* stream);
int dcn_filter_job_bytes(void);
int dcn_prepare_filters(const void* jobs, int njobs, int total_blocks, int total_amax_blocks,
                        uint32_t* amax_all, int64_t amax_words, void* stream);

int64_t dcn_conv2d_geom_size(int n, int h, int wd, int ksize, int stride);
int dcn_conv2d_geom(uint32_t* table, int n, int h, int wd, int ksize, int stride, void* stream);

int dcn_conv2d_bwd_weight(const float* x, int ldx, const float* dy, int lddy, float* dw, float* ws, uint32_t* counters,
                          const uint32_t* geom,
                          int n, int h, int wd, int cin, int cout, int ksize, int stride,
                          const uint32_t* amax_x, const uint32_t* amax_dy, void* stream);
int64_t dcn_conv2d_bwd_weight_ws(int n, int h, int wd, int cin, int cout, int ksize, int stride);
int dcn_stem_bwd_weight_bn(const float* x, const float* y, const float* dout, int lddo,
                           const float* mean, const float* invstd, const float* gamma, const float* beta,
                           int act, float slope, const float* sums, int64_t count,
                           int n, int h, int wd, int cout, float* dw, float* ws, void* stream);
int64_t dcn_stem_bwd_weight_bn_ws(int n, int h, int wd);
int dcn_stem_bwd_weight_bn_b16(const float* x, const float* y, const void* dout16, int lddo,
                               const float* mean, const float* invstd, const float* gamma, const float* beta,
                               int act, float slope, const float* sums, int64_t count,
                               int n, int h, int wd, int cout, float* dw, float* ws, void* stream);

int dcn_gemm3_supported(int m, int n, int k, int batch);
int dcn_gemm3_presplit(const float* src, int ld, int64_t bs, float* dst, int ldd, int64_t bsd, int batch, int rows, int c,
                       const uint32_t* amax, void* stream);
int dcn_gemm3(const float* a, int lda, int64_t a_bs, int a_t, const float* b, int ldb, int64_t b_bs, int b_t,
              float* c, int ldc, int64_t c_bs, const float* row_scale, int64_t rs_bs,
              int m, int n, int k, int batch, int accumulate, const uint32_t* amax_a, const uint32_t* amax_b, void* stream);

int64_t dcn_bn_ws(int c);
int dcn_bn_finalize(const float* stats, int rows, int c, int64_t count,
                    const float* gamma, const float* beta, float eps, float momentum,
                    float* running_mean, float* running_var,
                    float* mean, float* invstd, float* scale, float* shift, float* ws, void* stream);
int dcn_bn_fold(const float* gamma, const float* beta, const float* running_mean, const float* running_var,
                float eps, int c, float* scale, float* shift, void* stream);
int dcn_channel_stats(const float* x, int64_t rows, int c, int ld, float* stats, void* stream);
int dcn_channel_stats_rows(int64_t rows);
int dcn_scale_act(const float* y, const float* scale, const float* shift, int act, float slope,
                  const float* residual, float* out, int64_t rows, int c, int ldo, uint32_t* amax, void* stream);
int dcn_bn_act_amax_bound(const uint32_t* amax_y, const float* scale, const float* shift, int c, float slope,
                          uint32_t* amax_out, void* stream);
int dcn_bn_act_bwd_reduce(const float* y, const float* dout, int lddo, const float* mean, const float* invstd,
                          const float* gamma, const float* beta, int act, float slope,
                          int64_t rows, int c, float* stats, void* stream);
int dcn_bn_bwd_sums(const float* stats, int rows, int c, float* sums, float* ws, void* stream);
int dcn_bn_act_bwd_apply(const float* y, const float* dout, int lddo, const float* mean, const float* invstd,
                         const float* gamma, const float* beta, int act, float slope,
                         const float* sums, int64_t count, int64_t rows, int c, float* dy, uint32_t* amax, void* stream);
int dcn_act_bwd(const float* out, const float* dout, int lddo, float slope, int64_t rows, int c, float* dy, void* stream);
int dcn_frozen_bn_act_bwd(const float* a, const float* dout, int lddo, const float* scale, const float* gamma, const float* beta,
                          int act, float slope, int64_t rows, int c, int want_sums, float* dy, float* stats, uint32_t* amax, void* stream);

int64_t dcn_coattn_e_size(int b, int hw);
int64_t dcn_coattn_saved_size(int b, int hw, int c);
int64_t dcn_coattn_fwd_ws(int b, int hw, int c);
int dcn_coattn_fwd(const float* f1, const float* f2, int ldf, int64_t bsf, float* f1_attn, float* f2_attn, int ldo,
                   int64_t bso, float* E, float* rinv, float* cinv, float* ws,
                   int b, int hw, int c, float temperature, void* stream);
int64_t dcn_coattn_bwd_ws(int b, int hw, int c);
int dcn_coattn_bwd(const float* f1, const float* f2, int ldf, int64_t bsf,
                   const float* d_f1_attn, const float* d_f2_attn, int lddo, int64_t bsdo,
                   const float* f1_attn, const float* f2_attn, int ldo, int64_t bso,
                   const float* E, const float* rinv, const float* cinv,
                   float* d_f1, float* d_f2, int lddf, int64_t bsdf, int accumulate, float* ws,
                   int b, int hw, int c, float temperature, void* stream);

int dcn_l2norm_score_fwd(const float* x, int ldx, float* out, int ldo, float* norm,
                         const float* q, float* score, float* score_flip, int64_t rows, int rows_per_image, int c,
                         float out_scale, int accumulate, void* stream);
int dcn_l2norm_score_bwd(const float* out, int ldo, const float* norm, const float* dout, int lddo,
                         const float* q, const float* dscore, const float* dscore_flip, float* dx, int lddx, float* dq,
                         int64_t rows, int rows_per_image, int c, void* stream);
int dcn_rowdot_fwd(const float* x, int ldx, const float* q, int flip, float* score, int64_t rows, int rows_per_image, int c,
                   void* stream);
int dcn_rowdot_bwd(const float* x, int ldx, const float* q, int flip, const float* dscore, float* dx, int lddx, float* dq,
                   int64_t rows, int rows_per_image, int c, void* stream);

int dcn_phrase_attn_fwd(const float* context, const float* embedded, const int64_t* ids,
                        const float* w0, const float* b0, const float* w1, const float* b1,
                        float* attn, float* out, float* vnorm, int n, int l, int d, int e, int normalize, void* stream);
int64_t dcn_phrase_attn_bwd_ws(int n, int d, int heads);
int dcn_phrase_attn_bwd(const float* context, const float* embedded, const float* w0, const float* w1,
                        const float* attn, const float* out, const float* vnorm, const float* dout,
                        float* dcontext, float* dembedded, float* dw, float* ws,
                        int n, int l, int d, int e, int normalize, void* stream);
int dcn_colsum(const float* in, int ld, int rows, int cols, float* out, void* stream);

int dcn_locemb_fwd(const float* coord, const float* w, const float* b, const float* gamma, const float* beta,
                   float* running_mean, float* running_var, float momentum, float eps, int training, int64_t count,
                   int p, float* e8, float* xhat, float* stat, double* mom, void* stream);
int dcn_locemb_bwd(const float* coord, const float* w, const float* gamma, const float* beta, const float* xhat,
                   const float* stat, const float* de_a, const float* de_b, const double* dmom, int training, int p,
                   float* grads, void* stream);
int dcn_head_obj(const float* const* logits, const int* ld, const float* const* sim, const int* hw, const float* e8,
                 float* const* only_obj, float* obj_map, float* objn, float* x, int b, void* stream);
int dcn_pad_rows(const float* src, int lds, float* dst, int ldd, int rows, int cols, int cols_out, void* stream);
int dcn_locbn_fwd(const float* m, const double* mom, const float* bias, const float* gamma, const float* beta,
                  float* running_mean, float* running_var, float momentum, float eps, int training, int batch,
                  int64_t count, int c, float* mp, float* bp, float* saved, void* stream);
int dcn_locbn_bwd(const float* m, const double* mom, const float* bias, const float* gamma, const float* running_mean,
                  const float* saved, const float* dmp, int64_t dmp_bs, const float* dbp, int training, int batch,
                  int64_t count, int c, float* dm, float* out, double* dmom, void* stream);
int dcn_head_final_fwd(const float* const* logits, const int* ld, const float* const* sim, const int* hw,
                       const float* loc_map, float* const* outbox, float* const* loc_score, float* minmax, int b, void* stream);
int dcn_head_dloc(const float* const* logits, const int* ld, const float* const* sim, const int* hw,
                  const float* const* loc_score, const float* const* d_outbox, const float* const* d_loc,
                  const float* minmax, float* dloc_map, int b, void* stream);
int dcn_head_fold(const float* dx, const float* e8, const float* obj_map, int b, int p, int ppad, float* dobj_map,
                  float* de8, void* stream);
int dcn_head_dlogits(const float* const* logits, const int* ld, const float* const* sim, const int* hw,
                     const float* const* loc_score, const float* const* only_obj, const float* const* d_outbox,
                     const float* const* d_only, const float* obj_map, const float* objn, const float* dobj_map,
                     float* const* dlogits, float* const* dsim, int b, void* stream);

int dcn_k9_fwd(const float* cmap, const float* fv, const int64_t* raw_neg, int pairs, int hw, int e, int top_k, int neg_n,
               int64_t* index, int64_t* neg_idx, float* frame, float* corr, float* negf, void* stream);
int dcn_k9_bwd(const int64_t* index, const int64_t* neg_idx, const float* d_frame, const float* d_corr, const float* d_neg,
               int pairs, int hw, int e, int top_k, int neg_n, float* dfv, void* stream);
int dcn_colnorm_fwd(const float* v, int n, int hw, int e, float* vit, float* cnorm, void* stream);
int dcn_colnorm_bwd(const float* vit, const float* cnorm, const float* dq, const float* extra, int n_extra,
                    int n, int hw, int e, float* dv, void* stream);
int dcn_lagnorm_fwd(const float* context, int n, int l, int d, float* lag, float* lnorm, void* stream);
int dcn_crossmap(const float* lag, const float* vit, const float* conv_w, const float* conv_b, int n, int l, int hw, int e,
                 int64_t* cols, float* lvmap, void* stream);
int dcn_k14_gather(const float* lag, const float* vit, const int64_t* cols, const int64_t* neg, int n, int l, int hw, int e,
                   int neg_n, float* lag_pos, float* neg_cross, void* stream);
int dcn_k14_negscatter(const float* d_neg, const int* csr_off, const int* csr_src, int hw, int e, float* extra, void* stream);
int dcn_k14_dlag(const float* lag, const float* lnorm, const int64_t* cols, const float* d_k, int n, int l, int hw, int e,
                 float* dcontext, void* stream);

int dcn_build_target(const float* bbox, const float* anchors, int size, int n, int* target_i, float* target_f, void* stream);
int dcn_target_dense(const int* target_i, const float* target_f, int size, int n, float* const* bbox_list,
                     float* const* center_list, void* stream);
int dcn_dense_loss_fwd(const float* const* outbox, const float* const* sim, const float* const* negsim, const float* const* loc,
                       const int* target_i, const float* target_f, int size, int n, float* vals, float* lse, float* out,
                       void* stream);
int dcn_dense_loss_bwd(const float* const* outbox, const float* const* sim, const float* const* negsim, const float* const* loc,
                       const int* target_i, const float* target_f, const float* lse, const float* grad_out, int size, int n,
                       float* const* d_outbox, float* const* d_sim, float* const* d_negsim, float* const* d_loc, void* stream);
int dcn_contrastive_fwd(const float* q, const float* pos, const float* neg, int64_t rows, int e, int m, float temperature,
                        float* loss_rows, float* loss, void* stream);
int dcn_contrastive_bwd(const float* q, const float* pos, const float* neg, int64_t rows, int e, int m, float temperature,
                        const float* grad_out, float* dq, float* dpos, float* dneg, void* stream);
int dcn_decode_boxes(const float* const* outbox, const float* anchors, int size, int n, float* boxes, int* cellinfo, void* stream);
int dcn_box_iou(const float* box1, const float* box2, int n, float* iou, void* stream);

int dcn_conv2d_stats_rows_b16(int n, int h, int wd, int cout, int ksize, int stride);
int dcn_conv2d_fwd_b16(const void* x, const void* w16, void* y, int y_f32, int n, int h, int wd, int cin, int cout, int ksize, int stride,
                       const float* scale, const float* shift, int act, float slope, const void* residual, int ldr, int ldy,
                       float* stats, int accumulate, void* stream);
int dcn_conv2d_bwd_data_b16(const void* dy, int lddy, const void* wt16, void* dx, int dx_f32, int n, int h, int wd, int cin, int cout,
                            int ksize, int stride, int accumulate, const void* tap_y, const float* tap_mean, const float* tap_invstd,
                            const float* tap_gamma, const float* tap_beta, int tap_act, float tap_slope, float* tap_stats,
                            int tap_stats_rows, int* tap_rows, void* stream);
int64_t dcn_conv2d_bwd_weight_ws_b16(int n, int h, int wd, int cin, int cout, int ksize, int stride);
int dcn_conv2d_bwd_weight_b16(const void* x, int ldx, const void* dy, int lddy, float* dw, float* ws, uint32_t* counters, const uint32_t* geom,
                              int n, int h, int wd, int cin, int cout, int ksize, int stride, void* stream);
int dcn_scale_act_b16(const void* y, int y_f32, const float* scale, const float* shift, int act, float slope, const void* residual,
                      int ldr, void* out, int out_f32, int64_t rows, int c, int ldo, void* stream);
int dcn_bn_act_bwd_reduce_rows_b16(int64_t rows);
int dcn_bn_act_bwd_reduce_b16(const void* y, int y_f32, const void* dout, int dout_f32, int lddo, const float* mean, const float* invstd,
                              const float* gamma, const float* beta, int act, float slope, int64_t rows, int c, float* stats,
                              void* stream);
int dcn_bn_act_bwd_apply_b16(const void* y, int y_f32, const void* dout, int dout_f32, int lddo, const float* mean, const float* invstd,
                             const float* gamma, const float* beta, int act, float slope, const float* sums, int64_t count,
                             int64_t rows, int c, void* dy, void* stream);
int dcn_frozen_bn_act_bwd_b16(const void* a, const void* dout, int dout_f32, int lddo, const float* scale, const float* gamma,
                              const float* beta, int act, float slope, int64_t rows, int c, int want_sums, void* dy, float* stats,
                              void* stream);
int dcn_cast_rows(const void* src, int src_b16, int lds, void* dst, int dst_b16, int ldd, int64_t rows, int c, int accumulate,
                  void* stream);
int dcn_upsample2_nhwc_b16(const void* src, int lds, void* dst, int ldd, int n, int h, int w, int c, void* stream);
int dcn_upsample2_nhwc_bwd_b16(const void* ddst, int ldd, void* dsrc, int lds, int n, int h, int w, int c, int accumulate,
                               void* stream);

int dcn_quant_rows_e4m3(const void* x, int ld, int64_t rows, int c, void* q, int ldq, void* scales, void* stream);
int dcn_quant_job_bytes(void);
int dcn_quant_rows_e4m3_batched(const void* jobs, int njobs, int blocks, int64_t elements, void* stream);
int dcn_quant_fusable(int c);
int dcn_scale_act_b16_q(const void* y, const float* scale, const float* shift, int act, float slope, const void* residual, int ldr, void* out,
                        int64_t rows, int c, void* q8, void* qs, void* stream);
int dcn_bn_act_bwd_apply_b16_q(const void* y, const void* dout, int lddo, const float* mean, const float* invstd, const float* gamma,
                               const float* beta, int act, float slope, const float* sums, int64_t count, int64_t rows, int c, void* dy,
                               void* q8, void* qs, void* stream);
int dcn_conv2d_stats_rows_f8(int n, int h, int wd, int cout, int ksize, int stride);
int dcn_conv2d_fwd_f8(const void* x8, const void* xs, const void* w8, const void* ws, void* y, int y_f32, int n, int h, int wd, int cin, int cout,
                      int ksize, int stride, const float* scale, const float* shift, int act, float slope, const void* residual, int ldr,
                      int ldy, float* stats, int accumulate, void* stream);
int dcn_conv2d_bwd_data_f8(const void* dy8, const void* dys, const void* wt8, const void* wts, void* dx, int dx_f32, int n, int h, int wd, int cin,
                           int cout, int ksize, int stride, int accumulate, const void* tap_y, const float* tap_mean, const float* tap_invstd,
                           const float* tap_gamma, const float* tap_beta, int tap_act, float tap_slope, float* tap_stats, int tap_stats_rows,
                           int* tap_rows, void* stream);

int dcn_post_topk(const float* const* outbox, const float* const* feat, const int64_t* feat_strides, const int* grids,
                  const float* anchors, int size, int n, int e, int top_k, const float* ratio, const float* dw, const float* dh,
                  const int64_t* frame_hw, float* boxes, float* scores, float* feats, int64_t* cells, void* stream);
int dcn_post_fusion(const float* center, const float* ref, const float* ref_score, const unsigned char* valid, int n, int k, int r,
                    int e, float* fused, int64_t* best, void* stream);

int dcn_bank_write(const float* x, int ldx, float* bank, float* split, int64_t rows, int c, void* stream);
int dcn_coattn_bank_fwd(const float* f1, const float* f2, const float* f1s, const float* f2s, int64_t bsf, float* f1_attn,
                        float* f2_attn, int ldo, int64_t bso, float* E, float* rinv, float* cinv, float* ws, int b, int hw, int c,
                        float temperature, void* stream);
int dcn_post_fusion_bank(const float* feats, const float* scores, int n, int k, int r, int e, float* fused, int64_t* best,
                         void* stream);
int dcn_bank_write_b16(const float* x, int ldx, void* rows16, float* bank, float* split, int64_t rows, int c, void* stream);
int dcn_bank_concat_b16(const void* rows16, int64_t bs16, const float* attn, int ld_attn, int64_t bs_attn, void* cat, int n, int hw,
                        int c, void* stream);
int dcn_coattn_bank_form(int hw, int c);

typedef struct DcnPrepJob {
  int64_t src_off;
  int32_t h, w;
  int32_t rh, rw;
  int32_t top, left;
  int32_t flip;
  int32_t hsv;
  float a_v;
  int32_t warp;
  double minv[6];
} DcnPrepJob;
int64_t dcn_clip_prep_ws(int n, int size);
int dcn_clip_prep(const uint8_t* src, int64_t src_bytes, const DcnPrepJob* jobs, const DcnPrepJob* jobs_host, int n, int size,
                  uint8_t* ws, float* out, uint8_t* u8_out, void* stream);

int dcn_locmod_fwd(const float* E, const float* Mp, const float* bp, const float* q, float* loc,
                   int n, int p, int c, void* stream);
int64_t dcn_locmod_bwd_ws(int n, int p);
int dcn_locmod_bwd(const float* E, const float* Mp, const float* bp, const float* q, const float* dloc,
                   float* dE_part, float* dsum, float* ws, int n, int p, int c, void* stream);

int dcn_gemm_nt(const float* A, int lda, const float* B, int ldb, float* C, int ldc, int M, int N, int K,
                const float* bias, int act, const float* residual, int ldr, int accumulate, void* stream);
int dcn_gemm_nn(const float* A, int lda, const float* B, int ldb, float* C, int ldc, int M, int N, int K, int kvalid,
                int accumulate, void* stream);
int dcn_gemm_tn(const float* A, int lda, const float* B, int ldb, float* C, int ldc, int M, int N, int K,
                int accumulate, void* stream);
int dcn_lstm_cell_fwd(const float* gates, const float* c_prev, const float* h_prev, const int64_t* lens, int t,
                      float* act, float* c_out, float* h_out, float* y, int ldy, int n, int hidden, void* stream);
int dcn_lstm_cell_bwd(const float* dy, int lddy, const float* dh_rec, const float* dc_next, const float* act,
                      const float* c_prev, const int64_t* lens, int t, float* dgates, int ldg, float* dc_prev,
                      float* dh_pass, int n, int hidden, void* stream);

int64_t dcn_bilstm_sync_bytes(void);
int dcn_bilstm_fwd(const float* xg, const float* whh_fwd, const float* whh_rev, const float* bhh_fwd, const float* bhh_rev,
                   const int64_t* lens, float* out, float* hprev, float* cprev, float* acts, void* sync,
                   int n, int l, int hidden, void* stream);
int dcn_bilstm_bwd(const float* dout, const float* whh_fwd, const float* whh_rev, const float* acts, const float* cprev,
                   const int64_t* lens, float* dxg, void* sync, int n, int l, int hidden, void* stream);

int dcn_upsample2_nhwc(const float* src, int lds, float* dst, int ldd, int n, int h, int w, int c, void* stream);
int dcn_upsample2_nhwc_bwd(const float* ddst, int ldd, float* dsrc, int lds, int n, int h, int w, int c,
                           int accumulate, void* stream);
int dcn_copy_slice(const float* src, int lds, float* dst, int ldd, int64_t rows, int c, int accumulate, void* stream);

int dcn_set_tuning(const char* key, int value);
int dcn_tuning_info(int index, const char** name, int* value, int* def, const char** desc, int* ablation);

int dcn_rmsprop_step(float* const* params, const float* const* grads, float* const* square_avgs, const int64_t* numel,
                     int count, float lr, const float* lr_dev ,
                     float alpha, float eps, float weight_decay, void* stream);
int dcn_adam_prepare(int* const* steps, float* const* scal, int count, float lr, const float* lr_dev, double beta1, double beta2, void* stream);
int dcn_adam_step(float* const* params, const float* const* grads, float* const* exp_avgs, float* const* exp_avg_sqs,
                  const float* const* scal, const int64_t* numel, int count, double beta1, double beta2, float eps, float weight_decay,
                  void* stream);
int dcn_sgd_step(float* const* params, const float* const* grads, float* const* momentum_bufs, const int64_t* numel, int count,
                 float lr, const float* lr_dev, float momentum, float weight_decay, void* stream);
int64_t dcn_grad_sumsq_slots(const int64_t* numel, int count);
int dcn_grad_sumsq(const float* const* grads, const int64_t* numel, int count, double* partials, int64_t slots, void* stream);
int dcn_grad_clip_coef(const double* partials, int64_t slots, float max_norm, int skip_nonfinite, void* ctrl, void* stream);
int dcn_grad_scale(float* const* grads, const int64_t* numel, int count, const void* ctrl, void* stream);
int dcn_rmsprop_step_clipped(float* const* params, const float* const* grads, float* const* square_avgs, const int64_t* numel,
                             int count, float lr, const float* lr_dev, float alpha, float eps, float weight_decay, const void* ctrl,
                             void* stream);
int dcn_adam_prepare_clipped(int* const* steps, float* const* scal, int count, float lr, const float* lr_dev, double beta1, double beta2,
                             const void* ctrl, void* stream);
int dcn_adam_step_clipped(float* const* params, const float* const* grads, float* const* exp_avgs, float* const* exp_avg_sqs,
                          const float* const* scal, const int64_t* numel, int count, double beta1, double beta2, float eps,
                          float weight_decay, const void* ctrl, void* stream);
int dcn_sgd_step_clipped(float* const* params, const float* const* grads, float* const* momentum_bufs, const int64_t* numel, int count,
                         float lr, const float* lr_dev, float momentum, float weight_decay, const void* ctrl, void* stream);
int dcn_adamw_prepare(int* const* steps, float* const* scal, int count, float lr, const float* lr_dev, double beta1, double beta2,
                      double weight_decay, void* stream);
int dcn_adamw_step(float* const* params, const float* const* grads, float* const* exp_avgs, float* const* exp_avg_sqs,
                   const float* const* scal, const int64_t* numel, int count, double beta1, double beta2, float eps, void* stream);
int dcn_adamw_prepare_clipped(int* const* steps, float* const* scal, int count, float lr, const float* lr_dev, double beta1, double beta2,
                              double weight_decay, const void* ctrl, void* stream);
int dcn_adamw_step_clipped(float* const* params, const float* const* grads, float* const* exp_avgs, float* const* exp_avg_sqs,
                           const float* const* scal, const int64_t* numel, int count, double beta1, double beta2, float eps,
                           const void* ctrl, void* stream);
int dcn_ema_prepare(int* step, float* w, double decay, double tau, const void* ctrl, void* stream);
int dcn_ema_update(float* const* shadow, const float* const* src, const int64_t* numel, int count, const float* w, const void* ctrl,
                   void* stream);
int dcn_tensor_swap(float* const* a, float* const* b, const int64_t* numel, int count, void* stream);

int dcn_fusion_prefill(const float* A, const float* coord, const float* w3, int ldw, float* out, int n, int hw, int co, void* stream);
int64_t dcn_fusion_bwd_ws(int n, int co);
int dcn_fusion_bwd(const float* dy, const float* coord, const float* flang, float* ws, float* d_img, float* dw2, float* dw3,
                   int ldd, int n, int hw, int co, int e, void* stream);
int dcn_row_lengths(const int64_t* ids, int n, int L, int64_t* out, void* stream);
int dcn_embedding_fwd(const int64_t* ids, const float* table, float* out, int tokens, int e, int vocab, void* stream);
int dcn_embedding_bwd(const int64_t* ids, const float* dout, float* dtable, int tokens, int e, int vocab, void* stream);

void* dcn_stream_create(int level);
int dcn_stream_destroy(void* stream);
// ... 22 lines not shown
```

Before: 86.67 clips/s.

## Flatten optimizer grids into fixed units and prepare only needed filter forms

The fused optimizer kernels now launch a 1D grid of fixed-size work units (4 float4 trips per thread) spread over all tensors in a chunk, instead of a 2D grid sized by the largest tensor. Each block finds its tensor by prefix count and issues all loads before computing. This removes idle blocks on small tensors. Separately, the filter-bank transform processes all taps of a 32x32 tile per block and takes a form mask, so only the weight layouts the current precision mode reads are written, with lazy fill on first access to others. The cost is more shared memory per block and added Python-side bookkeeping that could re-trigger prepares.

```diff
diff --git a/dcnet_amd/csrc/optim.hip b/dcnet_amd/csrc/optim.hip
--- a/dcnet_amd/csrc/optim.hip
+++ b/dcnet_amd/csrc/optim.hip
@@ -3,20 +3,26 @@
 namespace {
 
 constexpr int RMS_CHUNK = 32;
-template <int K> struct Chunk { float* t[K][RMS_CHUNK]; long long n[RMS_CHUNK]; };
+constexpr int WALK_TRIPS = 4;
+constexpr int WALK_UNIT = 256 * 4 * WALK_TRIPS;
+template <int K> struct Chunk { float* t[K][RMS_CHUNK]; long long n[RMS_CHUNK]; int u[RMS_CHUNK]; };
+
+template <int K>
+__device__ __forceinline__ int unit_tensor(const Chunk<K>& c) {
+  int t = 0;
+#pragma unroll
+  for (int i = 1; i < RMS_CHUNK; ++i) t += c.u[i] <= (int)blockIdx.x ? 1 : 0;
+  return t;
+}
 
 template <int W, bool READ, class F>
-__device__ __forceinline__ void walk(float* const (&w)[W], const float* __restrict__ g, const long long n, F f) {
+__device__ __forceinline__ void walk(float* const (&w)[W], const float* __restrict__ g, const long long n, const long long unit, F f) {
   uintptr_t bits = READ ? (uintptr_t)g : 0;
 #pragma unroll
   for (int k = 0; k < W; ++k) bits |= (uintptr_t)w[k];
   const long long n4 = (bits & 15) == 0 ? n / 4 : 0;
-  const long long stride = (long long)gridDim.x * 256;
-  for (long long i = (long long)blockIdx.x * 256 + threadIdx.x; i < n4; i += stride) {
-    f32x4 x[W];
-#pragma unroll
-    for (int k = 0; k < W; ++k) x[k] = reinterpret_cast<const f32x4*>(w[k])[i];
-    const f32x4 gg = READ ? reinterpret_cast<const f32x4*>(g)[i] : f32x4{};
+  const long long e0 = unit * WALK_UNIT, e1 = e0 + WALK_UNIT < n ? e0 + WALK_UNIT : n;
+  const auto f4 = [&](f32x4 (&x)[W], const f32x4 gg) {
 #pragma unroll
     for (int e = 0; e < 4; ++e) {
       float a[W];
@@ -26,10 +32,34 @@
 #pragma unroll
       for (int k = 0; k < W; ++k) x[k][e] = a[k];
     }
+  };
+  long long i = e0 / 4 + threadIdx.x;
+  if (e0 / 4 + WALK_UNIT / 4 <= n4) {
+    f32x4 x[WALK_TRIPS][W], gg[WALK_TRIPS];
+#pragma unroll
+    for (int d = 0; d < WALK_TRIPS; ++d) {
+#pragma unroll
+      for (int k = 0; k < W; ++k) x[d][k] = reinterpret_cast<const f32x4*>(w[k])[i + d * 256];
+      gg[d] = READ ? reinterpret_cast<const f32x4*>(g)[i + d * 256] : f32x4{};
+    }
+    __builtin_amdgcn_sched_barrier(0);
+#pragma unroll
+    for (int d = 0; d < WALK_TRIPS; ++d) f4(x[d], gg[d]);
+#pragma unroll
+    for (int d = 0; d < WALK_TRIPS; ++d)
+#pragma unroll
+      for (int k = 0; k < W; ++k) reinterpret_cast<f32x4*>(w[k])[i + d * 256] = x[d][k];
+    return;
+  }
+  for (; i < n4; i += 256) {
+    f32x4 x[W];
+#pragma unroll
+    for (int k = 0; k < W; ++k) x[k] = reinterpret_cast<const f32x4*>(w[k])[i];
+    f4(x, READ ? reinterpret_cast<const f32x4*>(g)[i] : f32x4{});
 #pragma unroll
     for (int k = 0; k < W; ++k) reinterpret_cast<f32x4*>(w[k])[i] = x[k];
   }
-  for (long long i = n4 * 4 + (long long)blockIdx.x * 256 + threadIdx.x; i < n; i += stride) {
+  for (i = (e0 > n4 * 4 ? e0 : n4 * 4) + threadIdx.x; i < e1; i += 256) {
     float a[W];
 #pragma unroll
     for (int k = 0; k < W; ++k) a[k] = w[k][i];
@@ -53,26 +83,25 @@
 }
 
 template <bool CLIP, int NS, int K, class F>
-__device__ __forceinline__ void update_walk(const Chunk<K>& c, const float* __restrict__ ctl, F f) {
+__device__ __forceinline__ void update_walk(const Chunk<K>& c, const int t, const float* __restrict__ ctl, F f) {
   static_assert(K >= 2 + NS, "parameter, gradient and NS state tables");
   float coef = 1.f;
   if (CLIP) {
     if (reinterpret_cast<const int*>(ctl)[CTL_APPLY] == 0) return;
     coef = ctl[CTL_COEF];
   }
-  const int t = blockIdx.y;
   float* w[1 + NS];
   w[0] = c.t[0][t];
 #pragma unroll
   for (int k = 0; k < NS; ++k) w[1 + k] = c.t[2 + k][t];
-  walk<1 + NS, true>(w, c.t[1][t], c.n[t], [=](float (&a)[1 + NS], const float g0) { f(a, CLIP ? clip_mul(g0, coef) : g0); });
+  walk<1 + NS, true>(w, c.t[1][t], c.n[t], (int)blockIdx.x - c.u[t], [=](float (&a)[1 + NS], const float g0) { f(a, CLIP ? clip_mul(g0, coef) : g0); });
 }
 
 template <bool CLIP>
 __device__ __forceinline__ void rmsprop_body(const Chunk<3>& c, float lr, const float* __restrict__ lr_dev, float alpha, float eps, float wd,
                                              const float* __restrict__ ctl) {
   if (lr_dev) lr = lr_dev[0];
-  update_walk<CLIP, 1>(c, ctl, [=](float (&a)[2], const float g) { rms_update(a[0], g, a[1], lr, alpha, eps, wd); });
+  update_walk<CLIP, 1>(c, unit_tensor(c), ctl, [=](float (&a)[2], const float g) { rms_update(a[0], g, a[1], lr, alpha, eps, wd); });
 }
 
 __global__ __launch_bounds__(256) void rmsprop_kernel(const Chunk<3> c, float lr, const float* __restrict__ lr_dev, float alpha, float eps, float wd) {
@@ -138,9 +167,10 @@
 
 template <bool CLIP, bool DECOUPLED = false>
 __device__ __forceinline__ void adam_body(const Chunk<5>& c, float w1, float beta2, float w2, float eps, float wd, const float* __restrict__ ctl) {
-  const float* __restrict__ s = c.t[4][blockIdx.y];
+  const int t = unit_tensor(c);
+  const float* __restrict__ s = c.t[4][t];
   const float step_size = s[0], inv_bc2_sqrt = s[1], decay = DECOUPLED ? s[2] : 1.f;
-  update_walk<CLIP, 2>(c, ctl, [=](float (&a)[3], const float g) {
+  update_walk<CLIP, 2>(c, t, ctl, [=](float (&a)[3], const float g) {
     if (DECOUPLED) adamw_update(a[0], g, a[1], a[2], step_size, inv_bc2_sqrt, decay, w1, beta2, w2, eps);
     else adam_update(a[0], g, a[1], a[2], step_size, inv_bc2_sqrt, w1, beta2, w2, eps, wd);
   });
@@ -171,7 +201,7 @@
 template <bool CLIP>
 __device__ __forceinline__ void sgd_body(const Chunk<3>& c, float lr, const float* __restrict__ lr_dev, float mu, float wd, const float* __restrict__ ctl) {
   if (lr_dev) lr = lr_dev[0];
-  update_walk<CLIP, 1>(c, ctl, [=](float (&a)[2], const float g) { sgd_update(a[0], g, a[1], lr, mu, wd); });
+  update_walk<CLIP, 1>(c, unit_tensor(c), ctl, [=](float (&a)[2], const float g) { sgd_update(a[0], g, a[1], lr, mu, wd); });
 }
 
 __global__ __launch_bounds__(256) void sgd_kernel(const Chunk<3> c, float lr, const float* __restrict__ lr_dev, float mu, float wd) {
@@ -323,8 +353,9 @@
 
 __global__ __launch_bounds__(256) void grad_scale_kernel(const Chunk<1> c, const float* __restrict__ ctl) {
   const float coef = ctl[CTL_COEF];
-  float* const w[1] = {c.t[0][blockIdx.y]};
-  walk<1, false>(w, nullptr, c.n[blockIdx.y], [=](float (&a)[1], float) { a[0] = clip_mul(a[0], coef); });
+  const int t = unit_tensor(c);
+  float* const w[1] = {c.t[0][t]};
+  walk<1, false>(w, nullptr, c.n[t], (int)blockIdx.x - c.u[t], [=](float (&a)[1], float) { a[0] = clip_mul(a[0], coef); });
 }
 
 inline unsigned blocks_for(long long biggest) {
@@ -368,13 +399,25 @@
   return DCN_OK;
 }
 
+enum GridKind { GRID_TENSORS, GRID_UNITS };
 template <int K, class L>
-int launch_chunks(const char* who, Tables<K> tab, const int64_t* numel, int count, bool empties, L launch) {
+int launch_chunks(const char* who, Tables<K> tab, const int64_t* numel, int count, GridKind kind, bool empties, L launch) {
   return for_chunks(count, RMS_CHUNK, [&](int base, int m) -> int {
     Chunk<K> c{};
-    for (int i = 0; i < m; ++i) {
+    long long units = 0;
+    for (int i = 0; i < RMS_CHUNK; ++i) {
+      c.u[i] = (int)units;
+      if (i >= m) continue;
       for (int j = 0; j < K; ++j) c.t[j][i] = const_cast<float*>(tab[j][base + i]);
       c.n[i] = numel[base + i];
+      units += (numel[base + i] + WALK_UNIT - 1) / WALK_UNIT;
+      DCN_CHECK_ARG(units <= 0x7fffffffLL, "%s: tensors %d .. %d are too large for one launch", who, base, base + i);
+    }
+    if (kind == GRID_UNITS) {
+      if (units == 0) return DCN_OK;
+      launch(c, dim3((unsigned)units));
+      DCN_CHECK_LAUNCH(who);
+      return DCN_OK;
     }
     const long long biggest = longest(numel + base, m);
     if (empties && biggest == 0) return DCN_OK;
@@ -401,7 +444,7 @@
   DCN_CHECK_ARG(slots == sumsq_slots(numel, count), "grad_sumsq: the partials buffer has %lld slots, these tensors need %lld (dcn_grad_sumsq_slots)",
                 (long long)slots, sumsq_slots(numel, count));
   long long at = 0;
-  return launch_chunks<1>("grad_sumsq", {grads}, numel, count, false, [&](const Chunk<1>& c, dim3 grid) {
+  return launch_chunks<1>("grad_sumsq", {grads}, numel, count, GRID_TENSORS, false, [&](const Chunk<1>& c, dim3 grid) {
     OPTIM_LAUNCH(grad_sumsq_kernel, c, partials + at);
     at += (long long)grid.x * grid.y;
   });
@@ -419,7 +462,7 @@
 extern "C" int dcn_grad_scale(float* const* grads, const int64_t* numel, int count, const void* ctrl, void* stream) {
   DCN_CHECK_ARG(grads && numel && ctrl && count > 0, "grad_scale: bad argument");
   if (const int e = check_tensors<1>("grad_scale", {grads}, numel, count)) return e;
-  return launch_chunks<1>("grad_scale", {grads}, numel, count, false,
+  return launch_chunks<1>("grad_scale", {grads}, numel, count, GRID_UNITS, false,
                           [&](const Chunk<1>& c, dim3 grid) { OPTIM_LAUNCH(grad_scale_kernel, c, (const float*)ctrl); });
 }
 
@@ -427,7 +470,7 @@
                         int count, float lr, const float* lr_dev, float alpha, float eps, float weight_decay, const float* ctl, void* stream) {
   DCN_CHECK_ARG(params && grads && square_avgs && numel && count > 0, "%s: bad argument", who);
   if (const int e = check_tensors<3>(who, {params, grads, square_avgs}, numel, count)) return e;
-  return launch_chunks<3>(who, {params, grads, square_avgs}, numel, count, false, [&](const Chunk<3>& c, dim3 grid) {
+  return launch_chunks<3>(who, {params, grads, square_avgs}, numel, count, GRID_UNITS, false, [&](const Chunk<3>& c, dim3 grid) {
     if (ctl) OPTIM_LAUNCH(rmsprop_clip_kernel, c, lr, lr_dev, alpha, eps, weight_decay, ctl);
     else OPTIM_LAUNCH(rmsprop_kernel, c, lr, lr_dev, alpha, eps, weight_decay);
   });
@@ -495,7 +538,7 @@
   else DCN_CHECK_ARG(eps >= 0.f && weight_decay >= 0.f, "%s: negative eps or weight_decay", who);
   if (const int e = check_tensors<5>(who, {params, grads, exp_avgs, exp_avg_sqs, scal}, numel, count)) return e;
   const float w1 = (float)(1.0 - beta1), b2 = (float)beta2, w2 = (float)(1.0 - beta2);
-  return launch_chunks<5>(who, {params, grads, exp_avgs, exp_avg_sqs, scal}, numel, count, false, [&](const Chunk<5>& c, dim3 grid) {
+  return launch_chunks<5>(who, {params, grads, exp_avgs, exp_avg_sqs, scal}, numel, count, GRID_UNITS, false, [&](const Chunk<5>& c, dim3 grid) {
     if (decoupled && ctl) OPTIM_LAUNCH(adamw_clip_kernel, c, w1, b2, w2, eps, ctl);
     else if (decoupled) OPTIM_LAUNCH(adamw_kernel, c, w1, b2, w2, eps);
     else if (ctl) OPTIM_LAUNCH(adam_clip_kernel, c, w1, b2, w2, eps, weight_decay, ctl);
@@ -535,7 +578,7 @@
   DCN_CHECK_ARG(params && grads && momentum_bufs && numel && count > 0, "%s: bad argument", who);
   DCN_CHECK_ARG(momentum >= 0.f && weight_decay >= 0.f, "%s: negative momentum or weight_decay", who);
   if (const int e = check_tensors<3>(who, {params, grads, momentum_bufs}, numel, count)) return e;
-  return launch_chunks<3>(who, {params, grads, momentum_bufs}, numel, count, false, [&](const Chunk<3>& c, dim3 grid) {
+  return launch_chunks<3>(who, {params, grads, momentum_bufs}, numel, count, GRID_UNITS, false, [&](const Chunk<3>& c, dim3 grid) {
     if (ctl) OPTIM_LAUNCH(sgd_clip_kernel, c, lr, lr_dev, momentum, weight_decay, ctl);
     else OPTIM_LAUNCH(sgd_kernel, c, lr, lr_dev, momentum, weight_decay);
   });
@@ -565,12 +608,12 @@
                               void* stream) {
   DCN_CHECK_ARG(count >= 0 && w && (count == 0 || (shadow && src && numel)), "ema_update: bad argument");
   if (const int e = check_tensors<2>("ema_update", {shadow, src}, numel, count, true)) return e;
-  return launch_chunks<2>("ema_update", {shadow, src}, numel, count, true,
+  return launch_chunks<2>("ema_update", {shadow, src}, numel, count, GRID_TENSORS, true,
                           [&](const Chunk<2>& c, dim3 grid) { OPTIM_LAUNCH(ema_update_kernel, c, w, (const int*)ctrl); });
 }
 
 extern "C" int dcn_tensor_swap(float* const* a, float* const* b, const int64_t* numel, int count, void* stream) {
   DCN_CHECK_ARG(count >= 0 && (count == 0 || (a && b && numel)), "tensor_swap: bad argument");
   if (const int e = check_tensors<2>("tensor_swap", {a, b}, numel, count, true)) return e;
-  return launch_chunks<2>("tensor_swap", {a, b}, numel, count, true, [&](const Chunk<2>& c, dim3 grid) { OPTIM_LAUNCH(tensor_swap_kernel, c); });
-}
+  return launch_chunks<2>("tensor_swap", {a, b}, numel, count, GRID_TENSORS, true, [&](const Chunk<2>& c, dim3 grid) { OPTIM_LAUNCH(tensor_swap_kernel, c); });
+}
diff --git a/dcnet_amd/csrc/wprep.hip b/dcnet_amd/csrc/wprep.hip
--- a/dcnet_amd/csrc/wprep.hip
+++ b/dcnet_amd/csrc/wprep.hip
@@ -67,57 +67,91 @@
   *reinterpret_cast<f16x8_t*>(dst + 4) = l;
 }
 
-__global__ __launch_bounds__(256) void filters_xform_kernel(const FilterJob* __restrict__ jobs, int njobs) {
-  __shared__ float tile[32][33];
+enum { FORM_OHWI = 1, FORM_SPLIT = 2, FORM_T = 4, FORM_TSPLIT = 8, FORM_B16 = 16, FORM_TB16 = 32, FORM_KEEP_AMAX = 64 };
+constexpr int XF_TAPS = 9;
+
+__global__ __launch_bounds__(256) void filters_xform_kernel(const FilterJob* __restrict__ jobs, int njobs, int forms) {
+  __shared__ float tile[XF_TAPS][32][33];
   const int j = find_job(jobs, njobs, blockIdx.x, false);
-  const FilterJob job = jobs[j];
-  const int tci = job.ci / 32, tco = job.co / 32;
-  int b = blockIdx.x - job.blk0;
-  const int ci0 = (b % tci) * 32; b /= tci;
-  const int co0 = (b % tco) * 32; b /= tco;
-  const int tap = b;
+  FilterJob job = jobs[j];
+  if (!(forms & FORM_OHWI)) job.ohwi = nullptr;
+  if (!(forms & FORM_SPLIT)) job.ohwi_split = nullptr;
+  if (!(forms & FORM_T)) job.t = nullptr;
+  if (!(forms & FORM_TSPLIT)) job.t_split = nullptr;
+  if (!(forms & FORM_B16)) job.ohwi_b16 = nullptr;
+  if (!(forms & FORM_TB16)) job.t_b16 = nullptr;
+  const int T = job.T, tci = job.ci / 32;
+  const int b = blockIdx.x - job.blk0;
+  const int ci0 = (b % tci) * 32, co0 = (b / tci) * 32;
   const float s = scale_of(amax_read(job.amax));
   const long long numel = (long long)job.co * job.ci * job.T;
-  const int r = threadIdx.x >> 3, c4 = (threadIdx.x & 7) * 4;
-  {
-    const float* sp = job.src + ((long long)(co0 + r) * job.ci + ci0 + c4) * job.T + tap;
+  const int tid = threadIdx.x;
+  const int run4 = 8 * T;
+  for (int t0 = 0; t0 < T; t0 += XF_TAPS) {
+    const int tt = T - t0 < XF_TAPS ? T - t0 : XF_TAPS;
+    if (t0) __syncthreads();
+    for (int k0 = 0; k0 < T; k0 += XF_TAPS) {
+      f32x4 v[XF_TAPS];
+      int rr[XF_TAPS], qq[XF_TAPS];
 #pragma unroll
-    for (int e = 0; e < 4; ++e) tile[r][c4 + e] = sp[(long long)e * job.T];
-  }
-  __syncthreads();
-  if (job.ohwi) {
-    const f32x4 v = {tile[r][c4], tile[r][c4 + 1], tile[r][c4 + 2], tile[r][c4 + 3]};
-    *reinterpret_cast<f32x4*>(job.ohwi + ((long long)(co0 + r) * job.T + tap) * job.ci + ci0 + c4) = v;
-  }
-  if (job.t) {
-    const f32x4 v = {tile[c4][r], tile[c4 + 1][r], tile[c4 + 2][r], tile[c4 + 3][r]};
-    *reinterpret_cast<f32x4*>(job.t + ((long long)(ci0 + r) * job.T + tap) * job.co + co0 + c4) = v;
-  }
-  if (threadIdx.x < 128) {
-    const int rr = threadIdx.x >> 2, g = (threadIdx.x & 3) * 8;
-    float v[8];
-    typedef __bf16 bf16x8_t __attribute__((ext_vector_type(8)));
-    if (job.ohwi_b16) {
-      bf16x8_t b;
+      for (int k = 0; k < XF_TAPS; ++k)
+        if (k0 + k < T) {
+          const int idx = (k0 + k) * 256 + tid;
+          rr[k] = idx / run4; qq[k] = idx - rr[k] * run4;
+          v[k] = *reinterpret_cast<const f32x4*>(job.src + ((long long)(co0 + rr[k]) * job.ci + ci0) * T + 4 * qq[k]);
+        }
 #pragma unroll
-      for (int e = 0; e < 8; ++e) b[e] = (__bf16)tile[rr][g + e];
-      *reinterpret_cast<bf16x8_t*>(reinterpret_cast<__bf16*>(job.ohwi_b16) + ((long long)(co0 + rr) * job.T + tap) * job.ci + ci0 + g) = b;
+      for (int k = 0; k < XF_TAPS; ++k)
+        if (k0 + k < T) {
+#pragma unroll
+          for (int e = 0; e < 4; ++e) {
+            const int c = (4 * qq[k] + e) / T, tp = 4 * qq[k] + e - c * T - t0;
+            if (tp >= 0 && tp < tt) tile[tp][rr[k]][c] = v[k][e];
+          }
+        }
     }
-    if (job.t_b16) {
-      bf16x8_t b;
+    __syncthreads();
+    {
+      const int r = tid >> 3, c4 = (tid & 7) * 4;
+      for (int tp = 0; tp < tt; ++tp) {
+        const int tap = t0 + tp;
+        if (job.ohwi) {
+          const f32x4 v = {tile[tp][r][c4], tile[tp][r][c4 + 1], tile[tp][r][c4 + 2], tile[tp][r][c4 + 3]};
+          *reinterpret_cast<f32x4*>(job.ohwi + ((long long)(co0 + r) * T + tap) * job.ci + ci0 + c4) = v;
+        }
+        if (job.t) {
+          const f32x4 v = {tile[tp][c4][r], tile[tp][c4 + 1][r], tile[tp][c4 + 2][r], tile[tp][c4 + 3][r]};
+          *reinterpret_cast<f32x4*>(job.t + ((long long)(ci0 + r) * T + tap) * job.co + co0 + c4) = v;
+        }
+      }
+    }
+    for (int item = tid; item < tt * 128; item += 256) {
+      const int tp = item >> 7, tap = t0 + tp;
+      const int rr = (item & 127) >> 2, g = (item & 3) * 8;
+      float v[8];
+      typedef __bf16 bf16x8_t __attribute__((ext_vector_type(8)));
+      if (job.ohwi_b16) {
+        bf16x8_t b;
 #pragma unroll
-      for (int e = 0; e < 8; ++e) b[e] = (__bf16)tile[g + e][rr];
-      *reinterpret_cast<bf16x8_t*>(reinterpret_cast<__bf16*>(job.t_b16) + ((long long)(ci0 + rr) * job.T + tap) * job.co + co0 + g) = b;
-    }
-    if (job.ohwi_split) {
+        for (int e = 0; e < 8; ++e) b[e] = (__bf16)tile[tp][rr][g + e];
+        *reinterpret_cast<bf16x8_t*>(reinterpret_cast<__bf16*>(job.ohwi_b16) + ((long long)(co0 + rr) * T + tap) * job.ci + ci0 + g) = b;
+      }
+      if (job.t_b16) {
+        bf16x8_t b;
 #pragma unroll
-      for (int e = 0; e < 8; ++e) v[e] = tile[rr][g + e];
-      split_store8(job.ohwi_split + ((long long)(co0 + rr) * job.T + tap) * job.ci + ci0 + g, v, s);
-    }
-    if (job.t_split) {
+        for (int e = 0; e < 8; ++e) b[e] = (__bf16)tile[tp][g + e][rr];
+        *reinterpret_cast<bf16x8_t*>(reinterpret_cast<__bf16*>(job.t_b16) + ((long long)(ci0 + rr) * T + tap) * job.co + co0 + g) = b;
+      }
+      if (job.ohwi_split) {
 #pragma unroll
-      for (int e = 0; e < 8; ++e) v[e] = tile[g + e][rr];
-      split_store8(job.t_split + ((long long)(ci0 + rr) * job.T + tap) * job.co + co0 + g, v, s);
+        for (int e = 0; e < 8; ++e) v[e] = tile[tp][rr][g + e];
+        split_store8(job.ohwi_split + ((long long)(co0 + rr) * T + tap) * job.ci + ci0 + g, v, s);
+      }
+      if (job.t_split) {
+#pragma unroll
+        for (int e = 0; e < 8; ++e) v[e] = tile[tp][g + e][rr];
+        split_store8(job.t_split + ((long long)(ci0 + rr) * T + tap) * job.co + co0 + g, v, s);
+      }
     }
   }
   if (blockIdx.x == job.blk0 && threadIdx.x == 0) {
@@ -131,13 +165,16 @@
 extern "C" int dcn_filter_job_bytes(void) { return (int)sizeof(FilterJob); }
 
 extern "C" int dcn_prepare_filters(const void* jobs, int njobs, int total_blocks, int total_amax_blocks,
-                                   uint32_t* amax_all, int64_t amax_words, void* stream_) {
+                                   uint32_t* amax_all, int64_t amax_words, int forms, void* stream_) {
   hipStream_t stream = (hipStream_t)stream_;
   DCN_CHECK_ARG(jobs && njobs > 0 && total_blocks > 0 && total_amax_blocks > 0 && amax_all && amax_words > 0, "prepare_filters: bad argument");
-  if (hipMemsetAsync(amax_all, 0, (size_t)amax_words * 4, stream) != hipSuccess) { dcn_set_error("prepare_filters: memset failed"); return DCN_ERR_LAUNCH; }
-  hipLaunchKernelGGL(filters_amax_kernel, dim3(total_amax_blocks), dim3(256), 0, stream, (const FilterJob*)jobs, njobs);
-  DCN_CHECK_LAUNCH("filters_amax");
-  hipLaunchKernelGGL(filters_xform_kernel, dim3(total_blocks), dim3(256), 0, stream, (const FilterJob*)jobs, njobs);
+  DCN_CHECK_ARG(forms > 0 && forms < 128 && (forms & ~FORM_KEEP_AMAX), "prepare_filters: forms %d names no form (DCN_FORM_*)", forms);
+  if (!(forms & FORM_KEEP_AMAX)) {
+    if (hipMemsetAsync(amax_all, 0, (size_t)amax_words * 4, stream) != hipSuccess) { dcn_set_error("prepare_filters: memset failed"); return DCN_ERR_LAUNCH; }
+    hipLaunchKernelGGL(filters_amax_kernel, dim3(total_amax_blocks), dim3(256), 0, stream, (const FilterJob*)jobs, njobs);
+    DCN_CHECK_LAUNCH("filters_amax");
+  }
+  hipLaunchKernelGGL(filters_xform_kernel, dim3(total_blocks), dim3(256), 0, stream, (const FilterJob*)jobs, njobs, forms);
   DCN_CHECK_LAUNCH("filters_xform");
   return DCN_OK;
 }
diff --git a/dcnet_amd/darknet.py b/dcnet_amd/darknet.py
--- a/dcnet_amd/darknet.py
+++ b/dcnet_amd/darknet.py
@@ -297,7 +297,7 @@
                 torch.cuda.current_stream().wait_stream(banks.pending)
                 banks.pending = None
             if bank is not None:
-                w, aw, wsp, w16 = bank["ohwi"], (bank["amax"] if am else None), bank["split"], bank["b16"]
+                w, aw, wsp, w16 = bank["ohwi"], (bank["amax"] if am else None), ops.bank_form(bank, "split"), ops.bank_form(bank, "b16")
             else:
                 w = ops.weight_to_ohwi(p["w"]); wsp = w16 = None
                 aw = ops.absmax(p["w"]) if (am and op.cin > 4) else None
@@ -467,7 +467,7 @@
                                                P[prev.slot]["beta"], ops.ACT_LEAKY if prev.leaky else ops.ACT_NONE, 0.1)
                 fb = rec.bank
                 dx, part = convblock.conv_dgrad(dy, x.shape, op.k, op.stride, w=rec.w, bank=fb, out=cur, accumulate=cur is not None, tap=tap,
-                                                amax_dy=ady, amax_w=rec.aw, wt_ready=fb and (fb["t"], fb["tsplit"]), wt_b16=fb and fb["tb16"])
+                                                amax_dy=ady, amax_w=rec.aw, wt_ready=fb and (fb["t"], ops.bank_form(fb, "tsplit")), wt_b16=fb and ops.bank_form(fb, "tb16"))
                 if part is not None:
                     tapped[prev.slot] = part
                 if cur is None:
diff --git a/dcnet_amd/functions.py b/dcnet_amd/functions.py
--- a/dcnet_amd/functions.py
+++ b/dcnet_amd/functions.py
@@ -24,7 +24,7 @@
             x = ops.to_b16(x.contiguous())
         else:
             if bank is not None:
-                w, wsp = bank["ohwi"], bank["split"]
+                w, wsp = bank["ohwi"], ops.bank_form(bank, "split")
                 aw = bank["amax"] if am else None
             else:
                 w = ops.weight_to_ohwi(weight, ci_pad=x.shape[3])
@@ -77,7 +77,7 @@
             if not ctx.needs_input_grad[0]:
                 return None
             return convblock.conv_dgrad(dy, x.shape, ksize, 1, w=w, bank=bank, out_f32=ctx.x_f32, amax_dy=ady, amax_w=aw,
-                                        wt_ready=bank and (bank["t"], bank["tsplit"]))[0]
+                                        wt_ready=bank and (bank["t"], ops.bank_form(bank, "tsplit")))[0]
 
         dx, dwt = convblock.schedule_wgrad(x, dy, ksize, 1, wshape, dgrad, amax_x=ax, amax_dy=ady, direct_into=ctx.wparam)
         if ctx.wparam is None:
diff --git a/dcnet_amd/lib.py b/dcnet_amd/lib.py
--- a/dcnet_amd/lib.py
+++ b/dcnet_amd/lib.py
@@ -37,7 +37,7 @@
     "dcn_gemm3_presplit": (I, [P, I, L, P, I, L, I, I, I, P, P]),
     "dcn_gemm3": (I, [P, I, L, I, P, I, L, I, P, I, L, P, L, I, I, I, I, I, P, P, P]),
     "dcn_filter_job_bytes": (I, []),
-    "dcn_prepare_filters": (I, [P, I, I, I, P, L, P]),
+    "dcn_prepare_filters": (I, [P, I, I, I, P, L, I, P]),
     "dcn_conv2d_geom_size": (L, [I, I, I, I, I]),
     "dcn_conv2d_geom": (I, [P, I, I, I, I, I, P]),
     "dcn_conv2d_bwd_weight": (I, [P, I, P, I, P, P, P, P, I, I, I, I, I, I, I, P, P, P]),
@@ -189,7 +189,7 @@
                 "dcn_conv2d_stats_rows_b16", "dcn_bn_act_bwd_reduce_rows_b16", "dcn_conv2d_stats_rows_f8", "dcn_quant_fusable", "dcn_quant_job_bytes",
                 "dcn_conv1_tile", "dcn_l2norm_score_fwd_form", "dcn_bn_apply_form", "dcn_igemm_split_build", "dcn_gemm3_variant",
                 "dcn_coattn_bank_form"}
-ABI_VERSION = 317
+ABI_VERSION = 318
 
 
 class DcnError(RuntimeError):
diff --git a/dcnet_amd/ops.py b/dcnet_amd/ops.py
--- a/dcnet_amd/ops.py
+++ b/dcnet_amd/ops.py
@@ -503,12 +503,43 @@
 FILTER_BANKS = True
 
 
+FORM_BITS = {"ohwi": 1, "split": 2, "t": 4, "tsplit": 8, "b16": 16, "tb16": 32}
+_FORMS_FP32, _FORM_KEEP_AMAX = 1 | 4, 64
+MODE_FORMS = {"fp32": _FORMS_FP32 | 2 | 8, "fp32_mfma": _FORMS_FP32, "fp32_bf16x3": _FORMS_FP32, "fp8": _FORMS_FP32,
+              "bf16": _FORMS_FP32 | 16 | 32, "bf16s": _FORMS_FP32 | 16 | 32, "fp8s": _FORMS_FP32 | 16 | 32}
+
+
+def bank_reads(form: str) -> bool:
+    return bool(MODE_FORMS[_precision] & FORM_BITS[form])
+
+
+def bank_form(bank, form: str):
+    return bank[form] if bank_reads(form) else None
+
+
+class _Bank(dict):
+
+    def __init__(self, owner, entries):
+        super().__init__(entries)
+        self._owner = owner
+
+    def __getitem__(self, key):
+        bit = FORM_BITS.get(key)
+        if bit:
+            self._owner.fill(bit)
+        return dict.__getitem__(self, key)
+
+    def peek(self, key):
+        return dict.__getitem__(self, key)
+
+
 class FilterBanks:
 
     def __init__(self, weights, device):
         import struct
         self.device = torch.device(device)
         self.items = {}
+        self.fresh = 0
         pairs = weights.items() if isinstance(weights, dict) else enumerate(weights)
         ok = [(i, w) for i, w in pairs if w is not None and w.dim() == 4 and w.shape[0] % 32 == 0 and w.shape[1] % 32 == 0
               and w.is_cuda and w.dtype == torch.float32 and w.is_contiguous()]
@@ -529,11 +560,11 @@
             am = self.amax[j * AMAX_WORDS:(j + 1) * AMAX_WORDS]
             b16 = torch.empty(numel, dtype=torch.bfloat16, device=self.device)
             tb16 = torch.empty(numel, dtype=torch.bfloat16, device=self.device)
-            self.items[i] = dict(ohwi=ohwi, split=split, t=t, tsplit=tsplit, amax=am, b16=b16, tb16=tb16, shape=(co, ci, kh, kw))
+            self.items[i] = _Bank(self, dict(ohwi=ohwi, split=split, t=t, tsplit=tsplit, amax=am, b16=b16, tb16=tb16, shape=(co, ci, kh, kw)))
             blob += struct.pack("<8Q6i", w.data_ptr(), 0 if ohwi is None else ohwi.data_ptr(), split.data_ptr(), t.data_ptr(),
                                 tsplit.data_ptr(), am.data_ptr(), b16.data_ptr(), tb16.data_ptr(), co, ci, T, blk, ablk, 0)
             self._ptrs.append((i, w.data_ptr()))
-            blk += T * (co // 32) * (ci // 32); ablk += (numel + 4095) // 4096
+            blk += (co // 32) * (ci // 32); ablk += (numel + 4095) // 4096
         self.njobs, self.blocks, self.ablocks = len(ok), blk, ablk
         self._q8_jobs = None; self._q8_key = None
         self.jobs = torch.frombuffer(blob, dtype=torch.uint8).clone().to(self.device) if ok else None
@@ -544,10 +575,25 @@
 
     def refresh(self):
         if self.njobs:
+            forms = MODE_FORMS[_precision]
             lib().prepare_filters(self.jobs.data_ptr(), self.njobs, self.blocks, self.ablocks, self.amax.data_ptr(),
-                                  self.amax.numel(), _s())
+                                  self.amax.numel(), forms, _s())
+            self.fresh = forms
             if storage_f8():
                 self._refresh_q8()
+
+    def fill(self, forms: int) -> None:
+        missing = forms & ~self.fresh
+        if not (missing and self.njobs):
+            return
+        if not self.fresh:
+            self.refresh()
+            missing = forms & ~self.fresh
+            if not missing:
+                return
+        lib().prepare_filters(self.jobs.data_ptr(), self.njobs, self.blocks, self.ablocks, self.amax.data_ptr(), self.amax.numel(),
+                              missing | _FORM_KEEP_AMAX, _s())
+        self.fresh |= missing
 
     def _refresh_q8(self):
         import struct
@@ -558,7 +604,7 @@
             for it in self.items.values():
                 co, ci, kh, kw = it["shape"]
                 it.pop("q8", None); it.pop("tq8", None)
-                for key, src, rows, ok in (("q8", it["b16"], co, f8_takes(ci, co, kh)), ("tq8", it["tb16"], ci, f8_takes(co, ci, kh))):
+                for key, src, rows, ok in (("q8", it.peek("b16"), co, f8_takes(ci, co, kh)), ("tq8", it.peek("tb16"), ci, f8_takes(co, ci, kh))):
                     if not ok:
                         continue
                     c = src.numel() // rows
@@ -577,9 +623,9 @@
         it = self.items.get(i)
         if it is None:
             return None
-        if it["ohwi"] is None:
-            co, ci, kh, kw = it["shape"]
-            it = dict(it); it["ohwi"] = w.detach().view(co, 1, 1, ci)
+        if it.peek("ohwi") is None:
+            co, ci, kh, kw = it.peek("shape")
+            it = _Bank(self, it); dict.__setitem__(it, "ohwi", w.detach().view(co, 1, 1, ci))
         return it
 
 
diff --git a/include/dcnet_hip.h b/include/dcnet_hip.h
--- a/include/dcnet_hip.h
+++ b/include/dcnet_hip.h
@@ -17,7 +17,7 @@
 #define DCN_ACT_NONE 0
 #define DCN_ACT_LEAKY 1
 
-#define DCN_ABI_VERSION 317
+#define DCN_ABI_VERSION 318
 
 const char* dcn_last_error(void);
 int dcn_version(void);
@@ -65,8 +65,15 @@
                               const float* pre_scale, const float* pre_shift, int pre_act, float pre_slope,
                               const uint32_t* amax_x, const uint32_t* amax_dy, void* stream);
 int dcn_filter_job_bytes(void);
+#define DCN_FORM_OHWI 1
+#define DCN_FORM_SPLIT 2
+#define DCN_FORM_T 4
+#define DCN_FORM_TSPLIT 8
+#define DCN_FORM_B16 16
+#define DCN_FORM_TB16 32
+#define DCN_FORM_KEEP_AMAX 64
 int dcn_prepare_filters(const void* jobs, int njobs, int total_blocks, int total_amax_blocks,
-                        uint32_t* amax_all, int64_t amax_words, void* stream);
+                        uint32_t* amax_all, int64_t amax_words, int forms, void* stream);
 
 int64_t dcn_conv2d_geom_size(int n, int h, int wd, int ksize, int stride);
 int dcn_conv2d_geom(uint32_t* table, int n, int h, int wd, int ksize, int stride, void* stream);
```

Result: no change. 87.06 clips/s, median of 6 (+0.4%).
